# pk17r/online_3d_reconstruction

Hardware: AMD Instinct MI355X
Metric: frames_per_sec (higher is better)
Workload: dtype f32; 1 GPU; synthetic 1280x720 dense stereo, jump_pixels 1, 200 frames/GPU, voxel_size 0.05, min_points_per_voxel 1, SOR off, frames resident in HBM (BASELINE.json configs[1]); frames_per_gpu=200, rows=720, cols=1280, jump_pixels=1, parallelism=frame-sharded x1

## Files before the change

### include/o3dr_testing.h

```cpp
#ifndef O3DR_TESTING_H
#define O3DR_TESTING_H
#include "o3dr.h"
#ifdef __cplusplus
extern "C" {
#endif

int o3dr_test_corrupt_next_gather(o3dr_ctx* ctx);

int o3dr_test_sor_distances(o3dr_ctx* ctx, float* out, int64_t n);

int o3dr_test_local_comm_create(int32_t n_ranks, void** comm_out);
int o3dr_test_local_comm_destroy(void* comm);
int o3dr_test_merge_partitioned_local(o3dr_ctx* ctx, void* local_comm, int32_t rank, int32_t gather_result, o3dr_point* out,
                                      int64_t out_capacity, int64_t* n_out, int64_t* n_total, uint32_t* status, int32_t mem);
int o3dr_test_fail_at(o3dr_ctx* ctx, int32_t point);
int o3dr_test_plane_hypotheses(o3dr_ctx* ctx, float* planes, uint32_t* counts, int64_t capacity, int64_t* n_out);

#ifdef __cplusplus
}
#endif
#endif
```

### online_3d_reconstruction_amd/_lib.py

```python
import ctypes as C
import os

import numpy as np

_HERE = os.path.dirname(os.path.abspath(__file__))
_LIB = os.path.join(_HERE, "lib", "libo3dr.so")

POINT = np.dtype([("x", "<f4"), ("y", "<f4"), ("z", "<f4"), ("rgba", "<u4")])

OK = 0
ERR_INVALID_ARG, ERR_NO_DEVICE, ERR_HIP, ERR_CAPACITY, ERR_NOT_CONFIGURED, ERR_ALLOC, ERR_INTERNAL, ERR_PEER = -1, -2, -3, -4, -5, -6, -7, -8
MEM_HOST, MEM_DEVICE = 0, 1
STATUS_VOXEL_OVERFLOW = 1
STATUS_INTERNAL = 0x80000000
K_COUNT, K_REPROJECT, K_KEYGEN, K_SORT_HIST, K_SORT_SCATTER, K_SEGMENT, K_CENTROID, K_OTHER, K_CENTROID_RUNS = range(9)
KERNEL_NAMES = ["reproject_count", "reproject_emit", "voxel_keys", "radix_hist", "radix_scatter", "run_segments",
                "centroid", "other", "centroid_runs"]


class O3drError(RuntimeError):
    def __init__(self, code, text):
        super().__init__(f"libo3dr error {code}: {text}")
        self.code = code

# ... 51 lines not shown

KNN2 = np.dtype([("train_idx", "<u4", (2,)), ("distance", "<u4", (2,))])
assert KNN2.itemsize == 16
RIGID_RESULT = np.dtype([("T", "<f8", (16,)), ("rms", "<f8"), ("n_used", "<i8"), ("status", "<i4"), ("reserved", "<i4")])
assert RIGID_RESULT.itemsize == C.sizeof(RigidResultStruct) == 152
MATCH_NONE = 0xFFFFFFFF
RIGID_OK, RIGID_TOO_FEW, RIGID_DEGENERATE = range(3)


def lib_path():
    return _LIB


_vp, _i64, _i32, _u32, _f = C.c_void_p, C.c_int64, C.c_int32, C.c_uint32, C.c_float
_pi64, _pu32 = C.POINTER(C.c_int64), C.POINTER(C.c_uint32)
SYMBOLS = [
    ("o3dr_version", C.c_int, []),
    ("o3dr_last_error", C.c_char_p, []),
    ("o3dr_default_params", None, [C.POINTER(ParamsStruct)]),
    ("o3dr_ctx_create", C.c_int, [C.c_int, C.POINTER(_vp)]),
    ("o3dr_ctx_destroy", C.c_int, [_vp]),
    ("o3dr_ctx_set_stream", C.c_int, [_vp, _vp]),
    ("o3dr_ctx_synchronize", C.c_int, [_vp]),
    ("o3dr_set_camera", C.c_int, [_vp, _vp]),
    ("o3dr_set_params", C.c_int, [_vp, C.POINTER(ParamsStruct)]),
    ("o3dr_get_params", C.c_int, [_vp, C.POINTER(ParamsStruct)]),
    ("o3dr_create_single_img_pt_cloud", C.c_int, [_vp, _vp, _i64, _vp, _i64, _i32, _i32, _vp, _i32, _vp, _i64, _pi64, _i32]),
    ("o3dr_max_points", _i64, [_vp, _i32, _i32]),
    ("o3dr_transform_pt_cloud", C.c_int, [_vp, _vp, _i64, _vp, _vp, _i32]),
    ("o3dr_reproject_transform", C.c_int, [_vp, _vp, _i64, _vp, _i64, _i32, _i32, _vp, _vp, _i32, _vp, _i64, _pi64, _i32]),
    ("o3dr_voxel_grid", C.c_int, [_vp, _vp, _i64, _vp, _u32, _f, _vp, _i64, _pi64, _pu32, _i32]),
    ("o3dr_statistical_outlier_removal", C.c_int, [_vp, _vp, _i64, _vp, _i64, _pi64, _i32]),
    ("o3dr_bilateral_filter_u8", C.c_int, [_vp, _vp, _i64, _i32, _i32, _i32, C.c_double, C.c_double, _vp, _i64, _i32]),
    ("o3dr_disparity_variance", C.c_int, [_vp, _vp, _i64, _i64, _i32, _i32, _i32, _vp, _i32]),
    ("o3dr_downsample_pt_cloud", C.c_int, [_vp, _vp, _i64, _i32, _vp, _i64, _pi64, _pu32, _i32]),
    ("o3dr_create_and_transform_pt_cloud", C.c_int, [_vp, _vp, _i64, _vp, _i64, _i32, _i32, _vp, _vp, _i32, _vp, _i64, _pi64, _pu32, _i32]),
    ("o3dr_accumulate_frames", C.c_int, [_vp, _vp, _i64, _i64, _vp, _i64, _i64, _i32, _i32, _vp, _i32, _i32]),
    ("o3dr_accumulate_frames_kp", C.c_int, [_vp, _vp, _i64, _i64, _vp, _i64, _i64, _i32, _i32, _vp, _i32, _vp, _vp, _i32]),
    ("o3dr_cloud_big_reserve", C.c_int, [_vp, _i64]),
    ("o3dr_cloud_big_reset", C.c_int, [_vp]),
    ("o3dr_cloud_big_size", C.c_int, [_vp, _pi64, _pu32]),
    ("o3dr_cloud_big_read", C.c_int, [_vp, _vp, _i64, _pi64, _i32]),
    ("o3dr_cloud_big_append", C.c_int, [_vp, _vp, _i64, _i32]),
    ("o3dr_cloud_big_transform", C.c_int, [_vp, _vp]),
    ("o3dr_finalize", C.c_int, [_vp, _vp, _i64, _pi64, _pu32, _i32]),
    ("o3dr_finalize_incremental", C.c_int, [_vp, _vp, _i64, _pi64, _pu32, _i32]),
    ("o3dr_finalize_incremental_stats", C.c_int, [_vp, _pi64]),
    ("o3dr_cloud_big_bbox", C.c_int, [_vp, _vp, _vp, _pi64]),
    ("o3dr_cloud_big_partition", C.c_int, [_vp, _vp, _vp, _i32, _pi64, _pu32]),
    ("o3dr_finalize_global", C.c_int, [_vp, _vp, _vp, _vp, _i64, _pi64, _pu32, _i32]),
    ("o3dr_cloud_big_view", C.c_int, [_vp, C.POINTER(_vp), _pi64]),
    ("o3dr_cloud_big_recv_buffer", C.c_int, [_vp, _i64, C.POINTER(_vp)]),
    ("o3dr_cloud_big_adopt", C.c_int, [_vp, _i64]),
    ("o3dr_cloud_big_header_dev", C.c_int, [_vp, _vp]),
    ("o3dr_cloud_big_assume_size", C.c_int, [_vp, _i64]),
    ("o3dr_cloud_big_partition_dev", C.c_int, [_vp, _vp, _i32, _i32, _vp]),
    ("o3dr_cloud_big_slice_counts_dev", C.c_int, [_vp, _vp, _i32, _i32, _vp]),
    ("o3dr_cloud_big_place_slices", C.c_int, [_vp, _i32, _i32, _vp, _i64, _i64, _pi64]),
    ("o3dr_cloud_big_set_size", C.c_int, [_vp, _i64]),
    ("o3dr_cloud_big_raw_view", C.c_int, [_vp, C.POINTER(_vp), _pi64]),
    ("o3dr_merge_partitioned", C.c_int, [_vp, _vp, _i32, _vp, _i64, _pi64, _pi64, C.POINTER(C.c_uint32), _i32]),
    ("o3dr_merge_partitioned_stats", C.c_int, [_vp, _pi64]),
    ("o3dr_cloud_big_capacity", C.c_int, [_vp, _pi64, _pi64]),
    ("o3dr_comm_init_all", C.c_int, [_i32, _vp, _vp]),
    ("o3dr_comm_destroy", C.c_int, [_vp]),
    ("o3dr_host_register", C.c_int, [_vp, _i64]),
    ("o3dr_host_unregister", C.c_int, [_vp]),
    ("o3dr_icp_default_params", None, [C.POINTER(IcpParamsStruct)]),
    ("o3dr_nearest_neighbors", C.c_int, [_vp, _vp, _i64, _vp, _i64, C.c_double, _vp, _vp, _i32]),
    ("o3dr_icp_align", C.c_int, [_vp, _vp, _i64, _vp, _i64, _vp, C.POINTER(IcpParamsStruct), C.POINTER(IcpResultStruct), _i32]),
    ("o3dr_match_default_params", None, [C.POINTER(MatchParamsStruct)]),
    ("o3dr_match_knn2_hamming", C.c_int, [_vp, _vp, _vp, _i32, _vp, _i64, C.POINTER(MatchParamsStruct), _vp, _vp, _i64, _pi64, _i32]),
    ("o3dr_keypoints_3d", C.c_int, [_vp, _vp, _i64, _i64, _vp, _i64, _i64, _i32, _i32, _vp, _i32, _vp, _vp, _vp, _i64, _pi64, _i32]),
    ("o3dr_estimate_rigid_transform", C.c_int, [_vp, _vp, _vp, _i64, _vp, _i32, _vp, _vp, _i32]),
    ("o3dr_mls_default_params", None, [C.POINTER(MlsParamsStruct)]),
    ("o3dr_mls_smooth", C.c_int, [_vp, _vp, _i64, C.POINTER(MlsParamsStruct), _vp, _vp, _vp, _vp, C.POINTER(MlsResultStruct), _i32]),
    ("o3dr_plane_default_params", None, [C.POINTER(PlaneParamsStruct)]),
    ("o3dr_segment_plane", C.c_int, [_vp, _vp, _i64, C.POINTER(PlaneParamsStruct), _vp, _vp, _vp, _vp, _i64, _pi64, _i32]),
    ("o3dr_profile_enable", C.c_int, [_vp, _i32, _i32]),
    ("o3dr_profile_read", C.c_int, [_vp, _i32, C.POINTER(C.c_double), _pi64]),
    ("o3dr_profile_reset", C.c_int, [_vp]),
    ("o3dr_profile_stats", C.c_int, [_vp, _pi64]),
    ("o3dr_test_corrupt_next_gather", C.c_int, [_vp]),
    ("o3dr_test_sor_distances", C.c_int, [_vp, _vp, _i64]),
    ("o3dr_test_local_comm_create", C.c_int, [_i32, C.POINTER(_vp)]),
    ("o3dr_test_local_comm_destroy", C.c_int, [_vp]),
    ("o3dr_test_merge_partitioned_local", C.c_int, [_vp, _vp, _i32, _i32, _vp, _i64, _pi64, _pi64, C.POINTER(C.c_uint32), _i32]),
    ("o3dr_test_fail_at", C.c_int, [_vp, _i32]),
    ("o3dr_test_plane_hypotheses", C.c_int, [_vp, _vp, _vp, _i64, _pi64]),
    ("o3dr_device_info", C.c_int, [_vp, C.c_char_p, _i32, C.POINTER(_i32), _pi64]),
]

_lib = None


def load_library():
    global _lib
    if _lib is None:
        if not os.path.exists(_LIB):
            raise O3drError(ERR_NO_DEVICE, f"{_LIB} is not built: run `python __graft_entry__.py` or `make` "
                                           "(there is no CPU fallback)")
        try:
            import torch
        except ImportError:
            pass
        L = C.CDLL(_LIB)
        for name, res, args in SYMBOLS:
            fn = getattr(L, name)
            fn.restype = res
            fn.argtypes = args
        _lib = L
    return _lib


def check(code):
    if code != OK:
        raise O3drError(code, load_library().o3dr_last_error().decode(errors="replace"))
```

### online_3d_reconstruction_amd/csrc/kernels/bookkeeping.inc

```

__global__ void k_minmax_init(float* mm, int64_t mm_stride, int slot, uint32_t* n_kp, int frames)
{
    const int i = blockIdx.x * blockDim.x + threadIdx.x;
    if (i < frames * 6) {
        const int f = i / 6, a = i % 6;
        mm[((int64_t)f * mm_stride + slot) * 6 + a] = (a < 3) ? __builtin_inff() : -__builtin_inff();
    }
    if (n_kp && i < frames) n_kp[i] = 0;
}
__global__ void k_set_counts(uint32_t* n_dev, uint32_t value, int frames)
{
    const int i = blockIdx.x * blockDim.x + threadIdx.x;
    if (i < frames) n_dev[i] = value;
}

__device__ __forceinline__ int64_t scan_row_len(const VoxelGeom* __restrict__ geom, int f, int pass, int n_tiles,
                                                int64_t L)
{
    if (!geom) return L;
    const VoxelGeom g = geom[f];
    if (g.overflow || pass >= (int)g.passes) return 0;
    return (int64_t)geom_bins(g) * n_tiles;
}
__device__ __forceinline__ int scan_live_tiles(const VoxelGeom* __restrict__ geom, int f, int n_tiles)
{
    if (!geom) return n_tiles;
    const int64_t live = ((int64_t)geom[f].n + kSortTile - 1) / kSortTile;
    return live < n_tiles ? (int)live : n_tiles;
}
__global__ __launch_bounds__(1024) void k_scan_rows(uint32_t* __restrict__ data, int64_t L_in, int64_t row_stride,
                                                    uint32_t* __restrict__ totals, const uint32_t* __restrict__ add,
                                                    const VoxelGeom* __restrict__ geom, int pass, int n_tiles,
                                                    int chunked)
{
    __shared__ uint32_t lds[1024 / 64 + 1];
    uint32_t* row = data + (int64_t)blockIdx.x * row_stride;
    int64_t L = scan_row_len(geom, blockIdx.x, pass, n_tiles, L_in);
    if (chunked) L = (L + 4095) / 4096;
    if (L == 0 && !totals) return;
    const int64_t chunk = (L + 1023) / 1024;
    const int64_t b = (int64_t)threadIdx.x * chunk;
    const int64_t e = (b + chunk < L) ? b + chunk : L;
    const bool tiles = geom != nullptr && !chunked;
    const int live = tiles ? scan_live_tiles(geom, blockIdx.x, n_tiles) : 0;
    uint32_t s = 0;
    {
        int t = tiles ? (int)(b % n_tiles) : 0;
        for (int64_t i = b; i < e; ++i) {
            if (!tiles || t < live) s += row[i];
            if (tiles && ++t == n_tiles) t = 0;
        }
    }
    uint32_t total;
    uint32_t run = block_excl_scan_u32<16>(s, lds, total);
    {
        int t = tiles ? (int)(b % n_tiles) : 0;
        for (int64_t i = b; i < e; ++i) {
            const uint32_t v = (!tiles || t < live) ? row[i] : 0u;
            row[i] = run;
            run += v;
            if (tiles && ++t == n_tiles) t = 0;
        }
    }
    if (totals && threadIdx.x == 0) totals[blockIdx.x] = total + (add ? add[blockIdx.x] : 0u);
}

__global__ __launch_bounds__(1024) void k_scan_hist_tm(uint32_t* __restrict__ hist, const VoxelGeom* __restrict__ geom, int pass,
                                                       int n_tiles)
{
    extern __shared__ uint32_t tm_row[];
    __shared__ uint32_t lds[1024 / 64 + 1];
    const int f = blockIdx.x;
    const VoxelGeom g = geom[f];
    if (g.overflow || pass >= (int)g.passes) return;
    const int bins = geom_bins(g);
    uint32_t* row = hist + (int64_t)f * kMaxRadix * n_tiles;
    const int words = n_tiles * kMaxRadix;
    const int live = scan_live_tiles(geom, f, n_tiles);
    for (int i = threadIdx.x; i < words; i += 1024)
        tm_row[(i >> kMaxRadixBits) * (kMaxRadix + 1) + (i & (kMaxRadix - 1))] = (i >> kMaxRadixBits) < live ? row[i] : 0u;
    __syncthreads();
    const int L = bins * n_tiles;
    const int chunk = (L + 1023) / 1024;
    const int b = (int)threadIdx.x * chunk, e = b + chunk < L ? b + chunk : L;
    uint32_t s = 0;
    {
        int d = b / n_tiles, t = b - d * n_tiles;
        for (int i = b; i < e; ++i) {
            s += tm_row[t * (kMaxRadix + 1) + d];
            if (++t == n_tiles) t = 0, ++d;
        }
    }
    uint32_t total;
    uint32_t run = block_excl_scan_u32<16>(s, lds, total);
    {
        int d = b / n_tiles, t = b - d * n_tiles;
        for (int i = b; i < e; ++i) {
            const uint32_t v = tm_row[t * (kMaxRadix + 1) + d];
            tm_row[t * (kMaxRadix + 1) + d] = run;
            run += v;
            if (++t == n_tiles) t = 0, ++d;
        }
    }
    __syncthreads();
    for (int i = threadIdx.x; i < words; i += 1024)
        if ((i & (kMaxRadix - 1)) < bins) row[i] = tm_row[(i >> kMaxRadixBits) * (kMaxRadix + 1) + (i & (kMaxRadix - 1))];
}

constexpr int kScanChunk = 4096;
__global__ __launch_bounds__(256) void k_scan_chunk_sums(const uint32_t* __restrict__ data, int64_t L_in,
                                                         int64_t row_stride, int n_chunks,
                                                         uint32_t* __restrict__ partial,
                                                         const VoxelGeom* __restrict__ geom, int pass, int n_tiles)
{
    __shared__ uint32_t lds[4];
    const int64_t L = scan_row_len(geom, blockIdx.y, pass, n_tiles, L_in);
    if ((int64_t)blockIdx.x * kScanChunk >= L) return;
    const uint32_t* row = data + (int64_t)blockIdx.y * row_stride;
    const int64_t b = (int64_t)blockIdx.x * kScanChunk + (int64_t)threadIdx.x * 16;
    const int live = scan_live_tiles(geom, blockIdx.y, n_tiles);
    int t = geom ? (int)(b % n_tiles) : 0;
    uint32_t s = 0;
#pragma unroll
    for (int k = 0; k < 16; ++k) {
        if (b + k < L && (!geom || t < live)) s += row[b + k];
        if (geom && ++t == n_tiles) t = 0;
    }
    s = wave_sum_u32(s);
    if ((threadIdx.x & 63) == 0) lds[threadIdx.x >> 6] = s;
    __syncthreads();
    if (threadIdx.x == 0) partial[(int64_t)blockIdx.y * n_chunks + blockIdx.x] = lds[0] + lds[1] + lds[2] + lds[3];
}
__global__ __launch_bounds__(256) void k_scan_chunk_apply(uint32_t* __restrict__ data, int64_t L_in, int64_t row_stride,
                                                          int n_chunks, const uint32_t* __restrict__ partial_scanned,
                                                          const VoxelGeom* __restrict__ geom, int pass, int n_tiles)
{
    __shared__ uint32_t lds[5];
    const int64_t L = scan_row_len(geom, blockIdx.y, pass, n_tiles, L_in);
    if ((int64_t)blockIdx.x * kScanChunk >= L) return;
    uint32_t* row = data + (int64_t)blockIdx.y * row_stride;
    const int64_t b = (int64_t)blockIdx.x * kScanChunk + (int64_t)threadIdx.x * 16;
    const int live = scan_live_tiles(geom, blockIdx.y, n_tiles);
    int t = geom ? (int)(b % n_tiles) : 0;
    uint32_t v[16];
    uint32_t s = 0;
#pragma unroll
    for (int k = 0; k < 16; ++k) {
        v[k] = (b + k < L && (!geom || t < live)) ? row[b + k] : 0u;
        s += v[k];
        if (geom && ++t == n_tiles) t = 0;
    }
    uint32_t total;
    uint32_t run = block_excl_scan_u32<4>(s, lds, total) + partial_scanned[(int64_t)blockIdx.y * n_chunks + blockIdx.x];
#pragma unroll
    for (int k = 0; k < 16; ++k) {
        if (b + k < L) row[b + k] = run;
        run += v[k];
    }
}

__global__ __launch_bounds__(kPtThreads) void k_points_minmax(const o3dr_point* __restrict__ in, int64_t in_fstride,
                                                              const uint32_t* __restrict__ n_dev, int64_t mm_stride,
                                                              float* __restrict__ mm)
{
    __shared__ float mm_lds[6 * (kPtThreads / 64)];
    const int f = blockIdx.y;
    const int64_t n = n_dev[f];
    const uint4* src = reinterpret_cast<const uint4*>(in + (int64_t)f * in_fstride);
    float lo[3] = {__builtin_inff(), __builtin_inff(), __builtin_inff()};
    float hi[3] = {-__builtin_inff(), -__builtin_inff(), -__builtin_inff()};
    bool any = false;
    const int64_t stride = (int64_t)gridDim.x * (kPtThreads * 4);
    for (int64_t base = (int64_t)blockIdx.x * (kPtThreads * 4); base < n; base += stride) {
#pragma unroll
        for (int k = 0; k < 4; ++k) {
            const int64_t i = base + k * kPtThreads + threadIdx.x;
            if (i < n) {
// ... 12 lines not shown
```

### online_3d_reconstruction_amd/csrc/kernels/radix_sort.inc

```

__device__ __forceinline__ int64_t hist_at(bool tm, int dgt, int tile, int n_tiles)
{
    return tm ? (int64_t)tile * kMaxRadix + dgt : (int64_t)dgt * n_tiles + tile;
}

__global__ __launch_bounds__(kSortThreads) void k_radix_hist(const uint32_t* __restrict__ keys0,
                                                             const uint32_t* __restrict__ keys1, int64_t cap,
                                                             const VoxelGeom* __restrict__ geom, int pass,
                                                             int n_tiles, uint32_t* __restrict__ hist,
                                                             uint32_t* __restrict__ hist_part, int tm)
{
    constexpr int kSub = 4;
    __shared__ uint32_t h[kSub * kSortWaves * kMaxRadix];
    const int f = blockIdx.y, tile = blockIdx.x;
    const VoxelGeom g = geom[f];
    if (g.overflow || pass >= (int)g.passes) return;
    const uint32_t n = g.n;
    if ((int64_t)tile * kSortTile >= (int64_t)n) return;
    const int bins = geom_bins(g), shift = pass * (int)g.bpp;
    const uint32_t dmask = (uint32_t)bins - 1u;
    for (int i = threadIdx.x; i < kSub * kSortWaves * kMaxRadix; i += kSortThreads) h[i] = 0;
    __syncthreads();
    const uint32_t* src = (((pass + g.buf0) & 1) ? keys1 : keys0) + (int64_t)f * cap;
    const int64_t base = (int64_t)tile * kSortTile;
    uint32_t* hw = h + (((threadIdx.x >> 6) * kSub) + (threadIdx.x & (kSub - 1))) * kMaxRadix;
    if (base < n) {
        const bool vec = (((int64_t)f * cap) & 3) == 0;
        static_assert(kScatParts == 2 && kSortRounds / 4 == 4, "the first scatter part is rounds 0 and 1");
        uint4 v[kSortRounds / 4];
        bool whole[kSortRounds / 4];
#pragma unroll
        for (int r = 0; r < kSortRounds / 4; ++r) {
            const int64_t i = base + ((int64_t)r * kSortThreads + threadIdx.x) * 4;
            whole[r] = vec && i + 3 < n;
            if (whole[r]) v[r] = stream_load_u4(reinterpret_cast<const uint4*>(src + i));
        }
#pragma unroll
        for (int r = 0; r < kSortRounds / 4; ++r) {
            const int64_t i = base + ((int64_t)r * kSortThreads + threadIdx.x) * 4;
            if (r == kSortRounds / 8) {
                __syncthreads();
                for (int dgt = threadIdx.x; dgt < bins; dgt += kSortThreads) {
                    uint32_t t = 0;
#pragma unroll
                    for (int ww = 0; ww < kSub * kSortWaves; ++ww) t += h[ww * kMaxRadix + dgt];
                    hist_part[(int64_t)f * kMaxRadix * n_tiles + hist_at(tm != 0, dgt, tile, n_tiles)] = t;
                }
                __syncthreads();
            }
            if (whole[r]) {
                atomicAdd(&hw[(v[r].x >> shift) & dmask], 1u);
                atomicAdd(&hw[(v[r].y >> shift) & dmask], 1u);
                atomicAdd(&hw[(v[r].z >> shift) & dmask], 1u);
                atomicAdd(&hw[(v[r].w >> shift) & dmask], 1u);
            } else {
                for (int k = 0; k < 4; ++k)
                    if (i + k < n) atomicAdd(&hw[(src[i + k] >> shift) & dmask], 1u);
            }
        }
    }
    __syncthreads();
    uint32_t* dst = hist + (int64_t)f * kMaxRadix * n_tiles;
    for (int dgt = threadIdx.x; dgt < bins; dgt += kSortThreads) {
        uint32_t t = 0;
#pragma unroll
        for (int ww = 0; ww < kSub * kSortWaves; ++ww) t += h[ww * kMaxRadix + dgt];
        dst[hist_at(tm != 0, dgt, tile, n_tiles)] = t;
    }
}

__global__ __launch_bounds__(kSortThreads) void k_voxel_keys_hist0(const o3dr_point* __restrict__ in, int64_t in_fstride,
                                                                   const VoxelGeom* __restrict__ geom, float z_offset,
                                                                   int64_t cap, uint32_t* __restrict__ keys, int n_tiles,
                                                                   uint32_t* __restrict__ hist, uint32_t* __restrict__ hist_part,
                                                                   const VoxelGeom* __restrict__ skip_grouped, int tm)
{
    constexpr int kSub = 4;
    __shared__ uint32_t h[kSub * kSortWaves * kMaxRadix];
    const int f = blockIdx.y, tile = blockIdx.x;
    const VoxelGeom g = geom[f];
    if (g.overflow || g.n == 0u || g.passes == 0u) return;
    if (skip_grouped && skip_grouped[f].grouped != 0u) return;
    const uint32_t n = g.n;
    const int64_t base = (int64_t)tile * kSortTile;
    if (base >= (int64_t)n) return;
    const int bins = geom_bins(g);
    const uint32_t dmask = (uint32_t)bins - 1u;
    for (int i = threadIdx.x; i < kSub * kSortWaves * kMaxRadix; i += kSortThreads) h[i] = 0;
    __syncthreads();
    const uint4* src = reinterpret_cast<const uint4*>(in + (int64_t)f * in_fstride);
    uint32_t* dst = keys + (int64_t)f * cap;
    uint32_t* hw = h + (((threadIdx.x >> 6) * kSub) + (threadIdx.x & (kSub - 1))) * kMaxRadix;
#pragma unroll
    for (int r = 0; r < kSortRounds; ++r) {
        const int64_t i = base + (int64_t)r * kSortThreads + threadIdx.x;
        if (r == kSortRounds / kScatParts) {
            __syncthreads();
            for (int dgt = threadIdx.x; dgt < bins; dgt += kSortThreads) {
                uint32_t t = 0;
#pragma unroll
                for (int ww = 0; ww < kSub * kSortWaves; ++ww) t += h[ww * kMaxRadix + dgt];
                hist_part[(int64_t)f * kMaxRadix * n_tiles + hist_at(tm != 0, dgt, tile, n_tiles)] = t;
            }
            __syncthreads();
        }
        if (i < n) {
            const uint32_t key = voxel_key_of(src[i], g, z_offset);
            dst[i] = key;
            atomicAdd(&hw[key & dmask], 1u);
        }
    }
    __syncthreads();
    uint32_t* hd = hist + (int64_t)f * kMaxRadix * n_tiles;
    for (int dgt = threadIdx.x; dgt < bins; dgt += kSortThreads) {
        uint32_t t = 0;
#pragma unroll
        for (int ww = 0; ww < kSub * kSortWaves; ++ww) t += h[ww * kMaxRadix + dgt];
        hd[hist_at(tm != 0, dgt, tile, n_tiles)] = t;
    }
}

constexpr int kCntStride = 17;
constexpr int kCntWords = kMaxRadix * kCntStride;
constexpr int kRankWords = kScatWaves * kCntWords;
struct ScatterLds {
    __attribute__((aligned(16))) uint32_t smem[kRankWords > 2 * kScatTile ? kRankWords : 2 * kScatTile];
    uint32_t wave_tot[kScatWaves * kMaxRadix];
    uint32_t local_base[kMaxRadix];
    uint32_t delta[kMaxRadix];
    uint32_t scan_lds[kScatWaves + 1];
};
struct ScatterJob {
    const uint32_t *kin, *vin;
    uint32_t *kout, *vout;
    const uint32_t* hist;
    const uint32_t* hist_part;
    uint32_t n, dmask;
    int shift, bins, pass, n_tiles;
    bool frame_vec;
    bool tm;
};

__device__ __forceinline__ void scatter_load(const ScatterJob& J, int tile, int part, uint32_t (&key)[kSortRounds],
                                             uint32_t (&val)[kSortRounds], uint32_t& gstart)
{
    const int lane = threadIdx.x & 63, w = threadIdx.x >> 6;
    const int64_t n = J.n;
    const int64_t lbase = (int64_t)tile * kSortTile + (int64_t)part * kScatTile + (int64_t)w * kSortWaveItems + (int64_t)lane * kSortRounds;
    gstart = 0;
    if ((int)threadIdx.x < J.bins) {
        gstart = J.hist[hist_at(J.tm, threadIdx.x, tile, J.n_tiles)];
        if (part != 0) gstart += J.hist_part[hist_at(J.tm, threadIdx.x, tile, J.n_tiles)];
    }
    const bool vec = J.frame_vec && (lbase + kSortRounds <= n);
    if (vec) {
#pragma unroll
        for (int q = 0; q < kSortRounds / 4; ++q) {
            const uint4 k4 = *reinterpret_cast<const uint4*>(J.kin + lbase + 4 * q);
            key[4 * q] = k4.x; key[4 * q + 1] = k4.y; key[4 * q + 2] = k4.z; key[4 * q + 3] = k4.w;
        }
        if (J.pass != 0) {
#pragma unroll
            for (int q = 0; q < kSortRounds / 4; ++q) {
                const uint4 v4 = *reinterpret_cast<const uint4*>(J.vin + lbase + 4 * q);
                val[4 * q] = v4.x; val[4 * q + 1] = v4.y; val[4 * q + 2] = v4.z; val[4 * q + 3] = v4.w;
            }
        }
    } else {
#pragma unroll
        for (int r = 0; r < kSortRounds; ++r) {
            const int64_t i = lbase + r;
            const bool ok = i < n;
            key[r] = ok ? J.kin[i] : 0xffffffffu;
            val[r] = (J.pass != 0 && ok) ? J.vin[i] : 0u;
        }
    }
    if (J.pass == 0) {
#pragma unroll
        for (int r = 0; r < kSortRounds; ++r) val[r] = (uint32_t)(lbase + r);
    }
}

__device__ __forceinline__ void scatter_tile(const ScatterJob& J, int tile, int part, ScatterLds& L, const uint32_t (&key)[kSortRounds],
                                             const uint32_t (&val)[kSortRounds], uint32_t gstart)
{
    uint32_t* smem = L.smem;
    uint32_t* stage = L.smem;
    const int lane = threadIdx.x & 63, w = threadIdx.x >> 6;
    const int64_t n = J.n;
    const int64_t base = (int64_t)tile * kSortTile + (int64_t)part * kScatTile;
    const uint32_t cnt = (n - base < (int64_t)kScatTile) ? (uint32_t)(n - base) : (uint32_t)kScatTile;
    const int64_t lbase = base + (int64_t)w * kSortWaveItems + (int64_t)lane * kSortRounds;
    const int shift = J.shift, bins = J.bins;
    const uint32_t dmask = J.dmask;
    for (int i = threadIdx.x; i < kRankWords; i += kScatThreads) smem[i] = 0;
    __syncthreads();

    uint32_t* cw = smem + w * kCntWords;
    const int quad = lane >> 2, sub = lane & 3;
    const uint32_t fsh = 7u * (uint32_t)sub;
    uint32_t own[kSortRounds];
#pragma unroll
    for (int r = 0; r < kSortRounds; ++r) {
        own[r] = 0;
        if (lbase + r < n) {
            const uint32_t dgt = (key[r] >> shift) & dmask;
            const uint32_t old = atomicAdd(&cw[dgt * kCntStride + quad], 1u << fsh);
            own[r] = (old >> fsh) & 127u;
        }
    }
    __builtin_amdgcn_wave_barrier();
#pragma unroll
    for (int h = 0; h < kMaxRadix / 64; ++h) {
        const int row = lane + 64 * h;
        if (row < bins) {
            uint32_t run = 0;
#pragma unroll
            for (int j = 0; j < 16; ++j) {
                const uint32_t v = cw[row * kCntStride + j];
                const uint32_t t = v + (v << 7);
                const uint32_t t2 = t + (t << 14);
                cw[row * kCntStride + j] = (run << 21) | (t2 & 0x1fffffu);
                run += (t2 >> 21) & 127u;
            }
            L.wave_tot[w * kMaxRadix + row] = run;
        }
    }
    __syncthreads();

    uint32_t tot = 0;
    const int dg = threadIdx.x;
    if (dg < bins) {
#pragma unroll
        for (int ww = 0; ww < kScatWaves; ++ww) {
            const uint32_t t = L.wave_tot[ww * kMaxRadix + dg];
            L.wave_tot[ww * kMaxRadix + dg] = tot;
            tot += t;
        }
    }
    uint32_t tile_total;
    const uint32_t lb = block_excl_scan_u32<kScatWaves>(tot, L.scan_lds, tile_total);
    if (dg < bins) {
        L.local_base[dg] = lb;
        L.delta[dg] = gstart - lb;
    }
    __syncthreads();

    uint32_t pos[kSortRounds];
    const uint32_t qsh = sub ? 7u * (uint32_t)(sub - 1) : 0u, qmk = sub ? 127u : 0u;
#pragma unroll
    for (int r = 0; r < kSortRounds; ++r) {
        if (lbase + r < n) {
            const uint32_t dgt = (key[r] >> shift) & dmask;
            const uint32_t v = cw[dgt * kCntStride + quad];
            pos[r] = L.local_base[dgt] + L.wave_tot[w * kMaxRadix + dgt] + (v >> 21) + ((v >> qsh) & qmk) + own[r];
        }
    }
    __syncthreads();
    uint32_t* stage_v = L.smem + kScatTile;
#pragma unroll
    for (int r = 0; r < kSortRounds; ++r) {
        if (lbase + r < n) {
            stage[pos[r]] = key[r];
            stage_v[pos[r]] = val[r];
        }
    }
    __syncthreads();
#pragma unroll
    for (int r = 0; r < kSortRounds; ++r) {
        const uint32_t p = r * kScatThreads + threadIdx.x;
        if (p < cnt) {
            const uint32_t k = stage[p];
            const uint32_t d = p + L.delta[(k >> shift) & dmask];
            J.kout[d] = k;
            J.vout[d] = stage_v[p];
        }
    }
}

__global__ __launch_bounds__(kScatThreads) void k_radix_scatter_lane(uint32_t* __restrict__ keys0, uint32_t* __restrict__ vals0,
                                                                     uint32_t* __restrict__ keys1, uint32_t* __restrict__ vals1,
                                                                     int64_t cap, const VoxelGeom* __restrict__ geom, int pass,
                                                                     int n_tiles, const uint32_t* __restrict__ hist_scanned,
                                                                     const uint32_t* __restrict__ hist_part, int tm)
{
    __shared__ ScatterLds L;
    const int f = blockIdx.y;
    const VoxelGeom g = geom[f];
    if (g.overflow || pass >= (int)g.passes) return;
    const int item = xcd_chunk_item(blockIdx.x, (int)(((int64_t)g.n + kScatTile - 1) / kScatTile));
    if (item < 0) return;
    const int tile = item / kScatParts, part = item % kScatParts;
    ScatterJob J;
    const int par = (pass + (int)g.buf0) & 1;
    J.kin = (par ? keys1 : keys0) + (int64_t)f * cap;
    J.vin = (par ? vals1 : vals0) + (int64_t)f * cap;
    J.kout = (par ? keys0 : keys1) + (int64_t)f * cap;
    J.vout = (par ? vals0 : vals1) + (int64_t)f * cap;
    J.hist = hist_scanned + (int64_t)f * kMaxRadix * n_tiles;
    J.hist_part = hist_part + (int64_t)f * kMaxRadix * n_tiles;
    J.n = g.n;
    J.bins = geom_bins(g);
    J.dmask = (uint32_t)J.bins - 1u;
    J.shift = pass * (int)g.bpp;
    J.pass = pass;
    J.n_tiles = n_tiles;
    J.frame_vec = (((int64_t)f * cap) & 3) == 0;
    J.tm = tm != 0;
    uint32_t key0[kSortRounds], val0[kSortRounds], g0;
    scatter_load(J, tile, part, key0, val0, g0);
    scatter_tile(J, tile, part, L, key0, val0, g0);
}
```

### online_3d_reconstruction_amd/csrc/kernels/util.inc

```

__device__ __forceinline__ int xcd_chunk_item(int bx, int n_active)
{
    const int chunk = (n_active + kXcds - 1) / kXcds, q = bx / kXcds;
    const int item = (bx % kXcds) * chunk + q;
    return (q < chunk && item < n_active) ? item : -1;
}
typedef uint32_t u32x4_t __attribute__((ext_vector_type(4)));
__device__ __forceinline__ uint4 stream_load_u4(const uint4* p)
{
    const u32x4_t v = __builtin_nontemporal_load(reinterpret_cast<const u32x4_t*>(p));
    return make_uint4(v.x, v.y, v.z, v.w);
}
__device__ __forceinline__ uint32_t wave_incl_scan_u32(uint32_t v)
{
    v += (uint32_t)__builtin_amdgcn_update_dpp(0, (int)v, 0x111, 0xf, 0xf, false);
    v += (uint32_t)__builtin_amdgcn_update_dpp(0, (int)v, 0x112, 0xf, 0xf, false);
    v += (uint32_t)__builtin_amdgcn_update_dpp(0, (int)v, 0x114, 0xf, 0xf, false);
    v += (uint32_t)__builtin_amdgcn_update_dpp(0, (int)v, 0x118, 0xf, 0xf, false);
    v += (uint32_t)__builtin_amdgcn_update_dpp(0, (int)v, 0x142, 0xa, 0xf, false);
    v += (uint32_t)__builtin_amdgcn_update_dpp(0, (int)v, 0x143, 0xc, 0xf, false);
    return v;
}
__device__ __forceinline__ int32_t wave_shr1_i32(int32_t v) { return __builtin_amdgcn_update_dpp(v, v, 0x138, 0xf, 0xf, false); }
__device__ __forceinline__ uint32_t wave_max_u32(uint32_t v)
// ... 23 lines not shown
    return (uint32_t)__builtin_amdgcn_readlane((int)wave_incl_scan_u32(v), 63);
}
__device__ __forceinline__ uint32_t f32_ordered(float f)
{
    const uint32_t u = __float_as_uint(f);
    return u ^ ((uint32_t)((int32_t)u >> 31) | 0x80000000u);
}
__device__ __forceinline__ float ordered_f32(uint32_t u) { return __uint_as_float(u ^ (((u >> 31) - 1u) | 0x80000000u)); }
#define O3DR_WAVE_REDUCE_ORD(name, op, ident)                                                                                  \
    __device__ __forceinline__ float name(float f)                                                                       \
    {                                                                                                                    \
         \
        uint32_t v = f32_ordered(f);                                                                                     \
        v = op(v, (uint32_t)__builtin_amdgcn_update_dpp((int)(ident), (int)v, 0x111, 0xf, 0xf, false));                  \
        v = op(v, (uint32_t)__builtin_amdgcn_update_dpp((int)(ident), (int)v, 0x112, 0xf, 0xf, false));                  \
        v = op(v, (uint32_t)__builtin_amdgcn_update_dpp((int)(ident), (int)v, 0x114, 0xf, 0xf, false));                  \
        v = op(v, (uint32_t)__builtin_amdgcn_update_dpp((int)(ident), (int)v, 0x118, 0xf, 0xf, false));                  \
        v = op(v, (uint32_t)__builtin_amdgcn_update_dpp((int)(ident), (int)v, 0x142, 0xa, 0xf, false));                  \
        v = op(v, (uint32_t)__builtin_amdgcn_update_dpp((int)(ident), (int)v, 0x143, 0xc, 0xf, false));                  \
        return ordered_f32((uint32_t)__builtin_amdgcn_readlane((int)v, 63));                                             \
    }
__device__ __forceinline__ uint32_t u32_min(uint32_t a, uint32_t b) { return a < b ? a : b; }
__device__ __forceinline__ uint32_t u32_max(uint32_t a, uint32_t b) { return a > b ? a : b; }
O3DR_WAVE_REDUCE_ORD(wave_min_f32, u32_min, 0xffffffffu)
O3DR_WAVE_REDUCE_ORD(wave_max_f32, u32_max, 0u)
#undef O3DR_WAVE_REDUCE_ORD
template <int NW>
__device__ __forceinline__ uint32_t block_excl_scan_u32(uint32_t v, uint32_t* lds, uint32_t& total)
{
    const int lane = threadIdx.x & 63, w = threadIdx.x >> 6;
    const uint32_t incl = wave_incl_scan_u32(v);
    if (lane == 63) lds[w] = incl;
    __syncthreads();
    if (threadIdx.x == 0) {
        uint32_t run = 0;
#pragma unroll
        for (int i = 0; i < NW; ++i) {
            const uint32_t t = lds[i];
            lds[i] = run;
            run += t;
        }
        lds[NW] = run;
    }
    __syncthreads();
    const uint32_t r = lds[w] + incl - v;
    total = lds[NW];
    __syncthreads();
    return r;
}
template <int NW, int N>
__device__ __forceinline__ void block_excl_scan_multi_u32(uint32_t (&v)[N], uint32_t* lds, uint32_t (&total)[N])
{
    const int lane = threadIdx.x & 63, w = threadIdx.x >> 6;
    uint32_t incl[N];
#pragma unroll
    for (int j = 0; j < N; ++j) {
        incl[j] = wave_incl_scan_u32(v[j]);
        if (lane == 63) lds[w * N + j] = incl[j];
    }
    __syncthreads();
    if ((int)threadIdx.x < N) {
        uint32_t run = 0;
#pragma unroll
        for (int i = 0; i < NW; ++i) {
            const uint32_t t = lds[i * N + threadIdx.x];
            lds[i * N + threadIdx.x] = run;
            run += t;
        }
        lds[NW * N + threadIdx.x] = run;
    }
    __syncthreads();
#pragma unroll
    for (int j = 0; j < N; ++j) {
        v[j] = lds[w * N + j] + incl[j] - v[j];
        total[j] = lds[NW * N + j];
    }
    __syncthreads();
}
__device__ __forceinline__ int geom_bins(const VoxelGeom& g)
{
    const uint32_t bpp = g.bpp < (uint32_t)kMaxRadixBits ? g.bpp : (uint32_t)kMaxRadixBits;
    return 1 << bpp;
}
__device__ __forceinline__ uint32_t voxel_key_of(const uint4 v, const VoxelGeom& g, float z_offset)
{
    const float x = __uint_as_float(v.x), y = __uint_as_float(v.y), z = __uint_as_float(v.z) + z_offset;
    const int32_t i0 = (int32_t)floorf(x * g.inv[0]) - g.min_b[0];
    const int32_t i1 = (int32_t)floorf(y * g.inv[1]) - g.min_b[1];
    const int32_t i2 = (int32_t)floorf(z * g.inv[2]) - g.min_b[2];
    return (uint32_t)i0 + (uint32_t)i1 * g.mul1 + (uint32_t)i2 * g.mul2;
}
struct GroupCoord {
    int32_t bx, iy, iz;
};
__device__ __forceinline__ GroupCoord group_coord_of(const uint4 v, const float inv[3], float z_offset, uint32_t& cell)
{
    const float x = __uint_as_float(v.x), y = __uint_as_float(v.y), z = __uint_as_float(v.z) + z_offset;
    const int32_t i0 = (int32_t)floorf(x * inv[0]);
    cell = (uint32_t)(i0 & (kGroupCells - 1));
    GroupCoord c;
    c.bx = i0 >> kGroupBits;
    c.iy = (int32_t)floorf(y * inv[1]);
    c.iz = (int32_t)floorf(z * inv[2]);
    return c;
}
__device__ __forceinline__ bool group_differs(const GroupCoord& a, const GroupCoord& b)
{
    return a.bx != b.bx || a.iy != b.iy || a.iz != b.iz;
}
__device__ __forceinline__ uint32_t group_blocks_x(const VoxelGeom& g)
{
    return (uint32_t)(((g.min_b[0] + g.div_b[0] - 1) >> kGroupBits) - (g.min_b[0] >> kGroupBits) + 1);
}
__device__ __forceinline__ uint32_t group_key_of(const GroupCoord& c, const VoxelGeom& g)
{
    const uint32_t i1 = (uint32_t)(c.iy - g.min_b[1]), i2 = (uint32_t)(c.iz - g.min_b[2]);
    return (uint32_t)(c.bx - (g.min_b[0] >> kGroupBits)) + group_blocks_x(g) * (i1 + (uint32_t)g.div_b[1] * i2);
}
__device__ __forceinline__ void head_flag_place(uint64_t i, uint64_t& word, uint32_t& bit)
{
    word = i >> 4;
    bit = (uint32_t)(((i >> 2) & 3u) * 8u + (i & 3u));
}
__device__ __forceinline__ const uint32_t* sorted_buf(const VoxelGeom& g, const uint32_t* b0, const uint32_t* b1)
{
    return ((g.passes + g.buf0) & 1u) ? b1 : b0;
}
template <int NW>
__device__ __forceinline__ void block_minmax_store(const float lo[3], const float hi[3], bool any,
                                                   float* lds , float* __restrict__ slot6)
{
    const int lane = threadIdx.x & 63, w = threadIdx.x >> 6;
#pragma unroll
    for (int a = 0; a < 3; ++a) {
        const float l = wave_min_f32(any ? lo[a] : __builtin_inff());
        const float h = wave_max_f32(any ? hi[a] : -__builtin_inff());
        if (lane == 0) {
            lds[w * 6 + a] = l;
            lds[w * 6 + 3 + a] = h;
        }
    }
    __syncthreads();
    if (threadIdx.x < 6) {
        const int a = threadIdx.x;
        float v = lds[a];
#pragma unroll
        for (int i = 1; i < NW; ++i) v = (a < 3) ? fminf(v, lds[i * 6 + a]) : fmaxf(v, lds[i * 6 + a]);
        slot6[a] = v;
    }
    __syncthreads();
}

constexpr int kMlsJacobiSweeps = 8;
__device__ __forceinline__ void mls_jacobi3(double A[3][3], double V[3][3])
{
#pragma unroll
    for (int i = 0; i < 3; ++i)
#pragma unroll
        for (int j = 0; j < 3; ++j) V[i][j] = i == j ? 1.0 : 0.0;
    A[1][0] = A[0][1], A[2][0] = A[0][2], A[2][1] = A[1][2];
#pragma unroll
    for (int sweep = 0; sweep < kMlsJacobiSweeps; ++sweep) {
#pragma unroll
        for (int pq = 0; pq < 3; ++pq) {
            const int p = pq == 2 ? 1 : 0, q = pq == 0 ? 1 : 2, r = 3 - p - q;
            const double apq = A[p][q];
// ... 20 lines not shown
```

### online_3d_reconstruction_amd/csrc/kernels/voxel_runs.inc

```


constexpr int kHeadWaves = 4;
__global__ __launch_bounds__(kHeadWaves * kWave) void k_run_heads(const uint32_t* __restrict__ keys0, const uint32_t* __restrict__ keys1,
                                                                  int64_t cap, const VoxelGeom* __restrict__ geom, int n_tiles,
                                                                  uint32_t* __restrict__ seg_cnt, int buf_sel,
                                                                  uint8_t* __restrict__ head_bits)
{
    static_assert(kSegTile == 16 * kWave, "16 records per lane");
    const int f = blockIdx.y, lane = threadIdx.x & 63;
    const int tile = blockIdx.x * kHeadWaves + (threadIdx.x >> 6);
    const VoxelGeom g = geom[f];
    if (g.overflow || tile >= n_tiles) return;
    const int64_t n = g.n;
    const uint32_t* k = (buf_sel < 0 ? sorted_buf(g, keys0, keys1) : (buf_sel ? keys1 : keys0)) + (int64_t)f * cap;
    uint32_t c = 0;
    const int64_t i0 = (int64_t)tile * kSegTile + lane * 16;
    if ((int64_t)tile * kSegTile < n) {
        uint32_t kk[16];
        if (((((int64_t)f * cap) & 3) == 0) && i0 + 15 < n) {
#pragma unroll
            for (int q = 0; q < 4; ++q) {
                const uint4 v = *reinterpret_cast<const uint4*>(k + i0 + 4 * q);
                kk[4 * q] = v.x; kk[4 * q + 1] = v.y; kk[4 * q + 2] = v.z; kk[4 * q + 3] = v.w;
            }
        } else {
#pragma unroll
            for (int q = 0; q < 16; ++q) kk[q] = (i0 + q < n) ? k[i0 + q] : 0u;
        }
        uint32_t prev = (uint32_t)wave_shr1_i32((int32_t)kk[15]);
        if (lane == 0) prev = (i0 > 0 && i0 < n) ? k[i0 - 1] : 0u;
        uint32_t bits = 0;
#pragma unroll
        for (int q = 0; q < 16; ++q) {
            const int64_t i = i0 + q;
            if (i < n && (i == 0 || kk[q] != (q ? kk[q - 1] : prev))) bits |= 1u << ((q >> 2) * 8 + (q & 3));
        }
        reinterpret_cast<uint32_t*>(head_bits + ((int64_t)f * n_tiles + tile) * 256)[lane] = bits;
        c = (uint32_t)__popc(bits);
    }
    c = wave_sum_u32(c);
    if (lane == 0) seg_cnt[(int64_t)f * n_tiles + tile] = c;
}

constexpr int kStartWaves = 4;
__global__ __launch_bounds__(kStartWaves * kWave) void k_run_starts(
    const uint32_t* __restrict__ keys0, const uint32_t* __restrict__ keys1, int64_t cap, const VoxelGeom* __restrict__ geom,
    int n_tiles, const uint32_t* __restrict__ seg_off, const uint32_t* __restrict__ n_vox, uint32_t* __restrict__ seg_start,
    int buf_sel, uint32_t* __restrict__ head_keys_out, const VoxelGeom* __restrict__ mode, const o3dr_point* __restrict__ in_pts,
    float z_offset, const uint8_t* __restrict__ head_bits)
{
    static_assert(kSegTile == 16 * kWave, "16 records per lane");
    const int f = blockIdx.y, lane = threadIdx.x & 63;
    const int tile = blockIdx.x * kStartWaves + (threadIdx.x >> 6);
    const VoxelGeom g = geom[f];
    if (g.overflow) return;
    if (mode && mode[f].grouped == 0u) return;
    const uint32_t n = g.n;
    const int64_t base = (int64_t)tile * kSegTile;
    if (tile >= n_tiles || base >= n) return;
    uint32_t* ss = seg_start + (int64_t)f * (cap + 1);
    if (tile == 0 && lane == 0) ss[n_vox[f]] = n;
    uint32_t bits = reinterpret_cast<const uint32_t*>(head_bits + ((int64_t)f * n_tiles + tile) * 256)[lane];
    bits &= 0x0f0f0f0fu;
    if (base + lane * 16 + 16 > (int64_t)n) {
#pragma unroll
        for (int q = 0; q < 16; ++q)
            if (base + lane * 16 + q >= (int64_t)n) bits &= ~(1u << ((q >> 2) * 8 + (q & 3)));
    }
    const uint32_t cnt = (uint32_t)__popc(bits);
    const uint32_t incl = wave_incl_scan_u32(cnt);
    const uint32_t tile_runs = __shfl(incl, 63, 64);
    __shared__ uint32_t stage_all[kStartWaves][kSegTile];
    uint32_t* stage = stage_all[threadIdx.x >> 6];
    uint32_t pos = incl - cnt;
    const uint32_t i0 = (uint32_t)base + (uint32_t)lane * 16u;
#pragma unroll
    for (int q = 0; q < 16; ++q) {
        if (bits & (1u << ((q >> 2) * 8 + (q & 3)))) stage[pos++] = i0 + (uint32_t)q;
    }
    __builtin_amdgcn_wave_barrier();
    const uint32_t off = seg_off[(int64_t)f * n_tiles + tile];
    for (uint32_t j = lane; j < tile_runs; j += kWave) {
        const uint32_t i = stage[j];
        ss[off + j] = i;
        if (head_keys_out) {
            uint32_t cell;
            const GroupCoord gc = group_coord_of(reinterpret_cast<const uint4*>(in_pts)[i], g.inv, z_offset, cell);
            head_keys_out[(int64_t)f * cap + off + j] = group_key_of(gc, g);
        }
    }
}

__global__ __launch_bounds__(256) void k_keep_count(const uint32_t* __restrict__ seg_start, int64_t cap,
                                                    const VoxelGeom* __restrict__ geom,
                                                    const uint32_t* __restrict__ n_vox, uint32_t min_points,
                                                    int n_tiles, uint32_t* __restrict__ seg_cnt)
{
    __shared__ uint32_t lds[4];
    const int f = blockIdx.y, tile = blockIdx.x;
    if (geom[f].overflow || geom[f].grouped != 0u) return;
    const uint32_t nv = n_vox[f];
    const uint32_t* ss = seg_start + (int64_t)f * (cap + 1);
    uint32_t c = 0;
    const int64_t base = (int64_t)tile * kSegTile;
    if (base < nv) {
        for (int j = 0; j < kSegTile / 256; ++j) {
            const int64_t o = base + j * 256 + threadIdx.x;
            if (o < nv) c += (ss[o + 1] - ss[o] >= min_points) ? 1u : 0u;
        }
    }
    c = wave_sum_u32(c);
    if ((threadIdx.x & 63) == 0) lds[threadIdx.x >> 6] = c;
    __syncthreads();
    if (threadIdx.x == 0) seg_cnt[(int64_t)f * n_tiles + tile] = lds[0] + lds[1] + lds[2] + lds[3];
}
__global__ __launch_bounds__(256) void k_keep_write(const uint32_t* __restrict__ seg_start, int64_t cap,
                                                    const VoxelGeom* __restrict__ geom,
                                                    const uint32_t* __restrict__ n_vox, uint32_t min_points,
                                                    int n_tiles, const uint32_t* __restrict__ seg_off,
                                                    uint32_t* __restrict__ keep_idx)
{
    __shared__ uint32_t scan_lds[5];
    const int f = blockIdx.y, tile = blockIdx.x;
    if (geom[f].overflow || geom[f].grouped != 0u) return;
    const uint32_t nv = n_vox[f];
    const int64_t base = (int64_t)tile * kSegTile;
    if (base >= nv) return;
    const uint32_t* ss = seg_start + (int64_t)f * (cap + 1);
    uint32_t* ki = keep_idx + (int64_t)f * cap;
    uint32_t off = seg_off[(int64_t)f * n_tiles + tile];
    for (int j = 0; j < kSegTile / 256; ++j) {
        const int64_t o = base + j * 256 + threadIdx.x;
        const bool keep = (o < nv) && (ss[o + 1] - ss[o] >= min_points);
        uint32_t total;
        const uint32_t pos = block_excl_scan_u32<4>(keep ? 1u : 0u, scan_lds, total);
        if (keep) ki[off + pos] = (uint32_t)o;
        off += total;
    }
}

__global__ __launch_bounds__(256) void k_frame_offsets(const VoxelGeom* __restrict__ geom, const uint32_t* __restrict__ n_vox,
                                                       const uint32_t* __restrict__ n_keep,
                                                       const uint32_t* __restrict__ n_grp, int frames, int passthrough,
                                                       uint32_t* __restrict__ n_out, uint64_t* __restrict__ out_off,
                                                       CloudCounters* __restrict__ cc, SortStats* __restrict__ stats,
                                                       const VoxelGeom* __restrict__ sort_geom)
{
    __shared__ uint32_t scan_lds[5];
    __shared__ unsigned long long acc[6];
    if (threadIdx.x < 6) acc[threadIdx.x] = 0;
    __syncthreads();
    const uint64_t base = cc->count;
    uint64_t carry = 0;
    for (int f0 = 0; f0 < frames; f0 += 256) {
        const int f = f0 + threadIdx.x;
        uint32_t m = 0;
        if (f < frames) {
            const VoxelGeom g = geom[f];
            if (passthrough) {
                m = g.n;
            } else if (g.overflow) {
                m = g.n;
                atomicOr(&acc[3], (unsigned long long)O3DR_STATUS_VOXEL_OVERFLOW);
            } else {
                m = (n_grp && sort_geom[f].grouped) ? n_grp[f] : (n_keep ? n_keep[f] : n_vox[f]);
                atomicAdd(&acc[0], (unsigned long long)sort_geom[f].n * g.passes);
                atomicAdd(&acc[5], (unsigned long long)sort_geom[f].n);
                atomicAdd(&acc[1], (unsigned long long)g.n);
                atomicAdd(&acc[2], (unsigned long long)m);
            }
        }
        uint32_t total;
        const uint32_t excl = block_excl_scan_u32<4>(m, scan_lds, total);
        if (f < frames) {
            n_out[f] = m;
            out_off[f] = base + carry + excl;
        }
        carry += total;
    }
    __syncthreads();
    if (threadIdx.x == 0) {
        cc->count = base + carry;
        cc->status |= (uint32_t)acc[3];
        if (stats) {
            stats->sort_record_passes += acc[0];
            stats->voxel_points_in += acc[1];
            stats->voxel_points_out += acc[2];
            stats->sort_records += acc[5];
        }
    }
}

__global__ void k_test_corrupt_payload(uint32_t* __restrict__ vals0, uint32_t* __restrict__ vals1, const VoxelGeom* __restrict__ geom)
{
    const VoxelGeom g = geom[0];
    if (g.overflow || g.n == 0u) return;
    uint32_t* v = ((g.passes + g.buf0) & 1u) ? vals1 : vals0;
    v[g.n / 2u] = 0xfffffff0u;
}

__device__ __forceinline__ void centroid_block(int64_t bx, int f, const VoxelGeom& g, uint32_t n_o,
                                               const o3dr_point* __restrict__ in, int64_t in_fstride,
                                               const uint32_t* __restrict__ vals0, const uint32_t* __restrict__ vals1,
                                               int64_t cap, const uint32_t* __restrict__ seg_start,
                                               const uint32_t* __restrict__ keep_idx, const uint64_t* __restrict__ out_off,
                                               float z_offset, int passthrough, o3dr_point* __restrict__ out_base,
                                               float* __restrict__ out_mm, int nbx, CloudCounters* __restrict__ cc,
                                               const CloudHeads& ch)
{
    const int64_t o = bx * kPtThreads + threadIdx.x;
    const bool active = o < (int64_t)n_o;
    if (__ballot(active) == 0ull) return;
    uint4 res = make_uint4(0, 0, 0, 0);
    if (active) {
        const uint4* src = reinterpret_cast<const uint4*>(in + (int64_t)f * in_fstride);
        if (passthrough) {
            res = src[o];
        } else if (g.overflow) {
            res = src[o];
            res.z = __float_as_uint((__uint_as_float(res.z) + z_offset) - z_offset);
        } else {
            const uint32_t* ss = seg_start + (int64_t)f * (cap + 1);
            const uint32_t* pid = sorted_buf(g, vals0, vals1) + (int64_t)f * cap;
            const uint32_t v = keep_idx ? keep_idx[(int64_t)f * cap + o] : (uint32_t)o;
            uint32_t b = ss[v], e = ss[v + 1];
            bool bad = b > e || e > g.n;
            if (bad) b = e = 0;
            float sx = 0.f, sy = 0.f, sz = 0.f, sr = 0.f, sg = 0.f, sb = 0.f, sa = 0.f;
            for (uint32_t li = b; li < e; li += 8) {
                uint32_t id[8];
                uint4 p[8];
#pragma unroll
                for (int k = 0; k < 8; ++k) {
                    id[k] = (li + k < e) ? pid[li + k] : 0xffffffffu;
                    if (id[k] != 0xffffffffu && id[k] >= g.n) {
                        bad = true;
                        id[k] = 0xffffffffu;
                    }
                }
#pragma unroll
                for (int k = 0; k < 8; ++k)
                    if (id[k] != 0xffffffffu) p[k] = src[id[k]];
#pragma unroll
                for (int k = 0; k < 8; ++k) {
                    if (id[k] != 0xffffffffu) {
                        sx += __uint_as_float(p[k].x);
                        sy += __uint_as_float(p[k].y);
                        sz += __uint_as_float(p[k].z) + z_offset;
                        sr += (float)((p[k].w >> 16) & 255u);
                        sg += (float)((p[k].w >> 8) & 255u);
                        sb += (float)(p[k].w & 255u);
                        sa += (float)(p[k].w >> 24);
                    }
                }
            }
            const float nf = (float)(e - b);
            const float cx = sx / nf, cy = sy / nf, cz = sz / nf - z_offset;
            const uint32_t rgba = ((uint32_t)(sa / nf) << 24) | ((uint32_t)(sr / nf) << 16) | ((uint32_t)(sg / nf) << 8) |
                                  (uint32_t)(sb / nf);
            res = make_uint4(__float_as_uint(cx), __float_as_uint(cy), __float_as_uint(cz), rgba);
            if (bad) atomicOr(&cc->status, O3DR_STATUS_INTERNAL);
        }
        reinterpret_cast<uint4*>(out_base + out_off[f])[o] = res;
    }
    if (ch.flags) {
        uint32_t cell;
        GroupCoord gc = {0, 0, 0};
        if (active) gc = group_coord_of(res, ch.inv, ch.z_offset, cell);
        GroupCoord prev;
        prev.bx = wave_shr1_i32(gc.bx);
        prev.iy = wave_shr1_i32(gc.iy);
        prev.iz = wave_shr1_i32(gc.iz);
        const int lane = threadIdx.x & 63;
        const unsigned long long hm = __ballot(active && lane != 0 && group_differs(gc, prev));
        if (hm != 0ull && lane < 5) {
            const uint64_t g0 = out_off[f] + (uint64_t)(o - lane);
            const uint64_t word = (g0 >> 4) + (uint64_t)lane;
            const int shift = (int)((int64_t)(word << 4) - (int64_t)g0);
            uint32_t f16 = 0;
            if (shift < 64) f16 = (uint32_t)((shift >= 0 ? (hm >> shift) : (hm << -shift)) & 0xffffull);
            const uint32_t bits = (f16 & 0xfu) | ((f16 & 0xf0u) << 4) | ((f16 & 0xf00u) << 8) | ((f16 & 0xf000u) << 12);
            if (bits) atomicOr(&ch.flags[word], bits);
        }
        int32_t* slot = ch.wave_gc + (((int64_t)f * nbx + bx) * (kPtThreads / 64) + (threadIdx.x >> 6)) * 6;
        const int last = 63 - __builtin_clzll(__ballot(active));
        const int32_t f0 = __builtin_amdgcn_readlane(gc.bx, 0), f1 = __builtin_amdgcn_readlane(gc.iy, 0),
                      f2 = __builtin_amdgcn_readlane(gc.iz, 0);
        const int32_t l0 = __builtin_amdgcn_readlane(gc.bx, last), l1 = __builtin_amdgcn_readlane(gc.iy, last),
                      l2 = __builtin_amdgcn_readlane(gc.iz, last);
        if (lane < 6) slot[lane] = lane == 0 ? f0 : (lane == 1 ? f1 : (lane == 2 ? f2 : (lane == 3 ? l0 : (lane == 4 ? l1 : l2))));
    }
    if (out_mm) {
        float* slot = out_mm + (((int64_t)f * nbx + bx) * (kPtThreads / 64) + (threadIdx.x >> 6)) * 6;
        const float c3[3] = {__uint_as_float(res.x), __uint_as_float(res.y), __uint_as_float(res.z)};
        float mine = 0.f;
#pragma unroll
        for (int a = 0; a < 3; ++a) {
            const float l = wave_min_f32(active ? c3[a] : __builtin_inff());
            const float h = wave_max_f32(active ? c3[a] : -__builtin_inff());
            if ((threadIdx.x & 63) == a) mine = l;
            if ((threadIdx.x & 63) == 3 + a) mine = h;
        }
        if ((threadIdx.x & 63) < 6) slot[threadIdx.x & 63] = mine;
    }
}

template <bool kStride>
__global__ __launch_bounds__(kPtThreads) void k_centroid(const o3dr_point* __restrict__ in, int64_t in_fstride,
                                                         const uint32_t* __restrict__ vals0,
                                                         const uint32_t* __restrict__ vals1, int64_t cap,
                                                         const uint32_t* __restrict__ seg_start,
                                                         const uint32_t* __restrict__ keep_idx,
                                                         const VoxelGeom* __restrict__ geom,
                                                         const uint32_t* __restrict__ n_out,
                                                         const uint64_t* __restrict__ out_off, float z_offset,
                                                         int passthrough, o3dr_point* __restrict__ out_base,
                                                         float* __restrict__ out_mm, int nbx, CloudCounters* __restrict__ cc,
                                                         CloudHeads ch)
{
    const int f = blockIdx.y;
    const VoxelGeom g = geom[f];
    if (!passthrough && (g.n == 0 || g.grouped != 0u)) return;
    const uint32_t n_o = n_out[f];
    if (kStride) {
        for (int64_t bx = blockIdx.x; bx * kPtThreads < (int64_t)n_o; bx += gridDim.x)
            centroid_block(bx, f, g, n_o, in, in_fstride, vals0, vals1, cap, seg_start, keep_idx, out_off, z_offset,
                           passthrough, out_base, out_mm, nbx, cc, ch);
    } else {
        const int bx = xcd_chunk_item(blockIdx.x, (int)(((int64_t)n_o + kPtThreads - 1) / kPtThreads));
        if (bx < 0) return;
        centroid_block(bx, f, g, n_o, in, in_fstride, vals0, vals1, cap, seg_start, keep_idx, out_off, z_offset,
                       passthrough, out_base, out_mm, nbx, cc, ch);
    }
}

__global__ __launch_bounds__(256) void k_cloud_heads_fix(const uint32_t* __restrict__ n_out, const uint64_t* __restrict__ out_off,
                                                         int waves_per_frame, CloudHeads ch)
{
    const int f = blockIdx.y;
    const int64_t j = (int64_t)blockIdx.x * 256 + threadIdx.x;
    if (j >= waves_per_frame || j * kWave >= (int64_t)n_out[f]) return;
    bool head = j == 0;
    if (!head) {
        const int32_t* cur = ch.wave_gc + ((int64_t)f * waves_per_frame + j) * 6;
        head = cur[0] != cur[-3] || cur[1] != cur[-2] || cur[2] != cur[-1];
    }
    if (head) {
        uint64_t word;
        uint32_t bit;
        head_flag_place(out_off[f] + (uint64_t)j * kWave, word, bit);
        atomicOr(&ch.flags[word], 1u << bit);
    }
}

__global__ __launch_bounds__(256) void k_cloud_bbox_fold(const float* __restrict__ slots, int nbx, int frames,
                                                         const uint32_t* __restrict__ n_out, float* __restrict__ partial)
{
    __shared__ float mm_lds[6 * 4];
    float lo[3] = {__builtin_inff(), __builtin_inff(), __builtin_inff()};
    float hi[3] = {-__builtin_inff(), -__builtin_inff(), -__builtin_inff()};
    const int64_t total = (int64_t)nbx * frames;
    for (int64_t i = (int64_t)blockIdx.x * 256 + threadIdx.x; i < total; i += (int64_t)gridDim.x * 256) {
        const int f = (int)(i / nbx), bx = (int)(i - (int64_t)f * nbx);
        if ((int64_t)bx * 64 < (int64_t)n_out[f]) {
#pragma unroll
            for (int a = 0; a < 3; ++a) {
                lo[a] = fminf(lo[a], slots[i * 6 + a]);
                hi[a] = fmaxf(hi[a], slots[i * 6 + 3 + a]);
            }
        }
    }
    block_minmax_store<4>(lo, hi, true, mm_lds, partial + (int64_t)blockIdx.x * 6);
}
__global__ __launch_bounds__(384) void k_cloud_bbox_merge(const float* __restrict__ partial, int n_partial, float* __restrict__ box6)
{
    const int a = threadIdx.x >> 6, lane = threadIdx.x & 63;
    float v = a < 3 ? __builtin_inff() : -__builtin_inff();
    for (int i = lane; i < n_partial; i += 64) v = a < 3 ? fminf(v, partial[i * 6 + a]) : fmaxf(v, partial[i * 6 + a]);
    v = a < 3 ? wave_min_f32(v) : wave_max_f32(v);
    if (lane == 0) box6[a] = a < 3 ? fminf(box6[a], v) : fmaxf(box6[a], v);
}

__global__ void k_run_geom(const VoxelGeom* __restrict__ geom, const uint32_t* __restrict__ n_runs, int frames,
                           VoxelGeom* __restrict__ geom_runs, int force, int64_t slots)
{
    const int f = blockIdx.x * blockDim.x + threadIdx.x;
    if (f >= frames) return;
    VoxelGeom g = geom[f];
    const uint32_t nr = n_runs[f];
    const uint64_t group_keys = (uint64_t)group_blocks_x(g) * (uint64_t)(uint32_t)g.div_b[1] * (uint64_t)(uint32_t)g.div_b[2];
    uint64_t max_groups = group_keys;
    if ((uint64_t)nr < max_groups) max_groups = nr;
    const bool fits = max_groups * kGroupCells <= (uint64_t)slots;
    const bool pays = (uint64_t)nr * kGroupMinRunNum <= (uint64_t)g.n * kGroupMinRunDen;
    if (g.overflow) {
        g.grouped = 1;
        g.n = 0;
    } else if (fits && (pays || force)) {
        g.grouped = 1;
        g.n = nr;
        g.buf0 = 1;
        sort_plan(g, group_keys);
    }
    geom_runs[f] = g;
}

constexpr int kGroupChunks = 4;
constexpr int kGroupStep = kGroupChunks * kWave;
struct GroupLds {
    uint4 sorted[kGroupStep];
    unsigned long long mask[kWave][kGroupChunks];
    uint32_t pre[kWave][kGroupChunks];
    unsigned long long bnd[kGroupChunks];
};
__global__ __launch_bounds__(kGroupWaves * kWave) void k_centroid_groups(
    const o3dr_point* __restrict__ in, const uint32_t* __restrict__ keys0, const uint32_t* __restrict__ keys1,
    const uint32_t* __restrict__ ids0, const uint32_t* __restrict__ ids1, const uint32_t* __restrict__ seg_start,
    const uint32_t* __restrict__ run_start, const VoxelGeom* __restrict__ geom_runs, const VoxelGeom* __restrict__ geom_pts,
    const uint32_t* __restrict__ n_vox, float z_offset, uint32_t min_points, uint4* __restrict__ slots, int64_t n_slots,
    uint32_t* __restrict__ grp_cnt, CloudCounters* __restrict__ cc)
{
    __shared__ GroupLds lds[kGroupWaves];
    const VoxelGeom g = geom_runs[0];
    if (g.grouped == 0u || g.overflow) return;
    const VoxelGeom gp = geom_pts[0];
    const int lane = threadIdx.x & 63, w = threadIdx.x >> 6;
    GroupLds& L = lds[w];
#pragma unroll
    for (int q = 0; q < kGroupChunks; ++q) L.mask[lane][q] = 0ull;
    if (lane < kGroupChunks) L.bnd[lane] = 0ull;
    __builtin_amdgcn_wave_barrier();
    const uint32_t nv = n_vox[0], n_rec = g.n, n_points = gp.n;
    const uint32_t* sk = sorted_buf(g, keys0, keys1);
    const uint32_t* rv = sorted_buf(g, ids0, ids1);
    const uint4* src = reinterpret_cast<const uint4*>(in);
    const uint32_t need = min_points > 1u ? min_points : 1u;
    const bool flat = gp.div_b[2] == 1 && (uint32_t)gp.div_b[0] < (1u << 24) && (uint32_t)gp.div_b[1] < (1u << 24);
    const int32_t bx0 = gp.min_b[0] >> kGroupBits;
    const uint32_t nbx = group_blocks_x(gp);
    const unsigned long long lanes_below = (1ull << lane) - 1ull;
    const unsigned long long starts_upto = (2ull << lane) - 2ull;
    bool bad = false;
    for (uint32_t v = blockIdx.x * kGroupWaves + w; v < nv; v += gridDim.x * kGroupWaves) {
        uint32_t jb = seg_start[v], je = seg_start[v + 1];
        if (jb >= je || je > n_rec || ((int64_t)v + 1) * kGroupCells > n_slots) {
            bad = true;
            if (lane == 0 && ((int64_t)v + 1) * kGroupCells <= n_slots) grp_cnt[v] = 0;
// ... 98 lines not shown
                    }
                }
                __builtin_amdgcn_wave_barrier();
#pragma unroll
                for (int q = 0; q < kGroupChunks; ++q) {
                    if (okm & (1u << q)) {
                        const uint32_t pos = (L.pre[cq[q]][q] + (uint32_t)__popcll(L.mask[cq[q]][q] & lanes_below)) &
                                             (uint32_t)(kGroupStep - 1);
                        L.sorted[pos] = make_uint4(p[q].x, p[q].y, __float_as_uint(__uint_as_float(p[q].z) + z_offset), p[q].w);
                    }
                }
                __builtin_amdgcn_wave_barrier();
#pragma unroll
                for (int q = 0; q < kGroupChunks; ++q) L.mask[lane][q] = 0ull;
                n_pts += cnt;
                const uint32_t trips = wave_max_u32(cnt);
                for (uint32_t t = 0; t < trips; t += 4) {
                    uint4 a4[4];
#pragma unroll
                    for (int j = 0; j < 4; ++j) {
                        const uint4* at = (t + j < cnt) ? &L.sorted[(off + t) & (uint32_t)(kGroupStep - 1)] : &L.sorted[0];
                        a4[j] = at[j];
                    }
#pragma unroll
                    for (int j = 0; j < 4; ++j) {
                        if (t + j < cnt) {
                            const uint32_t c4 = a4[j].w;
                            s_xy += f32x2{__uint_as_float(a4[j].x), __uint_as_float(a4[j].y)};
                            sz += __uint_as_float(a4[j].z);
                            s_rg += f32x2{(float)((c4 >> 16) & 255u), (float)((c4 >> 8) & 255u)};
                            s_ba += f32x2{(float)(c4 & 255u), (float)(c4 >> 24)};
                        }
                    }
                }
                __builtin_amdgcn_wave_barrier();
#pragma unroll
                for (int q = 0; q < kGroupChunks; ++q) p[q] = pn[q];
                okm = okn;
            }
        }
        const bool keep = n_pts >= need;
        const unsigned long long km = __ballot(keep);
        if (keep) {
            const float nf = (float)n_pts;
            const float cx = s_xy.x / nf, cy = s_xy.y / nf, cz = sz / nf - z_offset;
            const uint32_t rgba = ((uint32_t)(s_ba.y / nf) << 24) | ((uint32_t)(s_rg.x / nf) << 16) | ((uint32_t)(s_rg.y / nf) << 8) |
                                  (uint32_t)(s_ba.x / nf);
            const uint32_t rank = (uint32_t)__popcll(km & lanes_below);
            slots[(int64_t)v * kGroupCells + rank] = make_uint4(__float_as_uint(cx), __float_as_uint(cy), __float_as_uint(cz), rgba);
        }
        if (lane == 0) grp_cnt[v] = (uint32_t)__popcll(km);
    }
    if (bad) atomicOr(&cc->status, O3DR_STATUS_INTERNAL);
}

__global__ __launch_bounds__(256) void k_group_compact(const o3dr_point* __restrict__ in, const VoxelGeom* __restrict__ geom_runs,
                                                       const VoxelGeom* __restrict__ geom_pts, const uint32_t* __restrict__ n_vox,
                                                       const uint32_t* __restrict__ grp_off, const uint4* __restrict__ slots,
                                                       const uint64_t* __restrict__ out_off, float z_offset,
                                                       o3dr_point* __restrict__ out_base)
{
    const VoxelGeom g = geom_runs[0];
    if (g.grouped == 0u) return;
    uint4* dst = reinterpret_cast<uint4*>(out_base + out_off[0]);
    const int64_t step = (int64_t)gridDim.x * 256;
    if (g.overflow) {
        const uint4* src = reinterpret_cast<const uint4*>(in);
        const int64_t n = geom_pts[0].n;
        for (int64_t o = (int64_t)blockIdx.x * 256 + threadIdx.x; o < n; o += step) {
            uint4 v = src[o];
            v.z = __float_as_uint((__uint_as_float(v.z) + z_offset) - z_offset);
            dst[o] = v;
        }
        return;
    }
    const int64_t total = (int64_t)n_vox[0] * kGroupCells;
    for (int64_t sidx = (int64_t)blockIdx.x * 256 + threadIdx.x; sidx < total; sidx += step) {
        const int64_t v = sidx >> kGroupBits;
        const uint32_t c = (uint32_t)(sidx & (kGroupCells - 1));
        const uint32_t o0 = grp_off[v], cnt = grp_off[v + 1] - o0;
        if (c < cnt) dst[o0 + c] = slots[sidx];
    }
}
```

### online_3d_reconstruction_amd/csrc/o3dr_api.hip

```cpp
#include <dlfcn.h>
#include <stdio.h>
#include <stdlib.h>
#include <string.h>

#include <algorithm>
#include <cfloat>
#include <chrono>
#include <cmath>
#include <condition_variable>
#include <mutex>
#include <string>
#include <vector>

#include <rccl/rccl.h>

#include "../../include/o3dr_testing.h"
#include "o3dr_device.h"
#include "o3dr_profile.h"

using namespace o3dr;

static thread_local std::string g_err;
static int fail(int code, const char* what)
{
    g_err = what;
    return code;
}
#define HIPCHK(expr)                                                                             \
    do {                                                                                         \
        hipError_t e_ = (expr);                                                                  \
        if (e_ != hipSuccess) {                                                                  \
            char buf_[512];                                                                      \
            snprintf(buf_, sizeof buf_, "%s failed: %s (%s:%d)", #expr, hipGetErrorString(e_), __FILE__, __LINE__); \
            g_err = buf_;                                                                        \
            return O3DR_ERR_HIP;                                                                 \
        }                                                                                        \
    } while (0)
#define CHK(expr)                  \
    do {                           \
        int r_ = (expr);           \
        if (r_ != O3DR_OK) return r_; \
    } while (0)

struct DevBuf {
    void* p = nullptr;
    size_t cap = 0;
};

struct o3dr_ctx {
    int device = 0;
    hipStream_t own_stream = nullptr;
    hipStream_t stream = nullptr;
    o3dr_params params;
    double Q[16];
    bool has_Q = false;
    QLutEntry* q_lut = nullptr;
    bool q_lut_on = false;
    DevBuf bil_tab, st_blur, st_blur_in, st_hist;
    int bil_d = 0, bil_radius = 0, bil_maxk = 0;
    double bil_sc = 0, bil_ss = 0;
    bool bil_valid = false;
    int max_batch = 256;
    int slab_shift_env = -2;
    int exact_box = 0;
    int use_runs = 1;
    int small_path = 1;

    Workspace ws;
    size_t ws_elems = 0;
    size_t ws_pts_elems = 0;
    int ws_frames = 0;
    size_t ws_emit_tiles = 0, ws_sort_tiles = 0, ws_seg_tiles = 0, ws_mm_floats = 0;
    DevBuf ws_block, ws_pts_block, ws_sor_block;
    int64_t ws_sor_cap = 0;
    int ws_sor_frames = 0;

    o3dr_point* cloud_big = nullptr;
    int64_t cloud_cap = 0;
    o3dr_point* cloud_alt = nullptr;
    int64_t cloud_alt_cap = 0;
    int64_t cloud_ub = 0;
    bool cloud_n_exact = true;
    float* cloud_box = nullptr;
    bool cloud_box_valid = false;
    uint32_t* cloud_heads = nullptr;
    int64_t cloud_heads_cap = 0;
    bool cloud_heads_valid = false;
    float cloud_heads_leaf[3] = {0.f, 0.f, 0.f};
    float cloud_heads_zo = 0.f;
    int cloud_box_enable = 1;
    CloudCounters* cc_big = nullptr;
    CloudCounters* cc_tmp = nullptr;
    CloudCounters* cc_host = nullptr;
    CloudCounters* cc_host_dev = nullptr;
    uint8_t* small_host = nullptr;
    uint32_t* n_host = nullptr;
    uint8_t* misc_dev = nullptr;
    uint8_t* misc_host = nullptr;
    uint8_t* misc_host_lut = nullptr;
    SortStats* stats_dev = nullptr;
    SortStats* stats_host = nullptr;

    DevBuf st_disp, st_bgr, st_in, st_out, st_kp, st_kpoff, st_poses;
    DevBuf st_xchg, st_merge, st_gather;
    uint8_t* xchg_host = nullptr;
    size_t xchg_host_cap = 0;
    DevBuf st2_disp[2], st2_bgr[2], st2_poses[2];
    hipStream_t copy_stream = nullptr;
    hipEvent_t ev_copied[2] = {nullptr, nullptr}, ev_done[2] = {nullptr, nullptr};
    int test_corrupt = 0;
    int test_fail_at = 0;
    int64_t xchg_stats[8] = {0, 0, 0, 0, 0, 0, 0, 0};
    DevBuf nn_q, nn_t, nn_cells, nn_src;
    DevBuf mls_out, mls_misc;
    DevBuf pl_pts, pl_tiles, pl_hyp, pl_misc, pl_out;
    uint64_t pl_last_hyp = 0;
    DevBuf mt_desc, mt_tab, mt_part, mt_out;
    std::vector<MatchPair> mt_tab_h;
    DevBuf rg_in, rg_work;
    std::vector<RigidSeg> rg_seg_h;
    std::vector<double> rg_T_h;
    int64_t place_ub = -1;
    int place_parts = 0;
    int test_hooks = 0;
    int host_batch = 32;
    uint64_t cloud_gen = 0;
    struct {
        bool valid = false;
        int64_t folded = 0;
        uint64_t gen = 0;
        float leaf[3] = {0.f, 0.f, 0.f};
        float zo = 0.f;
        uint32_t n_groups = 0, n_cells = 0;
        int cur = 0;
        DevBuf grp[2], off[2], cells[2], box;
        DevBuf scratch, tg, tmatch, flag, src, keep, partial, words;
        DevBuf fb;
        int64_t stats[8] = {0, 0, 0, 0, 0, 0, 0, 0};
    } inc;
    Profiler prof;
};

static int dev_ensure(o3dr_ctx* c, DevBuf& b, size_t bytes)
{
    if (bytes <= b.cap) return O3DR_OK;
    if (b.p) {
        HIPCHK(hipStreamSynchronize(c->stream));
        HIPCHK(hipFree(b.p));
        b.p = nullptr;
        b.cap = 0;
    }
    size_t want = bytes + bytes / 8 + 256;
    if (hipMalloc(&b.p, want) != hipSuccess) {
        (void)hipGetLastError();
        want = bytes;
        if (hipMalloc(&b.p, want) != hipSuccess) {
            b.p = nullptr;
            return fail(O3DR_ERR_ALLOC, "hipMalloc failed (workspace)");
        }
    }
    b.cap = want;
    return O3DR_OK;
}
static void dev_release(DevBuf& b)
{
    if (b.p) (void)hipFree(b.p);
    b.p = nullptr;
    b.cap = 0;
}

static inline size_t align256(size_t x) { return (x + 255) & ~(size_t)255; }

static int ws_ensure(o3dr_ctx* c, int frames, int64_t cap, bool need_pts, bool grp_tmp = false)
{
    if (cap < 1) cap = 1;
    const size_t elems = (size_t)frames * (size_t)(cap + 1);
    const size_t emit_tiles = (size_t)frames * (size_t)((cap + kEmitTile - 1) / kEmitTile);
    const size_t sort_tiles = (size_t)frames * (size_t)((cap + kSortTile - 1) / kSortTile);
    const size_t seg_tiles = (size_t)frames * (size_t)((cap + kSegTile - 1) / kSegTile);
    size_t mm_slots = (size_t)((cap + kEmitTile - 1) / kEmitTile) + 1;
    if (mm_slots < (size_t)kMinmaxBlocks) mm_slots = kMinmaxBlocks;
    const size_t mm_floats = (size_t)frames * mm_slots * 6;
    if (elems > c->ws_elems || frames > c->ws_frames || emit_tiles > c->ws_emit_tiles ||
        sort_tiles > c->ws_sort_tiles || seg_tiles > c->ws_seg_tiles || mm_floats > c->ws_mm_floats) {
        const size_t MM = mm_floats > c->ws_mm_floats ? mm_floats : c->ws_mm_floats;
        const size_t E = elems > c->ws_elems ? elems : c->ws_elems;
        const int F = frames > c->ws_frames ? frames : c->ws_frames;
        const size_t TE = emit_tiles > c->ws_emit_tiles ? emit_tiles : c->ws_emit_tiles;
        const size_t TS = sort_tiles > c->ws_sort_tiles ? sort_tiles : c->ws_sort_tiles;
        const size_t TG = seg_tiles > c->ws_seg_tiles ? seg_tiles : c->ws_seg_tiles;
        size_t off = 0;
        size_t o_keys0 = off; off += align256(E * 4);
        size_t o_keys1 = off; off += align256(E * 4);
        size_t o_vals0 = off; off += align256(E * 4);
        size_t o_vals1 = off; off += align256(E * 4);
        size_t o_seg = off;   off += align256(E * 4);
        size_t o_keep = off;  off += align256(E * 4);
        size_t o_rs = off;    off += align256(E * 4);
        size_t o_gc = off;    off += align256(((E > (size_t)kGroupMinSlots ? E : (size_t)kGroupMinSlots) / kGroupCells + 2) * 4);
        size_t o_tile = off;  off += align256(TE * 4);
        size_t o_hist = off;  off += align256(TS * kMaxRadix * 4);
        size_t o_histp = off; off += align256(TS * kMaxRadix * 4);
        size_t o_segc = off;  off += align256(TG * 4);
        size_t o_hb = off;    off += align256(TG * 256);
        size_t o_part = off;  off += align256(((TS * kMaxRadix + TG + TE + E) / 4096 + 8 * (size_t)F + 16) * 4);
        size_t o_mm = off;    off += align256(MM * 4);
        size_t o_nv = off;    off += align256((size_t)F * 4);
        size_t o_nk = off;    off += align256((size_t)F * 4);
        size_t o_nx = off;    off += align256((size_t)F * 4);
        size_t o_no = off;    off += align256((size_t)F * 4);
        size_t o_oo = off;    off += align256((size_t)F * 8);
        size_t o_geom = off;  off += align256((size_t)F * sizeof(VoxelGeom));
        size_t o_geomr = off; off += align256((size_t)F * sizeof(VoxelGeom));
        size_t o_nr = off;    off += align256((size_t)F * 4);
        size_t o_ng = off;    off += align256((size_t)F * 4);
        size_t o_omm = off;   off += align256((E / 64 + 8 * (size_t)F + 64) * 6 * sizeof(float));
        size_t o_ommp = off;  off += align256((size_t)kBoxFoldBlocks * 6 * sizeof(float));
        size_t o_wgc = off;   off += align256((E / 64 + 8 * (size_t)F + 64) * 6 * sizeof(int32_t));
        CHK(dev_ensure(c, c->ws_block, off));
        char* base = (char*)c->ws_block.p;
        Workspace& w = c->ws;
        w.keys[0] = (uint32_t*)(base + o_keys0);
        w.keys[1] = (uint32_t*)(base + o_keys1);
        w.vals[0] = (uint32_t*)(base + o_vals0);
        w.vals[1] = (uint32_t*)(base + o_vals1);
        w.seg_start = (uint32_t*)(base + o_seg);
        w.keep_idx = (uint32_t*)(base + o_keep);
        w.run_start = (uint32_t*)(base + o_rs);
        w.grp_cnt = (uint32_t*)(base + o_gc);
        w.n_grp_out = (uint32_t*)(base + o_ng);
        w.geom_runs = (VoxelGeom*)(base + o_geomr);
        w.n_runs = (uint32_t*)(base + o_nr);
        w.out_mm = (float*)(base + o_omm);
        w.out_mm_partial = (float*)(base + o_ommp);
        w.wave_gc = (int32_t*)(base + o_wgc);
        w.tile_cnt = (uint32_t*)(base + o_tile);
        w.hist = (uint32_t*)(base + o_hist);
        w.hist_part = (uint32_t*)(base + o_histp);
        w.seg_cnt = (uint32_t*)(base + o_segc);
        w.head_bits = (uint8_t*)(base + o_hb);
        w.scan_partial = (uint32_t*)(base + o_part);
        w.mm = (float*)(base + o_mm);
        w.n_valid = (uint32_t*)(base + o_nv);
        w.n_kp = (uint32_t*)(base + o_nk);
        w.n_vox = (uint32_t*)(base + o_nx);
        w.n_out = (uint32_t*)(base + o_no);
        w.out_off = (uint64_t*)(base + o_oo);
        w.geom = (VoxelGeom*)(base + o_geom);
        w.bytes = off;
        c->ws_elems = E;
        c->ws_frames = F;
        c->ws_emit_tiles = TE;
        c->ws_sort_tiles = TS;
        c->ws_seg_tiles = TG;
        c->ws_mm_floats = MM;
    }
    c->ws.mm_stride = (int64_t)mm_slots;
    c->ws.grp_slots = 0;
    if (need_pts || grp_tmp) {
        size_t pe = (size_t)frames * (size_t)cap;
        if (grp_tmp && pe < (size_t)kGroupMinSlots) pe = (size_t)kGroupMinSlots;
        if (grp_tmp) c->ws.grp_slots = (int64_t)pe;
        if (pe > c->ws_pts_elems) {
            CHK(dev_ensure(c, c->ws_pts_block, pe * sizeof(o3dr_point)));
            c->ws_pts_elems = pe;
        }
        c->ws.pts = (o3dr_point*)c->ws_pts_block.p;
    }
    c->ws.frames = frames;
    c->ws.cap = cap;
    return O3DR_OK;
}

static int sor_ensure(o3dr_ctx* c, int frames, int64_t cap)
{
    if (cap < 1) cap = 1;
    if (frames < 1) frames = 1;
    if (cap > c->ws_sor_cap || frames > c->ws_sor_frames) {
        const int64_t C = cap > c->ws_sor_cap ? cap : c->ws_sor_cap;
        const size_t F = (size_t)(frames > c->ws_sor_frames ? frames : c->ws_sor_frames);
        uint32_t max_cells = (uint32_t)(C / 2 > 1024 ? C / 2 : 1024);
        if (max_cells > (1u << 22)) max_cells = 1u << 22;
        size_t off = 0;
        size_t o_xyz = off;  off += align256(F * (size_t)C * 16);
        size_t o_pts = off;  off += align256(F * (size_t)C * 16);
        size_t o_dist = off; off += align256(F * (size_t)C * 4);
        size_t o_cf = off;   off += align256(F * ((size_t)max_cells + 1) * 4);
        size_t o_cz = off;   off += align256(F * ((size_t)max_cells + 1) * 8);
        size_t o_part = off; off += align256(F * 256 * 2 * 8);
        size_t o_geom = off; off += align256(F * sizeof(SorGeom));
        size_t o_n = off;    off += align256(F * 4);
        size_t o_left = off; off += align256(F * (size_t)C * 4);
        size_t o_lc = off;   off += align256(F * 4);
        CHK(dev_ensure(c, c->ws_sor_block, off));
        char* base = (char*)c->ws_sor_block.p;
        Workspace& w = c->ws;
        w.sor_xyz = (float4*)(base + o_xyz);
        w.sor_pts = (o3dr_point*)(base + o_pts);
        w.sor_dist = (float*)(base + o_dist);
        w.sor_cell_first = (uint32_t*)(base + o_cf);
        w.sor_cell_z = (float2*)(base + o_cz);
        w.sor_partial = (double*)(base + o_part);
        w.sor_geom = (SorGeom*)(base + o_geom);
        w.sor_n = (uint32_t*)(base + o_n);
        w.sor_left = (uint32_t*)(base + o_left);
        w.sor_left_cnt = (uint32_t*)(base + o_lc);
        w.sor_max_cells = max_cells;
        w.sor_cap = C;
        c->ws_sor_cap = C;
        c->ws_sor_frames = (int)F;
    }
    return O3DR_OK;
}
static inline bool sor_on(const o3dr_ctx* c) { return c->params.sor_enable && c->params.jump_pixels > 0; }

extern "C" int o3dr_version(void) { return O3DR_VERSION; }
extern "C" const char* o3dr_last_error(void) { return g_err.c_str(); }

extern "C" void o3dr_default_params(o3dr_params* p)
{
    if (!p) return;
    p->min_disparity = 64;
    p->voxel_size = 0.1;
    p->bounding_box = 20;
    p->cutout_ratio = 8;
    p->jump_pixels = 10;
    p->min_points_per_voxel = 1;
    p->dont_downsample = 0;
    p->sor_enable = 1;
    p->blur_kernel = 1;
    p->disparity_f64 = 0;
}

static int cloud_box_clear(o3dr_ctx* c);

extern "C" int o3dr_ctx_create(int device_id, o3dr_ctx** out_ctx)
{
    if (!out_ctx) return fail(O3DR_ERR_INVALID_ARG, "out_ctx is NULL");
    *out_ctx = nullptr;
    int n = 0;
    if (hipGetDeviceCount(&n) != hipSuccess || n <= 0) {
        (void)hipGetLastError();
        return fail(O3DR_ERR_NO_DEVICE, "no HIP device: libo3dr has no CPU path");
    }
    if (device_id < 0 || device_id >= n) return fail(O3DR_ERR_INVALID_ARG, "device_id out of range");
    if (hipSetDevice(device_id) != hipSuccess) return fail(O3DR_ERR_NO_DEVICE, "hipSetDevice failed");
    o3dr_ctx* c = new o3dr_ctx();
    c->device = device_id;
    o3dr_default_params(&c->params);
    if (hipStreamCreateWithFlags(&c->own_stream, hipStreamNonBlocking) != hipSuccess) {
        delete c;
        return fail(O3DR_ERR_NO_DEVICE, "hipStreamCreate failed");
    }
    c->stream = c->own_stream;
    if (hipMalloc((void**)&c->cloud_box, 6 * sizeof(float)) != hipSuccess ||
        hipMalloc((void**)&c->cc_big, sizeof(CloudCounters)) != hipSuccess ||
        hipMalloc((void**)&c->cc_tmp, sizeof(CloudCounters)) != hipSuccess ||
        hipHostMalloc((void**)&c->cc_host, 2 * sizeof(CloudCounters), hipHostMallocDefault) != hipSuccess ||
        hipHostMalloc((void**)&c->n_host, 4 * sizeof(uint32_t), hipHostMallocDefault) != hipSuccess ||
        hipHostMalloc((void**)&c->small_host, (size_t)kSmallMax * sizeof(o3dr_point), hipHostMallocDefault) != hipSuccess ||
        hipHostGetDevicePointer((void**)&c->cc_host_dev, c->cc_host, 0) != hipSuccess ||
        hipMalloc((void**)&c->stats_dev, sizeof(SortStats)) != hipSuccess ||
        hipMalloc((void**)&c->misc_dev, 4096) != hipSuccess ||
        hipHostMalloc((void**)&c->misc_host, 4096, hipHostMallocDefault) != hipSuccess ||
        hipHostMalloc((void**)&c->misc_host_lut, 256 * sizeof(QLutEntry), hipHostMallocDefault) != hipSuccess ||
        hipMalloc((void**)&c->q_lut, 256 * sizeof(QLutEntry)) != hipSuccess ||
        hipHostMalloc((void**)&c->stats_host, sizeof(SortStats), hipHostMallocDefault) != hipSuccess) {
        delete c;
        return fail(O3DR_ERR_ALLOC, "counter allocation failed");
    }
    (void)hipMemsetAsync(c->cc_big, 0, sizeof(CloudCounters), c->stream);
    (void)hipMemsetAsync(c->cc_tmp, 0, sizeof(CloudCounters), c->stream);
    (void)hipMemsetAsync(c->stats_dev, 0, sizeof(SortStats), c->stream);
    (void)hipMemsetAsync(c->misc_dev, 0, 4096, c->stream);
    const char* hb_env = getenv("O3DR_HOST_BATCH_FRAMES");
    if (hb_env && atoi(hb_env) > 0) c->host_batch = atoi(hb_env);
    const char* ru_env = getenv("O3DR_RUNS");
    if (ru_env && atoi(ru_env) == 0) c->use_runs = 0;
    else if (ru_env && atoi(ru_env) == 2) c->use_runs = 2;
    if (getenv("O3DR_NO_CLOUD_BOX")) c->cloud_box_enable = 0;
    const char* eb_env = getenv("O3DR_EXACT_BOX");
    c->exact_box = eb_env && atoi(eb_env) == 1;
    const char* sm_env = getenv("O3DR_SMALL");
    if (sm_env) c->small_path = atoi(sm_env) != 0;
    const char* th_env = getenv("O3DR_TEST_HOOKS");
    c->test_hooks = th_env && atoi(th_env) == 1;
    const char* sl_env = getenv("O3DR_SLABS");
    if (sl_env && sl_env[0] == '0') c->slab_shift_env = -1;
    else if (sl_env && sl_env[0] == 's' && atoi(sl_env + 1) >= 0 && atoi(sl_env + 1) <= 20) c->slab_shift_env = atoi(sl_env + 1);
    const char* env = getenv("O3DR_BATCH_FRAMES");
    if (env && atoi(env) > 0) c->max_batch = atoi(env) > 512 ? 512 : atoi(env);
    (void)cloud_box_clear(c);
    *out_ctx = c;
    return O3DR_OK;
}

extern "C" int o3dr_ctx_destroy(o3dr_ctx* c)
{
    if (!c) return O3DR_OK;
    (void)hipSetDevice(c->device);
    (void)hipStreamSynchronize(c->stream);
    dev_release(c->ws_block);
    dev_release(c->ws_pts_block);
    dev_release(c->ws_sor_block);
    dev_release(c->st_disp);
    dev_release(c->st_bgr);
    dev_release(c->st_in);
    dev_release(c->st_out);
    dev_release(c->st_kp);
    dev_release(c->st_kpoff);
    dev_release(c->st_poses);
    dev_release(c->st_xchg);
    dev_release(c->st_merge);
    dev_release(c->st_gather);
    if (c->xchg_host) (void)hipHostFree(c->xchg_host);
    dev_release(c->bil_tab);
    dev_release(c->st_blur);
    dev_release(c->st_blur_in);
    dev_release(c->st_hist);
    if (c->cloud_big) (void)hipFree(c->cloud_big);
    if (c->cloud_alt) (void)hipFree(c->cloud_alt);
    if (c->cloud_box) (void)hipFree(c->cloud_box);
    if (c->cloud_heads) (void)hipFree(c->cloud_heads);
    if (c->cc_big) (void)hipFree(c->cc_big);
    if (c->cc_tmp) (void)hipFree(c->cc_tmp);
    if (c->cc_host) (void)hipHostFree(c->cc_host);
    if (c->n_host) (void)hipHostFree(c->n_host);
    if (c->small_host) (void)hipHostFree(c->small_host);
    if (c->stats_dev) (void)hipFree(c->stats_dev);
    if (c->misc_dev) (void)hipFree(c->misc_dev);
    if (c->misc_host) (void)hipHostFree(c->misc_host);
    if (c->misc_host_lut) (void)hipHostFree(c->misc_host_lut);
    if (c->q_lut) (void)hipFree(c->q_lut);
    if (c->stats_host) (void)hipHostFree(c->stats_host);
    for (int i = 0; i < 2; ++i) {
        dev_release(c->st2_disp[i]);
        dev_release(c->st2_bgr[i]);
        dev_release(c->st2_poses[i]);
        if (c->ev_copied[i]) (void)hipEventDestroy(c->ev_copied[i]);
        if (c->ev_done[i]) (void)hipEventDestroy(c->ev_done[i]);
    }
    if (c->copy_stream) (void)hipStreamDestroy(c->copy_stream);
    if (c->own_stream) (void)hipStreamDestroy(c->own_stream);
    for (int i = 0; i < 2; ++i) {
        dev_release(c->inc.grp[i]);
        dev_release(c->inc.off[i]);
        dev_release(c->inc.cells[i]);
    }
    for (DevBuf* b : {&c->inc.box, &c->inc.scratch, &c->inc.tg, &c->inc.tmatch, &c->inc.flag, &c->inc.src, &c->inc.keep,
                      &c->inc.partial, &c->inc.words, &c->inc.fb, &c->nn_q, &c->nn_t, &c->nn_cells, &c->nn_src, &c->mls_out, &c->mls_misc,
                      &c->pl_pts, &c->pl_tiles, &c->pl_hyp, &c->pl_misc, &c->pl_out, &c->mt_desc, &c->mt_tab, &c->mt_part,
                      &c->mt_out, &c->rg_in, &c->rg_work})
        dev_release(*b);
    delete c;
    return O3DR_OK;
}

#define CTX_ENTER(c)                                                        \
    do {                                                                    \
        if (!(c)) return fail(O3DR_ERR_INVALID_ARG, "ctx is NULL");         \
        HIPCHK(hipSetDevice((c)->device));                                  \
    } while (0)

extern "C" int o3dr_ctx_set_stream(o3dr_ctx* c, void* hip_stream)
{
    CTX_ENTER(c);
    HIPCHK(hipStreamSynchronize(c->stream));
    c->stream = hip_stream ? (hipStream_t)hip_stream : c->own_stream;
    return O3DR_OK;
// ... 922 lines not shown
    const bool with_sor = sor_on(c) && !c->params.dont_downsample;
    int B = n_frames < c->max_batch ? n_frames : c->max_batch;
    {
        const int64_t per_frame = (with_sor ? 56 + 50 : 56) * cap + (1 << 20);
        const int64_t fit = ((int64_t)12 << 30) / per_frame;
        if (fit < B) B = fit < 1 ? 1 : (int)fit;
    }
    const bool streaming = mem == O3DR_MEM_HOST;
    if (streaming && c->host_batch < B) B = c->host_batch;
    CHK(ws_ensure(c, B, cap, true));
    if (with_sor) CHK(sor_ensure(c, B, cap));

    if (streaming) {
        if (!c->copy_stream) HIPCHK(hipStreamCreateWithFlags(&c->copy_stream, hipStreamNonBlocking));
        for (int i = 0; i < 2; ++i) {
            if (!c->ev_copied[i]) HIPCHK(hipEventCreateWithFlags(&c->ev_copied[i], hipEventDisableTiming));
            if (!c->ev_done[i]) HIPCHK(hipEventCreateWithFlags(&c->ev_done[i], hipEventDisableTiming));
        }
        HIPCHK(hipStreamSynchronize(c->stream));
    }
    int slot = 0;
    for (int f0 = 0; f0 < n_frames; f0 += B, slot ^= 1) {
        const int nb = (n_frames - f0) < B ? (n_frames - f0) : B;
        CHK(cloud_make_room(c, (int64_t)nb * cap));
        const void *disp_d, *bgr_d, *poses_d;
        if (streaming) {
            const size_t db = (size_t)nb * disp_frame_stride, cb = (size_t)nb * bgr_frame_stride, pb = (size_t)nb * 16 * sizeof(float);
            CHK(dev_ensure(c, c->st2_disp[slot], db));
            CHK(dev_ensure(c, c->st2_bgr[slot], cb));
            CHK(dev_ensure(c, c->st2_poses[slot], pb));
            if (f0 >= 2 * B) HIPCHK(hipStreamWaitEvent(c->copy_stream, c->ev_done[slot], 0));
            HIPCHK(hipMemcpyAsync(c->st2_disp[slot].p, disp + (int64_t)f0 * disp_frame_stride, db, hipMemcpyHostToDevice, c->copy_stream));
            HIPCHK(hipMemcpyAsync(c->st2_bgr[slot].p, bgr + (int64_t)f0 * bgr_frame_stride, cb, hipMemcpyHostToDevice, c->copy_stream));
            HIPCHK(hipMemcpyAsync(c->st2_poses[slot].p, poses + 16 * (int64_t)f0, pb, hipMemcpyHostToDevice, c->copy_stream));
            HIPCHK(hipEventRecord(c->ev_copied[slot], c->copy_stream));
            HIPCHK(hipStreamWaitEvent(c->stream, c->ev_copied[slot], 0));
            disp_d = c->st2_disp[slot].p;
            bgr_d = c->st2_bgr[slot].p;
            poses_d = c->st2_poses[slot].p;
        } else {
            disp_d = disp + (int64_t)f0 * disp_frame_stride;
            bgr_d = bgr + (int64_t)f0 * bgr_frame_stride;
            poses_d = poses + 16 * (int64_t)f0;
        }
        const uint8_t* dsp = (const uint8_t*)disp_d;
        int64_t dsp_pitch = disp_pitch, dsp_fstride = disp_frame_stride;
        CHK(maybe_blur(c, &dsp, &dsp_pitch, &dsp_fstride, rows, cols, nb));
        ReprojectArgs a;
        fill_args(c, a, dsp, dsp_pitch, dsp_fstride, (const uint8_t*)bgr_d, bgr_pitch,
                  bgr_frame_stride, rows, cols, g, cap);
        a.xf_mode = 2;
        a.poses = (const float*)poses_d;
        for (int i = 0; i < 3; ++i) a.slab_inv[i] = 1.0f / leaf[i];
        a.slab_shift = slab_shift_for(c, rows, cols, leaf);
        launch_minmax_init(&c->prof, c->stream, c->ws.mm, c->ws.mm_stride, a.n_tiles, c->ws.n_kp, nb);
        const bool fused = !use_kp && !c->params.dont_downsample && a.n_tiles > 0 && !with_sor;
        if (use_kp)
            launch_keypoint_pass(&c->prof, c->stream, a, kp_d, 0, c->ws.pts, c->ws.n_kp, c->ws.mm, kpoff_d + f0, nb);
        if (fused)
            launch_reproject_fused(&c->prof, c->stream, c->ws, a, nb, cap, leaf, !c->exact_box);
        else
            launch_reproject(&c->prof, c->stream, a, nb, c->ws.pts, c->ws.tile_cnt, c->ws.n_kp, c->ws.n_valid, c->ws.mm,
                             c->ws.scan_partial);
        VoxelArgs v;
        v.keys_ready = fused ? 1 : 0;
        v.cloud_box = c->cloud_box_valid ? c->cloud_box : nullptr;
        heads_for_append(c, v);
        v.in = c->ws.pts;
        v.in_fstride = cap;
        v.n_dev = c->ws.n_valid;
        v.frames = nb;
        v.cap = cap;
        v.leaf[0] = leaf[0];
        v.leaf[1] = leaf[1];
        v.leaf[2] = leaf[2];
        v.min_points = mp;
        v.z_offset = zo;
        v.out_base = c->cloud_big;
        v.cc = c->cc_big;
        v.passthrough = c->params.dont_downsample ? 1 : 0;
        v.mm_used = a.n_tiles + 1;
        v.stats = c->stats_dev;
        v.use_runs = 0;
        if (with_sor) {
            v.mm_used = launch_sor(&c->prof, c->stream, c->ws, c->ws.pts, cap, c->ws.n_valid, nb, cap, a.n_tiles + 1, 1.0, c->ws.sor_pts,
                                   cap, c->ws.sor_n);
            v.in = c->ws.sor_pts;
            v.n_dev = c->ws.sor_n;
        }
        launch_voxel_grid(&c->prof, c->stream, c->ws, v);
        HIPCHK(hipGetLastError());
        c->cloud_ub += (int64_t)nb * cap;
        c->cloud_n_exact = false;
        if (streaming) HIPCHK(hipEventRecord(c->ev_done[slot], c->stream));
    }
    if (streaming) HIPCHK(hipStreamSynchronize(c->stream));
    return O3DR_OK;
}

extern "C" int o3dr_accumulate_frames(o3dr_ctx* c, const uint8_t* disp, int64_t disp_frame_stride, int64_t disp_pitch,
                                      const uint8_t* bgr, int64_t bgr_frame_stride, int64_t bgr_pitch, int32_t rows,
                                      int32_t cols, const float* poses, int32_t n_frames, int32_t mem)
{
    return accumulate_impl(c, disp, disp_frame_stride, disp_pitch, bgr, bgr_frame_stride, bgr_pitch, rows, cols, poses, n_frames,
                           nullptr, nullptr, mem);
}
extern "C" int o3dr_accumulate_frames_kp(o3dr_ctx* c, const uint8_t* disp, int64_t disp_frame_stride, int64_t disp_pitch,
                                         const uint8_t* bgr, int64_t bgr_frame_stride, int64_t bgr_pitch, int32_t rows,
                                         int32_t cols, const float* poses, int32_t n_frames, const float* kp_xy,
                                         const int64_t* kp_offsets, int32_t mem)
{
    return accumulate_impl(c, disp, disp_frame_stride, disp_pitch, bgr, bgr_frame_stride, bgr_pitch, rows, cols, poses, n_frames,
                           kp_xy, kp_offsets, mem);
}

static int finalize_impl(o3dr_ctx* c, const float* gmin, const float* gmax, o3dr_point* out, int64_t out_capacity,
                         int64_t* n_out, uint32_t* status, int32_t mem)
{
    if (n_out) *n_out = 0;
    if (status) *status = 0;
    CTX_ENTER(c);
    if (!n_out) return fail(O3DR_ERR_INVALID_ARG, "n_out is NULL");
    if (mem != O3DR_MEM_HOST && mem != O3DR_MEM_DEVICE) return fail(O3DR_ERR_INVALID_ARG, "bad mem kind");
    CloudCounters cc;
    const bool known = c->cloud_n_exact && !c->params.dont_downsample && c->cloud_ub > 0;
    if (known) {
        cc.count = (uint64_t)c->cloud_ub;
        cc.status = 0;
    } else {
        CHK(read_counters(c, c->cc_big, &cc));
    }
    const int64_t n = (int64_t)cc.count;
    if (n == 0) return O3DR_OK;
    if (n >= (int64_t)0xffffffffLL) return fail(O3DR_ERR_INVALID_ARG, "cloud_big exceeds 2^32-1 points");
    if (!out) return fail(O3DR_ERR_INVALID_ARG, "out is NULL");
    if (c->params.dont_downsample) {
        if (n > out_capacity) return fail(O3DR_ERR_CAPACITY, "output buffer too small");
        return o3dr_cloud_big_read(c, out, out_capacity, n_out, mem);
    }
    float leaf[3], zo;
    uint32_t mp;
    downsample_leaf(c->params, 1, leaf, &mp, &zo);
    o3dr_point* out_d = out;
    if (mem == O3DR_MEM_HOST) {
        CHK(dev_ensure(c, c->st_out, (size_t)n * sizeof(o3dr_point)));
        out_d = (o3dr_point*)c->st_out.p;
    } else if (out_capacity < n) {
        return fail(O3DR_ERR_CAPACITY, "device output must hold cloud_big (overflow fallback returns the input)");
    }
    int64_t m = 0;
    uint32_t st = 0;
    CHK(voxel_single(c, c->cloud_big, n, leaf, mp, zo, out_d, &m, &st, gmin, gmax, false,
                     c->cloud_box_valid ? c->cloud_box : nullptr, heads_for_merge(c, leaf, zo), known ? &cc : nullptr));
    if ((int64_t)cc.count != n) return fail(O3DR_ERR_INTERNAL, "cloud_big's device count differs from the host's");
    if (mem == O3DR_MEM_HOST) {
        if (m > out_capacity) return fail(O3DR_ERR_CAPACITY, "output buffer too small");
        if (m > 0) {
            HIPCHK(hipMemcpyAsync(out, out_d, (size_t)m * sizeof(o3dr_point), hipMemcpyDeviceToHost, c->stream));
            HIPCHK(hipStreamSynchronize(c->stream));
        }
    }
    *n_out = m;
    if (status) *status = st | cc.status;
    return O3DR_OK;
}

// ... 1036 lines not shown
        char buf[256];
        snprintf(buf, sizeof buf, "hipHostRegister failed: %s", hipGetErrorString(e));
        return fail(O3DR_ERR_HIP, buf);
    }
    return O3DR_OK;
}
extern "C" int o3dr_host_unregister(void* ptr)
{
    if (!ptr) return O3DR_OK;
    const hipError_t e = hipHostUnregister(ptr);
    if (e != hipSuccess) {
        (void)hipGetLastError();
        char buf[256];
        snprintf(buf, sizeof buf, "hipHostUnregister failed: %s", hipGetErrorString(e));
        return fail(O3DR_ERR_HIP, buf);
    }
    return O3DR_OK;
}

extern "C" int o3dr_bilateral_filter_u8(o3dr_ctx* c, const uint8_t* src, int64_t src_pitch, int32_t rows, int32_t cols, int32_t d,
                                        double sigma_color, double sigma_space, uint8_t* dst, int64_t dst_pitch, int32_t mem)
{
    CTX_ENTER(c);
    if (mem != O3DR_MEM_HOST && mem != O3DR_MEM_DEVICE) return fail(O3DR_ERR_INVALID_ARG, "bad mem kind");
    if (rows < 0 || cols < 0) return fail(O3DR_ERR_INVALID_ARG, "negative image size");
    if (rows == 0 || cols == 0) return O3DR_OK;
    if (!src || !dst) return fail(O3DR_ERR_INVALID_ARG, "src / dst is NULL");
    if (src_pitch < cols || dst_pitch < cols) return fail(O3DR_ERR_INVALID_ARG, "pitch smaller than a row");
    CHK(bilateral_prepare(c, d, sigma_color, sigma_space));
    const uint8_t* src_d = src;
    uint8_t* dst_d = dst;
    if (mem == O3DR_MEM_HOST) {
        const void* p;
        CHK(stage_in(c, c->st_blur_in, src, (size_t)src_pitch * rows, mem, &p));
        src_d = (const uint8_t*)p;
        CHK(dev_ensure(c, c->st_blur, (size_t)dst_pitch * rows));
        dst_d = (uint8_t*)c->st_blur.p;
    }
    launch_bilateral(&c->prof, c->stream, src_d, src_pitch, 0, rows, cols, 1, c->bil_radius, c->bil_maxk,
                     (const float*)c->bil_tab.p, dst_d, dst_pitch, 0);
    HIPCHK(hipGetLastError());
    if (mem == O3DR_MEM_HOST) {
        HIPCHK(hipMemcpy2DAsync(dst, (size_t)dst_pitch, dst_d, (size_t)dst_pitch, (size_t)cols, (size_t)rows,
                                hipMemcpyDeviceToHost, c->stream));
        HIPCHK(hipStreamSynchronize(c->stream));
    }
    return O3DR_OK;
}

extern "C" int o3dr_disparity_variance(o3dr_ctx* c, const uint8_t* disp, int64_t disp_pitch, int64_t disp_frame_stride,
                                       int32_t rows, int32_t cols, int32_t n_frames, double* variance_out, int32_t mem)
{
    CTX_ENTER(c);
    if (mem != O3DR_MEM_HOST && mem != O3DR_MEM_DEVICE) return fail(O3DR_ERR_INVALID_ARG, "bad mem kind");
    if (n_frames < 0 || rows <= 0 || cols <= 0) return fail(O3DR_ERR_INVALID_ARG, "bad image size / frame count");
    if (n_frames == 0) return O3DR_OK;
    if (!disp || !variance_out) return fail(O3DR_ERR_INVALID_ARG, "disp / variance_out is NULL");
    if (disp_pitch < cols) return fail(O3DR_ERR_INVALID_ARG, "pitch smaller than a row");
    if (c->params.disparity_f64) return fail(O3DR_ERR_INVALID_ARG, "o3dr_disparity_variance takes CV_8UC1 images");
    if (n_frames > 1 && disp_frame_stride < (int64_t)rows * disp_pitch)
        return fail(O3DR_ERR_INVALID_ARG, "frame stride smaller than a frame");
    const GridShape g = grid_shape(c->params, rows, cols);
    const void* disp_d;
    CHK(stage_in(c, c->st_blur_in, disp, (size_t)disp_frame_stride * (n_frames - 1) + (size_t)disp_pitch * rows, mem, &disp_d));
    const size_t hist_bytes = sizeof(unsigned long long) * 256 * (size_t)n_frames;
    CHK(dev_ensure(c, c->st_hist, hist_bytes + sizeof(double) * (size_t)n_frames));
    unsigned long long* hist = (unsigned long long*)c->st_hist.p;
    double* var_d = (double*)((char*)c->st_hist.p + hist_bytes);
    launch_disp_variance(&c->prof, c->stream, (const uint8_t*)disp_d, disp_pitch, disp_frame_stride, rows, cols, n_frames,
                         c->params.bounding_box, g.cs, c->params.min_disparity, hist, var_d);
    HIPCHK(hipGetLastError());
    HIPCHK(hipMemcpyAsync(variance_out, var_d, sizeof(double) * (size_t)n_frames, hipMemcpyDeviceToHost, c->stream));
    HIPCHK(hipStreamSynchronize(c->stream));
    return O3DR_OK;
}

extern "C" int o3dr_test_corrupt_next_gather(o3dr_ctx* c)
{
    CTX_ENTER(c);
    if (!c->test_hooks) return fail(O3DR_ERR_INVALID_ARG, "test hooks are off (create the context with O3DR_TEST_HOOKS=1)");
    c->test_corrupt = 1;
    return O3DR_OK;
}

extern "C" int o3dr_test_sor_distances(o3dr_ctx* c, float* out, int64_t n)
{
    CTX_ENTER(c);
    if (!c->test_hooks) return fail(O3DR_ERR_INVALID_ARG, "test hooks are off (create the context with O3DR_TEST_HOOKS=1)");
    if (!out || n < 0 || n > c->ws_sor_cap || !c->ws.sor_dist) return fail(O3DR_ERR_INVALID_ARG, "no outlier removal of that size has run");
    if (n == 0) return O3DR_OK;
    HIPCHK(hipMemcpyAsync(out, c->ws.sor_dist, (size_t)n * sizeof(float), hipMemcpyDeviceToHost, c->stream));
    HIPCHK(hipStreamSynchronize(c->stream));
    return O3DR_OK;
}

extern "C" void o3dr_icp_default_params(o3dr_icp_params* p)
{
    if (!p) return;
    p->max_iterations = 10;
    p->max_correspondence_distance = HUGE_VAL;
    p->transformation_epsilon = 0.0;
}

static int nn_target(o3dr_ctx* c, const o3dr_point* target, int64_t n, int mem, float** box6, float4** cell_lo, float4** cell_hi)
{
    c->place_ub = -1;
    const void* t_d;
    CHK(stage_in(c, c->nn_t, target, (size_t)n * sizeof(o3dr_point), mem, &t_d));
    CHK(ws_ensure(c, 1, n, false));
    CHK(sor_ensure(c, 1, n));
    const size_t cell_bytes = align256(((size_t)c->ws.sor_max_cells + 1) * sizeof(float4));
    CHK(dev_ensure(c, c->nn_cells, 2 * cell_bytes + 256));
    char* base = (char*)c->nn_cells.p;
    *cell_lo = (float4*)base;
    *cell_hi = (float4*)(base + cell_bytes);
    *box6 = (float*)(base + 2 * cell_bytes);
    launch_set_counts(&c->prof, c->stream, c->ws.n_valid, (uint32_t)n, 1);
    const int used = launch_points_minmax(&c->prof, c->stream, (const o3dr_point*)t_d, 0, c->ws.n_valid, 1, n, c->ws.mm_stride, c->ws.mm);
    launch_nn_grid(&c->prof, c->stream, c->ws, (const o3dr_point*)t_d, n, used, *box6, *cell_lo, *cell_hi);
    HIPCHK(hipGetLastError());
    return O3DR_OK;
}

struct NnSrc {
    uint32_t* idx[2];
    float* d2;
    double* partial;
    double* rec;
};
static int nn_source(o3dr_ctx* c, int64_t n, NnSrc* o)
{
    const size_t b_idx = align256((size_t)n * 4), b_part = align256((size_t)kIcpRecord * (size_t)nn_partial_blocks(n) * 8);
    CHK(dev_ensure(c, c->nn_src, 3 * b_idx + b_part + align256(kIcpRecord * 8)));
    char* base = (char*)c->nn_src.p;
    o->idx[0] = (uint32_t*)base;
    o->idx[1] = (uint32_t*)(base + b_idx);
    o->d2 = (float*)(base + 2 * b_idx);
    o->partial = (double*)(base + 3 * b_idx);
    o->rec = (double*)(base + 3 * b_idx + b_part);
    return O3DR_OK;
}

static int nn_check_cloud(int64_t n, const void* p)
{
    if (n < 0 || (n > 0 && !p)) return fail(O3DR_ERR_INVALID_ARG, "bad arguments (cloud pointer / size)");
    if (n > (int64_t)0xffffffffLL) return fail(O3DR_ERR_INVALID_ARG, "more than 2^32-1 points in one cloud");
    return O3DR_OK;
}

extern "C" int o3dr_nearest_neighbors(o3dr_ctx* c, const o3dr_point* query, int64_t n_query, const o3dr_point* target,
                                      int64_t n_target, double max_distance, uint32_t* idx_out, float* d2_out, int32_t mem)
{
    if (mem == O3DR_MEM_HOST && n_query > 0 && n_query <= (int64_t)0xffffffffLL) {
        if (idx_out) memset(idx_out, 0, (size_t)n_query * sizeof(uint32_t));
        if (d2_out) memset(d2_out, 0, (size_t)n_query * sizeof(float));
    }
    CTX_ENTER(c);
    CHK(nn_check_cloud(n_query, query));
    CHK(nn_check_cloud(n_target, target));
    if (n_query > 0 && (!idx_out || !d2_out)) return fail(O3DR_ERR_INVALID_ARG, "idx_out / d2_out is NULL");
    if (!(max_distance >= 0.0)) return fail(O3DR_ERR_INVALID_ARG, "max_distance must be >= 0 (+inf: no limit)");
    if (mem != O3DR_MEM_HOST && mem != O3DR_MEM_DEVICE) return fail(O3DR_ERR_INVALID_ARG, "bad mem kind");
    c->place_ub = -1;
    if (n_query == 0) return O3DR_OK;
    const float r2 = (float)(max_distance * max_distance);
    NnSrc o;
// ... 788 lines not shown
```

### online_3d_reconstruction_amd/csrc/o3dr_device.h

```cpp
#pragma once
#include <hip/hip_runtime.h>
#include <stdint.h>

#include "../../include/o3dr.h"

namespace o3dr {

constexpr int kWave = 64;
constexpr int kEmitThreads = 256;
constexpr int kEmitPerLane = 4;
constexpr int kEmitTile = kEmitThreads * kEmitPerLane;
constexpr int kSortWaves = 8;
constexpr int kSortThreads = kSortWaves * kWave;
constexpr int kSortRounds = 16;
constexpr int kSortWaveItems = kSortRounds * kWave;
constexpr int kSortTile = kSortWaves * kSortWaveItems;
constexpr int kScatParts = 2;
constexpr int kScatWaves = kSortWaves / kScatParts;
constexpr int kScatThreads = kScatWaves * kWave;
constexpr int kScatTile = kScatWaves * kSortWaveItems;
constexpr int kMaxRadixBits = 7;
constexpr int kMaxRadix = 1 << kMaxRadixBits;
constexpr int kMaxPasses = 5;
static_assert(kMaxRadix <= 2 * kSortThreads, "k_radix_scatter handles two digits per thread");
constexpr int kSlabClasses = 4;
constexpr int kXcds = 8;
constexpr int kPtThreads = 256;
constexpr int kSegTile = 1024;
constexpr int kMinmaxBlocks = 1024;
constexpr int kSmallMax = 8192;
constexpr int kGroupBits = 5;
constexpr int kGroupCells = 1 << kGroupBits;
static_assert(kGroupCells <= kWave, "one lane per voxel of a group");
constexpr int kGroupWaves = 4;
constexpr int kGroupMinRunNum = 5, kGroupMinRunDen = 4;
constexpr int64_t kGroupMinCloud = 1 << 20;
constexpr int64_t kGroupMinSlots = 1 << 20;

struct VoxelGeom {
    float inv[3];
    int32_t min_b[3];
    int32_t div_b[3];
    uint32_t mul1, mul2;
    uint32_t overflow;
    uint32_t n;
    uint32_t passes;
    uint32_t bpp;
    uint32_t buf0;
    uint32_t grouped;
};

constexpr int kSorMeanK = 50;
#ifndef O3DR_SOR_CELLPTS
#define O3DR_SOR_CELLPTS 30.0
#endif
constexpr double kSorCellPoints = O3DR_SOR_CELLPTS;
struct SorGeom {
    float mnx, mny, inv_h, h;
    int32_t gx, gy;
    uint32_t n, active;
    double threshold;
};

struct QLutEntry {
    double alpha;
    float z, pad;
};

struct ReprojectArgs {
    const uint8_t* disp;
    const uint8_t* bgr;
    int64_t disp_pitch, bgr_pitch, disp_fstride, bgr_fstride;
    const float* poses;
    int32_t xf_mode;
    float T[12];
    int32_t rows, cols, bb, cs, jump;
    int32_t Ny, Nx;
    int32_t n_tiles;
    int32_t vec4;
    double Q[16];
    double min_disp;
    int32_t min_disp_u8;
    int64_t out_fstride;
    int64_t mm_stride;
    const QLutEntry* lut;
    int32_t disp_f64;
    float slab_inv[3];
    int32_t slab_shift;
};

struct Workspace {
    int32_t frames = 0;
    int64_t cap = 0;
    int32_t n_emit_tiles = 0, n_sort_tiles = 0, n_seg_tiles = 0;
    o3dr_point* pts = nullptr;
    uint32_t* keys[2] = {nullptr, nullptr};
    uint32_t* vals[2] = {nullptr, nullptr};
    uint32_t* seg_start = nullptr;
    uint32_t* tile_cnt = nullptr;
    uint32_t* hist = nullptr;
    uint32_t* hist_part = nullptr;
    uint32_t* seg_cnt = nullptr;
    uint8_t* head_bits = nullptr;
    uint32_t* scan_partial = nullptr;
    SorGeom* sor_geom = nullptr;
    float4* sor_xyz = nullptr;
    float* sor_dist = nullptr;
    uint32_t* sor_cell_first = nullptr;
    float2* sor_cell_z = nullptr;
    uint32_t sor_max_cells = 0;
    double* sor_partial = nullptr;
    o3dr_point* sor_pts = nullptr;
    uint32_t* sor_n = nullptr;
    uint32_t* sor_left = nullptr;
    uint32_t* sor_left_cnt = nullptr;
    int64_t sor_cap = 0;
    uint32_t* keep_idx = nullptr;
    uint32_t* run_start = nullptr;
    uint32_t* grp_cnt = nullptr;
    int64_t grp_slots = 0;
    uint32_t* n_runs = nullptr;
    uint32_t* n_grp_out = nullptr;
    VoxelGeom* geom_runs = nullptr;
    float* out_mm = nullptr;
    float* out_mm_partial = nullptr;
    int32_t* wave_gc = nullptr;
    float* mm = nullptr;
    int64_t mm_stride = 0;
    uint32_t* n_valid = nullptr;
    uint32_t* n_kp = nullptr;
    uint32_t* n_vox = nullptr;
    uint32_t* n_out = nullptr;
    uint64_t* out_off = nullptr;
    VoxelGeom* geom = nullptr;
    size_t bytes = 0;
};

struct SortStats {
    uint64_t sort_record_passes;
    uint64_t voxel_points_in;
    uint64_t voxel_points_out;
    uint64_t reserved;
    uint64_t sort_records;
    uint64_t pad[3];
};

struct CloudHeads {
    uint32_t* flags;
    float inv[3];
    float z_offset;
    int32_t* wave_gc;
};

struct CloudCounters {
    uint64_t count;
    uint32_t status;
    uint32_t pad;
};

struct IncGroup {
    int32_t bx, iy, iz;
    uint32_t mask;
};
struct IncCell {
    float s[7];
    uint32_t n;
};
static_assert(sizeof(IncCell) == 32, "32-byte cell records");

struct Profiler;

void launch_minmax_init(Profiler* pf, hipStream_t s, float* mm, int64_t mm_stride, int slot, uint32_t* n_kp, int frames);
void launch_keypoint_pass(Profiler* pf, hipStream_t s, const ReprojectArgs& a, const float* kp_xy, int n_kp,
                          o3dr_point* out, uint32_t* n_kp_out, float* mm, const int32_t* kp_off = nullptr, int frames = 1);
void launch_reproject(Profiler* pf, hipStream_t s, const ReprojectArgs& a, int frames, o3dr_point* out,
                      uint32_t* tile_cnt, const uint32_t* n_kp, uint32_t* n_valid, float* mm,
                      uint32_t* scan_partial);
void launch_reproject_fused(Profiler* pf, hipStream_t s, Workspace& ws, const ReprojectArgs& a, int frames, int64_t cap,
                            const float leaf[3], bool conservative_box = true);
void launch_transform(Profiler* pf, hipStream_t s, const o3dr_point* in, int64_t n, const float* T16_host,
                      o3dr_point* out);
int launch_points_minmax(Profiler* pf, hipStream_t s, const o3dr_point* in, int64_t in_fstride,
                         const uint32_t* n_dev, int frames, int64_t cap, int64_t mm_stride, float* mm);
struct VoxelArgs {
    const o3dr_point* in;
    int64_t in_fstride;
    const uint32_t* n_dev;
    int frames;
    int64_t cap;
    float leaf[3];
    uint32_t min_points;
    float z_offset;
    o3dr_point* out_base;
    CloudCounters* cc;
    int passthrough;
    int mm_used;
    SortStats* stats;
    int use_runs;
    float* cloud_box = nullptr;
    CloudHeads cloud_heads = {nullptr, {0.f, 0.f, 0.f}, 0.f, nullptr};
    const uint8_t* heads_in = nullptr;
    int keys_ready = 0;
    int test_corrupt = 0;
};
constexpr int kBoxFoldBlocks = 1024;
void launch_voxel_grid(Profiler* pf, hipStream_t s, Workspace& ws, const VoxelArgs& v);
void launch_set_counts(Profiler* pf, hipStream_t s, uint32_t* n_dev, uint32_t value, int frames);
void launch_small_frame(Profiler* pf, hipStream_t s, const ReprojectArgs& a, const float* kp_xy, int n_kp, int downsample,
                        const float leaf[3], o3dr_point* pts, o3dr_point* out, CloudCounters* cc, uint32_t* n_out_dev,
                        float* box_out6);
void launch_sor_small(Profiler* pf, hipStream_t s, Workspace& ws, const o3dr_point* in, const uint32_t* n_dev, int64_t cap,
                      double stddev_mul, o3dr_point* out, uint32_t* n_out_dev);
void launch_small_voxel(Profiler* pf, hipStream_t s, const o3dr_point* in, const uint32_t* n_in_dev, uint32_t n_in,
                        const float* box6, const float leaf[3], uint32_t min_points, float z_offset, o3dr_point* out,
                        CloudCounters* cc);
constexpr int kBilMaxRadius = 64;
void launch_bilateral(Profiler* pf, hipStream_t s, const uint8_t* src, int64_t src_pitch, int64_t src_fstride, int rows,
                      int cols, int frames, int radius, int maxk, const float* tab, uint8_t* dst, int64_t dst_pitch,
                      int64_t dst_fstride);
int bilateral_tile_width(int radius);
void launch_disp_variance(Profiler* pf, hipStream_t s, const uint8_t* disp, int64_t pitch, int64_t fstride, int rows, int cols,
                          int frames, int bb, int cs, double min_disp, unsigned long long* hist, double* var_out);
void launch_bbox(Profiler* pf, hipStream_t s, const float* mm, int used, float* out6);
int launch_sor(Profiler* pf, hipStream_t s, Workspace& ws, const o3dr_point* in, int64_t in_fstride, const uint32_t* n_dev,
               int frames, int64_t cap, int mm_used, double stddev_mul, o3dr_point* out, int64_t out_fstride,
               uint32_t* n_out_dev);
void launch_search_grid(Workspace& ws, hipStream_t s, const o3dr_point* in, int64_t in_fstride, const uint32_t* n_dev, int frames,
                        int64_t cap, int mm_used, double cell_points, uint32_t active_above);
constexpr int kIcpRecord = 18;
void launch_nn_grid(Profiler* pf, hipStream_t s, Workspace& ws, const o3dr_point* target, int64_t n, int mm_used, float* box6,
                    float4* cell_lo, float4* cell_hi);
void launch_nn_query(Profiler* pf, hipStream_t s, const Workspace& ws, const o3dr_point* query, int64_t n, const float* T12,
                     const float* box6, const float4* cell_lo, const float4* cell_hi, float r2, uint32_t* idx_out, float* d2_out,
                     const uint32_t* idx_prev, const double c0[3], double* partial, double* rec);
inline int64_t nn_partial_blocks(int64_t n) { return (n + 255) / 256; }
void launch_mls_finite(Profiler* pf, hipStream_t s, const o3dr_point* in, int64_t n, uint32_t* flag);
void launch_mls(Profiler* pf, hipStream_t s, const Workspace& ws, const o3dr_point* cloud, int64_t n, const float* box6,
                const float4* cell_lo, const float4* cell_hi, double r, int order, double h, o3dr_point* out, float* normals,
                uint32_t* nn_count, uint8_t* fit, unsigned long long* counters);
struct MatchPair {
    uint32_t qbase, nq, tbase, nt;
    uint32_t chunks;
    uint32_t qwaves;
    uint64_t item0;
    uint64_t rec0;
    uint64_t part0;
};
struct MatchArgs {
    const uint4* desc;
    uint32_t n_pairs;
    uint32_t chunk_rows;
    uint64_t n_items, n_rec;
    uint4* rec;
    uint8_t* good;
    float ratio;
    uint32_t max_distance;
};
constexpr uint32_t kMatchMaxChunk = 1u << 23;
constexpr int64_t kMatchSliceItems = 1 << 24;
void launch_match(Profiler* pf, hipStream_t s, const MatchArgs& a, const MatchPair* pairs, uint2* partial);
void launch_keypoints_3d(Profiler* pf, hipStream_t s, const ReprojectArgs& a, const float* kp_xy, const int32_t* kp_off, int n_frames,
                         int n_kp, o3dr_point* out);
constexpr int kRigidPoints = 256;
constexpr int kRigidFields = 16;
struct RigidSeg {
    uint64_t start;
    uint32_t n;
    uint32_t block0;
};
struct RigidArgs {
    const o3dr_point* src;
    const o3dr_point* tgt;
    const uint8_t* mask;
    const RigidSeg* seg;
    uint32_t n_segs, n_blocks;
    uint32_t* first;
    double* partial;
    double* rec;
    double* c0;
    const double* T;
};
void launch_rigid(Profiler* pf, hipStream_t s, const RigidArgs& a, bool residual);
struct PlaneArgs {
    const float4* pts;
    const o3dr_point* cloud;
    int tiled;
// ... 64 lines not shown
```

### online_3d_reconstruction_amd/csrc/o3dr_kernels.hip

```cpp
#include <string.h>

#include "o3dr_device.h"
#include "o3dr_profile.h"

namespace o3dr {

#include "kernels/util.inc"
#include "kernels/reproject.inc"
#include "kernels/bookkeeping.inc"
#include "kernels/prepass.inc"
#include "kernels/voxel_index.inc"
#include "kernels/radix_sort.inc"
#include "kernels/voxel_runs.inc"
#include "kernels/incremental.inc"
#include "kernels/multigpu.inc"
#include "kernels/sor.inc"
#include "kernels/small.inc"
#include "kernels/nn.inc"
#include "kernels/mls.inc"
#include "kernels/plane.inc"
#include "kernels/match.inc"

static inline int cdiv64(int64_t a, int64_t b) { return (int)((a + b - 1) / b); }

// ... 117 lines not shown
    {
        ProfScope ps(pf, O3DR_K_REPROJECT, s);
        if (a.disp_f64)
            k_reproject_emit<true, false><<<grid, kEmitThreads, 0, s>>>(a, out, tile_cnt, n_kp, mm, nullptr, 0, nullptr);
        else
            k_reproject_emit<false, false><<<grid, kEmitThreads, 0, s>>>(a, out, tile_cnt, n_kp, mm, nullptr, 0, nullptr);
    }
}

static inline int xcd_grid(int64_t n) { return (int)((n + kXcds - 1) / kXcds * kXcds); }
void launch_reproject_fused(Profiler* pf, hipStream_t s, Workspace& ws, const ReprojectArgs& a, int frames, int64_t cap,
                            const float leaf[3], bool conservative_box)
{
    const dim3 grid(a.n_tiles, frames);
    const bool cbox = a.lut != nullptr && !a.disp_f64 && conservative_box;
    const dim3 cgrid(cdiv64(a.n_tiles, kCountTiles), frames);
    {
        ProfScope ps(pf, O3DR_K_COUNT, s);
        if (cbox)
            k_reproject_count_cbox<kCboxTiles><<<dim3(cdiv64(a.n_tiles, kCboxTiles), frames), kEmitThreads, 0, s>>>(a, ws.tile_cnt, ws.mm);
        else if (a.disp_f64)
            k_reproject_bbox_count<true><<<cgrid, kEmitThreads, 0, s>>>(a, ws.tile_cnt, ws.mm, nullptr);
        else
            k_reproject_bbox_count<false><<<cgrid, kEmitThreads, 0, s>>>(a, ws.tile_cnt, ws.mm, nullptr);
    }
    {
        ProfScope ps(pf, O3DR_K_OTHER, s);
        launch_scan(s, ws.tile_cnt, a.n_tiles, a.n_tiles, frames, ws.n_valid, ws.n_kp, ws.scan_partial);
        k_voxel_geom<<<frames, 256, 0, s>>>(ws.mm, ws.mm_stride, a.n_tiles + 1, ws.n_valid, leaf[0], leaf[1], leaf[2], 0.f, ws.geom);
    }
    if (cbox) {
        ProfScope ps(pf, O3DR_K_COUNT, s);
        k_reproject_bbox_count<false><<<cgrid, kEmitThreads, 0, s>>>(a, ws.tile_cnt, ws.mm, ws.geom);
        k_voxel_geom<<<frames, 256, 0, s>>>(ws.mm, ws.mm_stride, a.n_tiles + 1, ws.n_valid, leaf[0], leaf[1], leaf[2], 0.f, ws.geom, 1);
    }
    {
        ProfScope ps(pf, O3DR_K_REPROJECT, s);
        if (a.disp_f64)
            k_reproject_emit<true, true><<<grid, kEmitThreads, 0, s>>>(a, ws.pts, ws.tile_cnt, ws.n_kp, ws.mm, ws.geom, cap, ws.keys[0]);
        else
            k_reproject_emit<false, true><<<grid, kEmitThreads, 0, s>>>(a, ws.pts, ws.tile_cnt, ws.n_kp, ws.mm, ws.geom, cap, ws.keys[0]);
    }
}

void launch_transform(Profiler* pf, hipStream_t s, const o3dr_point* in, int64_t n, const float* T16_host,
                      o3dr_point* out)
{
    if (n <= 0) return;
    Mat34 T;
    for (int i = 0; i < 12; ++i) T.m[i] = T16_host[i];
    ProfScope ps(pf, O3DR_K_OTHER, s);
    k_transform<<<cdiv64(n, kPtThreads), kPtThreads, 0, s>>>(in, n, T, out);
}

int launch_points_minmax(Profiler* pf, hipStream_t s, const o3dr_point* in, int64_t in_fstride,
                         const uint32_t* n_dev, int frames, int64_t cap, int64_t mm_stride, float* mm)
{
    if (cap <= 0) return 0;
    int nblk = cdiv64(cap, kPtThreads * 4);
    if (nblk > kMinmaxBlocks) nblk = kMinmaxBlocks;
    ProfScope ps(pf, O3DR_K_OTHER, s);
    k_points_minmax<<<dim3(nblk, frames), kPtThreads, 0, s>>>(in, in_fstride, n_dev, mm_stride, mm);
    return nblk;
}

void launch_voxel_grid(Profiler* pf, hipStream_t s, Workspace& ws, const VoxelArgs& v)
{
    const int F = v.frames;
    const int64_t cap = v.cap;
    const int n_sort_tiles = cdiv64(cap, kSortTile);
    const int n_seg_tiles = cdiv64(cap, kSegTile);
    const size_t tm_lds = (size_t)n_sort_tiles * (kMaxRadix + 1) * sizeof(uint32_t);
    const int tm = tm_lds <= 48 * 1024 ? 1 : 0;
    if (!v.keys_ready) {
        ProfScope ps(pf, O3DR_K_OTHER, s);
        k_voxel_geom<<<F, 256, 0, s>>>(ws.mm, ws.mm_stride, v.mm_used, v.n_dev, v.leaf[0], v.leaf[1], v.leaf[2],
                                       v.z_offset, ws.geom);
    }
    uint32_t* n_keep = nullptr;
    const bool use_runs = v.use_runs && !v.passthrough && F == 1 && v.in != ws.pts && (v.use_runs > 1 || cap >= kGroupMinCloud);
    const int64_t grp_slots = use_runs ? ws.grp_slots : 0;
    const int64_t max_groups = grp_slots / kGroupCells;
    const VoxelGeom* sort_geom = use_runs ? ws.geom_runs : ws.geom;
    if (!v.passthrough && cap > 0) {
        const dim3 grid(n_sort_tiles, F);
        if (use_runs) {
            const uint8_t* hb = v.heads_in ? v.heads_in : ws.head_bits;
            {
                ProfScope ps(pf, O3DR_K_KEYGEN, s);
                if (v.heads_in)
                    k_head_counts<<<cdiv64(n_seg_tiles, 4), 256, 0, s>>>(v.heads_in, ws.geom, n_seg_tiles, ws.seg_cnt);
                else
                    k_group_heads<<<n_seg_tiles, 256, 0, s>>>(v.in, ws.geom, v.z_offset, n_seg_tiles, ws.seg_cnt, ws.head_bits);
            }
            {
                ProfScope ps(pf, O3DR_K_OTHER, s);
                launch_scan(s, ws.seg_cnt, n_seg_tiles, n_seg_tiles, F, ws.n_runs, nullptr, ws.scan_partial);
            }
            {
                ProfScope ps(pf, O3DR_K_SEGMENT, s);
                k_run_geom<<<cdiv64(F, 64), 64, 0, s>>>(ws.geom, ws.n_runs, F, ws.geom_runs, v.use_runs > 1 ? 1 : 0, grp_slots);
                k_run_starts<<<dim3(cdiv64(n_seg_tiles, kStartWaves), F), kStartWaves * kWave, 0, s>>>(
                    ws.keys[0], ws.keys[1], cap, ws.geom, n_seg_tiles, ws.seg_cnt, ws.n_runs, ws.run_start, 0, ws.keys[1],
                    ws.geom_runs, v.in, v.z_offset, hb);
            }
            {
                ProfScope ps(pf, O3DR_K_KEYGEN, s);
                k_voxel_keys_hist0<<<grid, kSortThreads, 0, s>>>(v.in, v.in_fstride, ws.geom, v.z_offset, cap, ws.keys[0],
                                                                 n_sort_tiles, ws.hist, ws.hist_part, ws.geom_runs, tm);
            }
        } else if (!v.keys_ready) {
            ProfScope ps(pf, O3DR_K_KEYGEN, s);
            k_voxel_keys_hist0<<<grid, kSortThreads, 0, s>>>(v.in, v.in_fstride, ws.geom, v.z_offset, cap, ws.keys[0],
                                                             n_sort_tiles, ws.hist, ws.hist_part, nullptr, tm);
        }
        const int64_t hist_row = (int64_t)kMaxRadix * n_sort_tiles;

        for (int pass = 0; pass < kMaxPasses; ++pass) {
            if (!(pass == 0 && !use_runs && !v.keys_ready)) {
                ProfScope ps(pf, O3DR_K_SORT_HIST, s);
                k_radix_hist<<<grid, kSortThreads, 0, s>>>(ws.keys[0], ws.keys[1], cap, sort_geom, pass, n_sort_tiles,
                                                          ws.hist, ws.hist_part, tm);
            }
            {
                ProfScope ps(pf, O3DR_K_OTHER, s);
                if (tm)
                    k_scan_hist_tm<<<F, 1024, tm_lds, s>>>(ws.hist, sort_geom, pass, n_sort_tiles);
                else
                    launch_scan(s, ws.hist, hist_row, hist_row, F, nullptr, nullptr, ws.scan_partial, sort_geom, pass,
                                n_sort_tiles);
            }
            {
                ProfScope ps(pf, O3DR_K_SORT_SCATTER, s);
                k_radix_scatter_lane<<<dim3(xcd_grid((int64_t)n_sort_tiles * kScatParts), F), kScatThreads, 0, s>>>(
                    ws.keys[0], ws.vals[0], ws.keys[1], ws.vals[1], cap, sort_geom, pass, n_sort_tiles, ws.hist, ws.hist_part, tm);
            }
        }
        const dim3 sgrid(n_seg_tiles, F);
        {
            ProfScope ps(pf, O3DR_K_SEGMENT, s);
            k_run_heads<<<dim3(cdiv64(n_seg_tiles, kHeadWaves), F), kHeadWaves * kWave, 0, s>>>(ws.keys[0], ws.keys[1], cap, sort_geom, n_seg_tiles,
                                                                                       ws.seg_cnt, -1, ws.head_bits);
        }
        {
            ProfScope ps(pf, O3DR_K_OTHER, s);
            launch_scan(s, ws.seg_cnt, n_seg_tiles, n_seg_tiles, F, ws.n_vox, nullptr, ws.scan_partial);
        }
        {
            ProfScope ps(pf, O3DR_K_SEGMENT, s);
            k_run_starts<<<dim3(cdiv64(n_seg_tiles, kStartWaves), F), kStartWaves * kWave, 0, s>>>(ws.keys[0], ws.keys[1], cap, sort_geom, n_seg_tiles, ws.seg_cnt, ws.n_vox,
                                              ws.seg_start, -1, nullptr, nullptr, nullptr, 0.f, ws.head_bits);
        }
        if (v.min_points > 1) {
            {
                ProfScope ps(pf, O3DR_K_SEGMENT, s);
                k_keep_count<<<sgrid, 256, 0, s>>>(ws.seg_start, cap, sort_geom, ws.n_vox, v.min_points, n_seg_tiles, ws.seg_cnt);
            }
            {
                ProfScope ps(pf, O3DR_K_OTHER, s);
                launch_scan(s, ws.seg_cnt, n_seg_tiles, n_seg_tiles, F, ws.n_out, nullptr, ws.scan_partial);
            }
            {
                ProfScope ps(pf, O3DR_K_SEGMENT, s);
                k_keep_write<<<sgrid, 256, 0, s>>>(ws.seg_start, cap, sort_geom, ws.n_vox, v.min_points, n_seg_tiles, ws.seg_cnt,
                                                  ws.keep_idx);
            }
            n_keep = ws.n_out;
        }
    }
    if (v.test_corrupt && cap > 0 && !v.passthrough)
        k_test_corrupt_payload<<<1, 1, 0, s>>>(ws.vals[0], ws.vals[1], sort_geom);
    if (cap > 0 && use_runs) {
        {
            ProfScope ps(pf, O3DR_K_OTHER, s);
            (void)hipMemsetAsync(ws.grp_cnt, 0, sizeof(uint32_t) * (size_t)(max_groups + 1), s);
        }
        {
            ProfScope ps(pf, O3DR_K_CENTROID_RUNS, s);
            int64_t nwg = cdiv64(max_groups < cap ? max_groups : cap, kGroupWaves);
            if (nwg > 16384) nwg = 16384;
            if (nwg < 1) nwg = 1;
            k_centroid_groups<<<(int)nwg, kGroupWaves * kWave, 0, s>>>(
                v.in, ws.keys[0], ws.keys[1], ws.vals[0], ws.vals[1], ws.seg_start, ws.run_start, ws.geom_runs, ws.geom, ws.n_vox,
                v.z_offset, v.min_points, reinterpret_cast<uint4*>(ws.pts), grp_slots, ws.grp_cnt, v.cc);
        }
        {
            ProfScope ps(pf, O3DR_K_OTHER, s);
            launch_scan(s, ws.grp_cnt, max_groups + 1, max_groups + 1, 1, ws.n_grp_out, nullptr, ws.scan_partial);
        }
    }
    {
        ProfScope ps(pf, O3DR_K_OTHER, s);
        k_frame_offsets<<<1, 256, 0, s>>>(ws.geom, ws.n_vox, n_keep, use_runs ? ws.n_grp_out : nullptr, F, v.passthrough,
                                          ws.n_out, ws.out_off, v.cc, v.stats, sort_geom);
    }
    const int nbx = cdiv64(cap, kPtThreads);
    if (cap > 0 && use_runs) {
        ProfScope ps(pf, O3DR_K_CENTROID_RUNS, s);
        int64_t nwg = cdiv64(cap, 256);
        if (nwg > 8192) nwg = 8192;
        k_group_compact<<<(int)nwg, 256, 0, s>>>(v.in, ws.geom_runs, ws.geom, ws.n_vox, ws.grp_cnt,
                                                reinterpret_cast<const uint4*>(ws.pts), ws.out_off, v.z_offset, v.out_base);
    }
    if (cap > 0) {
        ProfScope ps(pf, O3DR_K_CENTROID, s);
        float* out_mm = v.cloud_box ? ws.out_mm : nullptr;
        CloudHeads heads = v.cloud_heads;
        heads.wave_gc = ws.wave_gc;
        const uint32_t* keep = (v.min_points > 1 && !v.passthrough) ? ws.keep_idx : nullptr;
        if (use_runs)
            k_centroid<true><<<dim3(nbx < 4096 ? nbx : 4096, F), kPtThreads, 0, s>>>(
                v.in, v.in_fstride, ws.vals[0], ws.vals[1], cap, ws.seg_start, keep, ws.geom_runs, ws.n_out, ws.out_off,
                v.z_offset, v.passthrough, v.out_base, out_mm, nbx, v.cc, CloudHeads{nullptr, {0.f, 0.f, 0.f}, 0.f, nullptr});
        else
            k_centroid<false><<<dim3(xcd_grid(nbx), F), kPtThreads, 0, s>>>(
                v.in, v.in_fstride, ws.vals[0], ws.vals[1], cap, ws.seg_start, keep, ws.geom, ws.n_out, ws.out_off,
                v.z_offset, v.passthrough, v.out_base, out_mm, nbx, v.cc, heads);
        if (!use_runs && v.cloud_heads.flags) {
            const int wpf = nbx * (kPtThreads / 64);
            k_cloud_heads_fix<<<dim3(cdiv64(wpf, 256), F), 256, 0, s>>>(ws.n_out, ws.out_off, wpf, heads);
        }
    }
    if (v.cloud_box && cap > 0 && !use_runs) {
        ProfScope ps(pf, O3DR_K_OTHER, s);
        const int nbx = cdiv64(cap, kPtThreads) * (kPtThreads / 64);
        k_cloud_bbox_fold<<<kBoxFoldBlocks, 256, 0, s>>>(ws.out_mm, nbx, F, ws.n_out, ws.out_mm_partial);
        k_cloud_bbox_merge<<<1, 384, 0, s>>>(ws.out_mm_partial, kBoxFoldBlocks, v.cloud_box);
    }
}

void launch_inc_runs(Profiler* pf, hipStream_t s, Workspace& ws, const o3dr_point* in, int64_t n, const float leaf[3], float z_offset,
                     const uint8_t* rec_heads, int64_t first, int test_corrupt)
{
    const int64_t cap = n;
    const int n_sort_tiles = cdiv64(cap, kSortTile);
    const int n_seg_tiles = cdiv64(cap, kSegTile);
    const size_t tm_lds = (size_t)n_sort_tiles * (kMaxRadix + 1) * sizeof(uint32_t);
    const int tm = tm_lds <= 48 * 1024 ? 1 : 0;
    const VoxelGeom* sort_geom = ws.geom_runs;
    {
        ProfScope ps(pf, O3DR_K_OTHER, s);
        k_voxel_geom<<<1, 256, 0, s>>>(ws.mm, ws.mm_stride, 1, ws.n_valid, leaf[0], leaf[1], leaf[2], z_offset, ws.geom);
    }
    {
        ProfScope ps(pf, O3DR_K_KEYGEN, s);
        if (rec_heads) {
            const int64_t bytes = (int64_t)n_seg_tiles * 256;
            k_inc_heads_shift<<<cdiv64(bytes, 256), 256, 0, s>>>(rec_heads, (uint64_t)first, (uint64_t)n, ws.head_bits, (uint64_t)bytes);
            k_head_counts<<<cdiv64(n_seg_tiles, 4), 256, 0, s>>>(ws.head_bits, ws.geom, n_seg_tiles, ws.seg_cnt);
        } else {
            k_group_heads<<<n_seg_tiles, 256, 0, s>>>(in, ws.geom, z_offset, n_seg_tiles, ws.seg_cnt, ws.head_bits);
        }
    }
    {
        ProfScope ps(pf, O3DR_K_OTHER, s);
        launch_scan(s, ws.seg_cnt, n_seg_tiles, n_seg_tiles, 1, ws.n_runs, nullptr, ws.scan_partial);
    }
    {
        ProfScope ps(pf, O3DR_K_SEGMENT, s);
        k_run_geom<<<1, 64, 0, s>>>(ws.geom, ws.n_runs, 1, ws.geom_runs, 1, INT64_MAX);
        k_run_starts<<<dim3(cdiv64(n_seg_tiles, kStartWaves), 1), kStartWaves * kWave, 0, s>>>(
            ws.keys[0], ws.keys[1], cap, ws.geom, n_seg_tiles, ws.seg_cnt, ws.n_runs, ws.run_start, 0, ws.keys[1], ws.geom_runs, in,
            z_offset, ws.head_bits);
    }
    const dim3 grid(n_sort_tiles, 1);
    const int64_t hist_row = (int64_t)kMaxRadix * n_sort_tiles;
    for (int pass = 0; pass < kMaxPasses; ++pass) {
        {
            ProfScope ps(pf, O3DR_K_SORT_HIST, s);
            k_radix_hist<<<grid, kSortThreads, 0, s>>>(ws.keys[0], ws.keys[1], cap, sort_geom, pass, n_sort_tiles, ws.hist, ws.hist_part, tm);
        }
        {
            ProfScope ps(pf, O3DR_K_OTHER, s);
            if (tm)
                k_scan_hist_tm<<<1, 1024, tm_lds, s>>>(ws.hist, sort_geom, pass, n_sort_tiles);
            else
                launch_scan(s, ws.hist, hist_row, hist_row, 1, nullptr, nullptr, ws.scan_partial, sort_geom, pass, n_sort_tiles);
        }
        {
            ProfScope ps(pf, O3DR_K_SORT_SCATTER, s);
            k_radix_scatter_lane<<<dim3(xcd_grid((int64_t)n_sort_tiles * kScatParts), 1), kScatThreads, 0, s>>>(
                ws.keys[0], ws.vals[0], ws.keys[1], ws.vals[1], cap, sort_geom, pass, n_sort_tiles, ws.hist, ws.hist_part, tm);
        }
    }
    {
        ProfScope ps(pf, O3DR_K_SEGMENT, s);
        k_run_heads<<<dim3(cdiv64(n_seg_tiles, kHeadWaves), 1), kHeadWaves * kWave, 0, s>>>(ws.keys[0], ws.keys[1], cap, sort_geom,
                                                                                             n_seg_tiles, ws.seg_cnt, -1, ws.head_bits);
    }
    {
        ProfScope ps(pf, O3DR_K_OTHER, s);
        launch_scan(s, ws.seg_cnt, n_seg_tiles, n_seg_tiles, 1, ws.n_vox, nullptr, ws.scan_partial);
    }
    {
        ProfScope ps(pf, O3DR_K_SEGMENT, s);
        k_run_starts<<<dim3(cdiv64(n_seg_tiles, kStartWaves), 1), kStartWaves * kWave, 0, s>>>(
            ws.keys[0], ws.keys[1], cap, sort_geom, n_seg_tiles, ws.seg_cnt, ws.n_vox, ws.seg_start, -1, nullptr, nullptr, nullptr, 0.f,
            ws.head_bits);
    }
    if (test_corrupt) k_test_corrupt_payload<<<1, 1, 0, s>>>(ws.vals[0], ws.vals[1], sort_geom);
}

void launch_inc_fold(Profiler* pf, hipStream_t s, Workspace& ws, const o3dr_point* in, float z_offset, const IncFoldArgs& a,
                     uint32_t* partial)
{
    {
        ProfScope ps(pf, O3DR_K_CENTROID_RUNS, s);
        int64_t nwg = cdiv64(a.nt, kGroupWaves);
        if (nwg > 16384) nwg = 16384;
        if (nwg < 1) nwg = 1;
        k_inc_fold<<<(int)nwg, kGroupWaves * kWave, 0, s>>>(in, ws.keys[0], ws.keys[1], ws.vals[0], ws.vals[1], ws.seg_start, ws.run_start,
                                                            ws.geom_runs, ws.geom, ws.n_vox, z_offset, a.old_g, a.old_off, a.old_cells,
                                                            a.n_old, a.n_old_cells, a.scratch, a.nt, a.tg, a.tmatch, a.cc);
    }
    ProfScope ps(pf, O3DR_K_OTHER, s);
    k_inc_new_flags<<<cdiv64((int64_t)a.nt + 1, 256), 256, 0, s>>>(a.tmatch, a.nt, a.flag);
    launch_scan(s, a.flag, (int64_t)a.nt + 1, (int64_t)a.nt + 1, 1, a.n_new_only, nullptr, partial);
}

void launch_inc_place(Profiler* pf, hipStream_t s, const IncFoldArgs& a, uint32_t n_new, IncGroup* new_g, uint32_t* src,
                      uint32_t* new_off, uint32_t* n_cells_dev, uint32_t* partial)
{
    ProfScope ps(pf, O3DR_K_OTHER, s);
    (void)hipMemsetAsync(new_off, 0, sizeof(uint32_t) * ((size_t)n_new + 1), s);
    if (a.n_old > 0)
        k_inc_place_old<<<cdiv64(a.n_old, 256), 256, 0, s>>>(a.old_g, a.n_old, a.tg, a.tmatch, a.nt, a.flag, new_g, src, new_off, n_new, a.cc);
    if (a.nt > 0)
        k_inc_place_new<<<cdiv64(a.nt, 256), 256, 0, s>>>(a.old_g, a.n_old, a.tg, a.tmatch, a.nt, a.flag, new_g, src, new_off, n_new, a.cc);
    launch_scan(s, new_off, (int64_t)n_new + 1, (int64_t)n_new + 1, 1, n_cells_dev, nullptr, partial);
}

void launch_inc_copy(Profiler* pf, hipStream_t s, const IncFoldArgs& a, const IncGroup* new_g, const uint32_t* new_off,
                     const uint32_t* src, uint32_t n_new, IncCell* cells, uint32_t cells_cap)
{
    if (n_new == 0) return;
    ProfScope ps(pf, O3DR_K_OTHER, s);
    k_inc_copy<<<cdiv64((int64_t)n_new * kGroupCells, 256), 256, 0, s>>>(new_g, new_off, src, n_new, a.old_off, a.old_cells, a.n_old,
                                                                         a.n_old_cells, a.scratch, a.nt, cells, cells_cap, a.cc);
}

void launch_inc_keep(Profiler* pf, hipStream_t s, const IncGroup* grp, const uint32_t* off, const IncCell* cells, uint32_t n_groups,
                     uint32_t n_cells, uint32_t need, uint32_t* keep_cnt, uint32_t* n_keep_dev, uint32_t* partial)
{
    ProfScope ps(pf, O3DR_K_OTHER, s);
    (void)hipMemsetAsync(keep_cnt + n_groups, 0, sizeof(uint32_t), s);
    if (n_groups > 0) k_inc_keep_count<<<cdiv64(n_groups, 4), 256, 0, s>>>(grp, off, cells, n_groups, n_cells, need, keep_cnt);
    launch_scan(s, keep_cnt, (int64_t)n_groups + 1, (int64_t)n_groups + 1, 1, n_keep_dev, nullptr, partial);
}

void launch_inc_snapshot(Profiler* pf, hipStream_t s, const IncGroup* grp, const uint32_t* off, const IncCell* cells, uint32_t n_groups,
                         uint32_t n_cells, uint32_t need, const uint32_t* out_off, float z_offset, o3dr_point* out, uint32_t out_cap,
                         CloudCounters* cc)
{
    if (n_groups == 0) return;
    ProfScope ps(pf, O3DR_K_CENTROID, s);
    k_inc_snapshot<<<cdiv64(n_groups, 4), 256, 0, s>>>(grp, off, cells, n_groups, n_cells, need, out_off, z_offset,
                                                       reinterpret_cast<uint4*>(out), out_cap, cc);
}

void launch_inc_box_fold(hipStream_t s, float* box6, const float* tail6, float* mm6) { k_inc_box_fold<<<1, 64, 0, s>>>(box6, tail6, mm6); }

void launch_bilateral(Profiler* pf, hipStream_t s, const uint8_t* src, int64_t src_pitch, int64_t src_fstride, int rows,
                      int cols, int frames, int radius, int maxk, const float* tab, uint8_t* dst, int64_t dst_pitch,
                      int64_t dst_fstride)
{
    if (rows <= 0 || cols <= 0 || frames <= 0) return;
    const int tiles_x = cdiv64(cols, kBilTX), tiles_y = cdiv64(rows, kBilTY);
    const size_t lds = 1024 + (size_t)(kBilTX + 2 * radius) * (kBilTY + 2 * radius);
    ProfScope ps(pf, O3DR_K_OTHER, s);
    k_bilateral_u8<<<dim3(tiles_x * tiles_y, frames), 256, lds, s>>>(src, src_pitch, src_fstride, rows, cols, radius, maxk, tab,
                                                                    dst, dst_pitch, dst_fstride, tiles_x);
}
int bilateral_tile_width(int radius) { return kBilTX + 2 * radius; }

void launch_disp_variance(Profiler* pf, hipStream_t s, const uint8_t* disp, int64_t pitch, int64_t fstride, int rows, int cols,
                          int frames, int bb, int cs, double min_disp, unsigned long long* hist, double* var_out)
{
    ProfScope ps(pf, O3DR_K_OTHER, s);
    (void)hipMemsetAsync(hist, 0, sizeof(unsigned long long) * 256 * (size_t)frames, s);
    const int roi_rows = rows - 2 * bb;
    if (roi_rows > 0) k_disp_hist<<<dim3(roi_rows, frames), 256, 0, s>>>(disp, pitch, fstride, rows, cols, bb, cs, min_disp, hist);
    k_disp_variance<<<cdiv64(frames, 64), 64, 0, s>>>(hist, frames, rows, cols, bb, cs, var_out);
}

void launch_bbox(Profiler* pf, hipStream_t s, const float* mm, int used, float* out6)
{
    ProfScope ps(pf, O3DR_K_OTHER, s);
    k_bbox_fold<<<1, 256, 0, s>>>(mm, used, out6);
}

void launch_pack_header(hipStream_t s, const float* box6_dev, const CloudCounters* cc, void* hdr32_dev)
{
    k_pack_header<<<1, 1, 0, s>>>(box6_dev, cc, reinterpret_cast<CloudHeader*>(hdr32_dev));
}
void launch_count_from_cc(hipStream_t s, const CloudCounters* cc, uint32_t* n_dev) { k_count_from_cc<<<1, 1, 0, s>>>(cc, n_dev); }
void launch_set_cloud_count(hipStream_t s, CloudCounters* cc, uint64_t n) { k_set_cloud_count<<<1, 1, 0, s>>>(cc, n); }

void launch_partition_count(Profiler* pf, hipStream_t s, Workspace& ws, const VoxelArgs& v, int n_parts, uint64_t* counts_dev,
                            uint32_t* overflow_dev, const void* hdrs_dev, int n_hdrs)
{
    const int64_t cap = v.cap;
    const int n_sort_tiles = cdiv64(cap, kSortTile);
    const int64_t hist_row = (int64_t)kMaxRadix * n_sort_tiles;
    ProfScope ps(pf, O3DR_K_OTHER, s);
    if (hdrs_dev) k_fold_headers<<<1, 1, 0, s>>>(reinterpret_cast<const CloudHeader*>(hdrs_dev), n_hdrs, ws.mm);
    k_voxel_geom<<<1, 256, 0, s>>>(ws.mm, ws.mm_stride, 1, v.n_dev, v.leaf[0], v.leaf[1], v.leaf[2], v.z_offset, ws.geom);
    k_part_plan<<<1, 1, 0, s>>>(ws.geom, n_parts);
    k_part_count<<<n_sort_tiles, kSortThreads, 0, s>>>(v.in, ws.geom, v.z_offset, n_parts, n_sort_tiles, ws.hist);
    launch_scan(s, ws.hist, hist_row, hist_row, 1, nullptr, nullptr, ws.scan_partial, ws.geom, 0, n_sort_tiles);
    k_part_counts_scanned<<<cdiv64(n_parts, 64), 64, 0, s>>>(ws.hist, ws.geom, n_parts, n_sort_tiles, counts_dev, overflow_dev);
}
void launch_partition_move(Profiler* pf, hipStream_t s, Workspace& ws, const VoxelArgs& v, int n_parts, o3dr_point* out,
                           const int64_t* part_shift_dev)
{
    ProfScope ps(pf, O3DR_K_OTHER, s);
    const int n_sort_tiles = cdiv64(v.cap, kSortTile);
    k_part_move<<<n_sort_tiles, kSortThreads, 0, s>>>(v.in, ws.geom, v.z_offset, n_parts, n_sort_tiles, ws.hist, out, part_shift_dev);
}
void launch_partition(Profiler* pf, hipStream_t s, Workspace& ws, const VoxelArgs& v, int n_parts, o3dr_point* out,
                      uint64_t* counts_dev, uint32_t* overflow_dev, const void* hdrs_dev, int n_hdrs)
{
    launch_partition_count(pf, s, ws, v, n_parts, counts_dev, overflow_dev, hdrs_dev, n_hdrs);
    launch_partition_move(pf, s, ws, v, n_parts, out, nullptr);
}

static void launch_radix_passes(Workspace& ws, hipStream_t s, int64_t cap, int passes, int frames = 1)
{
    const int F = frames;
    const int n_sort_tiles = cdiv64(cap, kSortTile);
    const int64_t hist_row = (int64_t)kMaxRadix * n_sort_tiles;
    const size_t tm_lds = (size_t)n_sort_tiles * (kMaxRadix + 1) * sizeof(uint32_t);
    const int tm = tm_lds <= 48 * 1024 ? 1 : 0;
    for (int pass = 0; pass < passes && pass < kMaxPasses; ++pass) {
        k_radix_hist<<<dim3(n_sort_tiles, F), kSortThreads, 0, s>>>(ws.keys[0], ws.keys[1], cap, ws.geom, pass, n_sort_tiles, ws.hist,
                                                                    ws.hist_part, tm);
        if (tm)
            k_scan_hist_tm<<<F, 1024, tm_lds, s>>>(ws.hist, ws.geom, pass, n_sort_tiles);
        else
            launch_scan(s, ws.hist, hist_row, hist_row, F, nullptr, nullptr, ws.scan_partial, ws.geom, pass, n_sort_tiles);
        k_radix_scatter_lane<<<dim3(xcd_grid((int64_t)n_sort_tiles * kScatParts), F), kScatThreads, 0, s>>>(
            ws.keys[0], ws.vals[0], ws.keys[1], ws.vals[1], cap, ws.geom, pass, n_sort_tiles, ws.hist, ws.hist_part, tm);
    }
}

void launch_search_grid(Workspace& ws, hipStream_t s, const o3dr_point* in, int64_t in_fstride, const uint32_t* n_dev, int frames,
                        int64_t cap, int mm_used, double cell_points, uint32_t active_above)
{
    const int F = frames;
    const int64_t cell_stride = (int64_t)ws.sor_max_cells + 1;
    uint32_t max_cells = (uint32_t)(cap / 2 > 1024 ? cap / 2 : 1024);
    if (max_cells > ws.sor_max_cells) max_cells = ws.sor_max_cells;
    int cell_bits = 1;
    while ((1u << cell_bits) < max_cells) ++cell_bits;
    const int sort_passes = (cell_bits + kMaxRadixBits - 1) / kMaxRadixBits;
    k_sor_plan<<<F, 256, 0, s>>>(ws.mm, ws.mm_stride, mm_used, n_dev, max_cells, ws.sor_geom, ws.geom, cell_points, active_above);
    (void)hipMemsetAsync(ws.sor_cell_first, 0, (size_t)F * (size_t)cell_stride * 4, s);
    k_sor_cells<<<dim3(cdiv64(cap, 256), F), 256, 0, s>>>(in, in_fstride, ws.sor_geom, cap, ws.keys[0]);
    launch_radix_passes(ws, s, cap, sort_passes, F);
    k_sor_cell_counts<<<dim3(cdiv64(cap, 256), F), 256, 0, s>>>(ws.keys[0], ws.keys[1], ws.geom, ws.sor_geom, cap, cell_stride, ws.sor_cell_first);
    launch_scan(s, ws.sor_cell_first, cell_stride, cell_stride, F, nullptr, nullptr, ws.scan_partial);
    k_sor_gather<<<dim3(cdiv64(cap, 256), F), 256, 0, s>>>(in, in_fstride, ws.vals[0], ws.vals[1], ws.sor_geom, ws.geom, cap, ws.sor_xyz);
}

int launch_sor(Profiler* pf, hipStream_t s, Workspace& ws, const o3dr_point* in, int64_t in_fstride, const uint32_t* n_dev,
               int frames, int64_t cap, int mm_used, double stddev_mul, o3dr_point* out, int64_t out_fstride,
               uint32_t* n_out_dev)
{
    ProfScope ps(pf, O3DR_K_OTHER, s);
    const int F = frames;
    const int n_tiles = cdiv64(cap, 1024);
    const int64_t cell_stride = (int64_t)ws.sor_max_cells + 1;
    launch_search_grid(ws, s, in, in_fstride, n_dev, F, cap, mm_used, kSorCellPoints, (uint32_t)kSorMeanK);
    (void)hipMemsetAsync(ws.sor_left_cnt, 0, (size_t)F * 4, s);
    k_sor_knn<<<dim3(cdiv64(cap, kWave), F), kWave, 0, s>>>(ws.sor_xyz, ws.vals[0], ws.vals[1], ws.geom, ws.sor_cell_first, cell_stride,
                                                           ws.sor_geom, cap, ws.sor_dist, ws.sor_left, ws.sor_left_cnt);
    {
        int lg = cdiv64(cap, kWave * kSorLeftWaves);
        if (lg > 1024) lg = 1024;
        int zg = cdiv64((int64_t)ws.sor_max_cells, 256);
        if (zg > 256) zg = 256;
        k_sor_cell_z<<<dim3(zg, F), 256, 0, s>>>(ws.sor_xyz, ws.sor_cell_first, cell_stride, ws.sor_geom, cap, ws.sor_left_cnt, ws.sor_cell_z);
        k_sor_knn_left<<<dim3(lg, F), kSorLeftWaves * kWave, 0, s>>>(ws.sor_xyz, ws.vals[0], ws.vals[1], ws.geom, ws.sor_cell_first, cell_stride,
                                                                    ws.sor_geom, cap, ws.sor_dist, ws.sor_left, ws.sor_left_cnt, ws.sor_cell_z);
    }
    k_sor_partial<<<dim3(kSorStatBlocks, F), 256, 0, s>>>(ws.sor_dist, cap, ws.sor_geom, ws.sor_partial);
    k_sor_threshold<<<cdiv64(F, 64), 64, 0, s>>>(ws.sor_partial, stddev_mul, ws.sor_geom, F);
    k_sor_count<<<dim3(n_tiles, F), 256, 0, s>>>(ws.sor_dist, cap, ws.sor_geom, n_tiles, ws.tile_cnt);
    launch_scan(s, ws.tile_cnt, n_tiles, n_tiles, F, n_out_dev, nullptr, ws.scan_partial);
    k_sor_emit<<<dim3(n_tiles, F), 256, 0, s>>>(in, in_fstride, ws.sor_dist, cap, ws.sor_geom, n_tiles, ws.tile_cnt, out, out_fstride,
                                                ws.mm_stride, ws.mm);
    return n_tiles;
}

void launch_nn_grid(Profiler* pf, hipStream_t s, Workspace& ws, const o3dr_point* target, int64_t n, int mm_used, float* box6,
                    float4* cell_lo, float4* cell_hi)
{
    ProfScope ps(pf, O3DR_K_OTHER, s);
    k_bbox_fold<<<1, 256, 0, s>>>(ws.mm, mm_used, box6);
    launch_search_grid(ws, s, target, 0, ws.n_valid, 1, n, mm_used, kNnCellPoints, 0u);
    int cg = cdiv64((int64_t)ws.sor_max_cells, 256);
    if (cg > 4096) cg = 4096;
    k_nn_cell_box<<<cg, 256, 0, s>>>(ws.sor_xyz, ws.sor_cell_first, ws.sor_geom, cell_lo, cell_hi);
}

void launch_nn_query(Profiler* pf, hipStream_t s, const Workspace& ws, const o3dr_point* query, int64_t n, const float* T12,
                     const float* box6, const float4* cell_lo, const float4* cell_hi, float r2, uint32_t* idx_out, float* d2_out,
                     const uint32_t* idx_prev, const double c0[3], double* partial, double* rec)
{
    if (n <= 0) return;
    ProfScope ps(pf, O3DR_K_OTHER, s);
    NnArgs a;
    memset(&a, 0, sizeof a);
    a.query = query;
    a.n = (uint32_t)n;
    a.xf = T12 ? 1 : 0;
    for (int k = 0; k < 12; ++k) a.T.m[k] = T12 ? T12[k] : 0.f;
    a.txyz = ws.sor_xyz;
    a.cell_first = ws.sor_cell_first;
    a.cell_lo = cell_lo;
    a.cell_hi = cell_hi;
    a.sg = ws.sor_geom;
    a.box6 = box6;
    a.r2 = r2;
    a.idx_out = idx_out;
// ... 163 lines not shown
```

Measured before the change: 34230 frames/s.

## Fuse last radix pass with voxel segmentation and centroid sums

During the final radix pass the histogram kernel now also counts distinct voxel keys per digit bucket. A new scatter-with-sums kernel then writes voxel centroids straight from the last scatter, skipping the separate run-heads, run-starts and centroid passes for eligible frames (more than one pass, not grouped). This removes a full pass over the sorted keys and payloads plus several launches. In exchange it adds backward scans in first_of_key, extra LDS histograms and a heads-fix kernel.

```diff
diff --git a/include/o3dr_testing.h b/include/o3dr_testing.h
--- a/include/o3dr_testing.h
+++ b/include/o3dr_testing.h
@@ -6,6 +6,8 @@
 #endif
 
 int o3dr_test_corrupt_next_gather(o3dr_ctx* ctx);
+
+int o3dr_test_corrupt_next_batch(o3dr_ctx* ctx);
 
 int o3dr_test_sor_distances(o3dr_ctx* ctx, float* out, int64_t n);
 
diff --git a/online_3d_reconstruction_amd/_lib.py b/online_3d_reconstruction_amd/_lib.py
--- a/online_3d_reconstruction_amd/_lib.py
+++ b/online_3d_reconstruction_amd/_lib.py
@@ -157,6 +157,7 @@
     ("o3dr_profile_reset", C.c_int, [_vp]),
     ("o3dr_profile_stats", C.c_int, [_vp, _pi64]),
     ("o3dr_test_corrupt_next_gather", C.c_int, [_vp]),
+    ("o3dr_test_corrupt_next_batch", C.c_int, [_vp]),
     ("o3dr_test_sor_distances", C.c_int, [_vp, _vp, _i64]),
     ("o3dr_test_local_comm_create", C.c_int, [_i32, C.POINTER(_vp)]),
     ("o3dr_test_local_comm_destroy", C.c_int, [_vp]),
diff --git a/online_3d_reconstruction_amd/csrc/kernels/bookkeeping.inc b/online_3d_reconstruction_amd/csrc/kernels/bookkeeping.inc
--- a/online_3d_reconstruction_amd/csrc/kernels/bookkeeping.inc
+++ b/online_3d_reconstruction_amd/csrc/kernels/bookkeeping.inc
@@ -14,12 +14,16 @@
     if (i < frames) n_dev[i] = value;
 }
 
+__device__ __forceinline__ bool scan_row_live(const VoxelGeom& g, int pass)
+{
+    return !g.overflow && (pass < 0 ? fused_frame(g) : pass < (int)g.passes);
+}
 __device__ __forceinline__ int64_t scan_row_len(const VoxelGeom* __restrict__ geom, int f, int pass, int n_tiles,
                                                 int64_t L)
 {
     if (!geom) return L;
     const VoxelGeom g = geom[f];
-    if (g.overflow || pass >= (int)g.passes) return 0;
+    if (!scan_row_live(g, pass)) return 0;
     return (int64_t)geom_bins(g) * n_tiles;
 }
 __device__ __forceinline__ int scan_live_tiles(const VoxelGeom* __restrict__ geom, int f, int n_tiles)
@@ -66,13 +70,13 @@
 }
 
 __global__ __launch_bounds__(1024) void k_scan_hist_tm(uint32_t* __restrict__ hist, const VoxelGeom* __restrict__ geom, int pass,
-                                                       int n_tiles)
+                                                       int n_tiles, uint32_t* __restrict__ totals)
 {
     extern __shared__ uint32_t tm_row[];
     __shared__ uint32_t lds[1024 / 64 + 1];
     const int f = blockIdx.x;
     const VoxelGeom g = geom[f];
-    if (g.overflow || pass >= (int)g.passes) return;
+    if (!scan_row_live(g, pass)) return;
     const int bins = geom_bins(g);
     uint32_t* row = hist + (int64_t)f * kMaxRadix * n_tiles;
     const int words = n_tiles * kMaxRadix;
@@ -93,6 +97,7 @@
     }
     uint32_t total;
     uint32_t run = block_excl_scan_u32<16>(s, lds, total);
+    if (totals && threadIdx.x == 0) totals[f] = total;
     {
         int d = b / n_tiles, t = b - d * n_tiles;
         for (int i = b; i < e; ++i) {
diff --git a/online_3d_reconstruction_amd/csrc/kernels/radix_sort.inc b/online_3d_reconstruction_amd/csrc/kernels/radix_sort.inc
--- a/online_3d_reconstruction_amd/csrc/kernels/radix_sort.inc
+++ b/online_3d_reconstruction_amd/csrc/kernels/radix_sort.inc
@@ -4,11 +4,25 @@
     return tm ? (int64_t)tile * kMaxRadix + dgt : (int64_t)dgt * n_tiles + tile;
 }
 
+__device__ __forceinline__ bool first_of_key(const uint32_t* __restrict__ src, int64_t i, uint32_t k, uint32_t prev, uint32_t lomask)
+{
+    if (i == 0 || ((prev ^ k) & lomask) != 0u) return true;
+    if (prev == k) return false;
+    for (int64_t j = i - 2; j >= 0; --j) {
+        const uint32_t kj = src[j];
+        if (((kj ^ k) & lomask) != 0u) return true;
+        if (kj == k) return false;
+    }
+    return true;
+}
+
+template <bool kVox>
 __global__ __launch_bounds__(kSortThreads) void k_radix_hist(const uint32_t* __restrict__ keys0,
                                                              const uint32_t* __restrict__ keys1, int64_t cap,
                                                              const VoxelGeom* __restrict__ geom, int pass,
                                                              int n_tiles, uint32_t* __restrict__ hist,
-                                                             uint32_t* __restrict__ hist_part, int tm)
+                                                             uint32_t* __restrict__ hist_part, int tm,
+                                                             uint32_t* __restrict__ vhist, uint32_t* __restrict__ vhist_part)
 {
     constexpr int kSub = 4;
     __shared__ uint32_t h[kSub * kSortWaves * kMaxRadix];
@@ -24,6 +38,17 @@
     const uint32_t* src = (((pass + g.buf0) & 1) ? keys1 : keys0) + (int64_t)f * cap;
     const int64_t base = (int64_t)tile * kSortTile;
     uint32_t* hw = h + (((threadIdx.x >> 6) * kSub) + (threadIdx.x & (kSub - 1))) * kMaxRadix;
+    __shared__ uint32_t hv[kVox ? kSub * kSortWaves * kMaxRadix : 1];
+    const bool vox = kVox && fused_frame(g) && pass == (int)g.passes - 1;
+    const uint32_t lomask = (1u << shift) - 1u;
+    uint32_t* hvw = hv + (kVox ? (((threadIdx.x >> 6) * kSub) + (threadIdx.x & (kSub - 1))) * kMaxRadix : 0);
+    if (kVox) {
+        for (int i = threadIdx.x; i < kSub * kSortWaves * kMaxRadix; i += kSortThreads) hv[i] = 0;
+        __syncthreads();
+    }
+    auto count_vox = [&](int64_t i, uint32_t k, uint32_t prev) {
+        if (first_of_key(src, i, k, prev, lomask)) atomicAdd(&hvw[(k >> shift) & dmask], 1u);
+    };
     if (base < n) {
         const bool vec = (((int64_t)f * cap) & 3) == 0;
         static_assert(kScatParts == 2 && kSortRounds / 4 == 4, "the first scatter part is rounds 0 and 1");
@@ -45,6 +70,12 @@
 #pragma unroll
                     for (int ww = 0; ww < kSub * kSortWaves; ++ww) t += h[ww * kMaxRadix + dgt];
                     hist_part[(int64_t)f * kMaxRadix * n_tiles + hist_at(tm != 0, dgt, tile, n_tiles)] = t;
+                    if (vox) {
+                        uint32_t c = 0;
+#pragma unroll
+                        for (int ww = 0; ww < kSub * kSortWaves; ++ww) c += hv[ww * kMaxRadix + dgt];
+                        vhist_part[(int64_t)f * kMaxRadix * n_tiles + hist_at(tm != 0, dgt, tile, n_tiles)] = c;
+                    }
                 }
                 __syncthreads();
             }
@@ -53,9 +84,19 @@
                 atomicAdd(&hw[(v[r].y >> shift) & dmask], 1u);
                 atomicAdd(&hw[(v[r].z >> shift) & dmask], 1u);
                 atomicAdd(&hw[(v[r].w >> shift) & dmask], 1u);
+                if (vox) {
+                    count_vox(i, v[r].x, i > 0 ? src[i - 1] : 0u);
+                    count_vox(i + 1, v[r].y, v[r].x);
+                    count_vox(i + 2, v[r].z, v[r].y);
+                    count_vox(i + 3, v[r].w, v[r].z);
+                }
             } else {
                 for (int k = 0; k < 4; ++k)
-                    if (i + k < n) atomicAdd(&hw[(src[i + k] >> shift) & dmask], 1u);
+                    if (i + k < n) {
+                        const uint32_t key = src[i + k];
+                        atomicAdd(&hw[(key >> shift) & dmask], 1u);
+                        if (vox) count_vox(i + k, key, i + k > 0 ? src[i + k - 1] : 0u);
+                    }
             }
         }
     }
@@ -66,6 +107,12 @@
 #pragma unroll
         for (int ww = 0; ww < kSub * kSortWaves; ++ww) t += h[ww * kMaxRadix + dgt];
         dst[hist_at(tm != 0, dgt, tile, n_tiles)] = t;
+        if (vox) {
+            uint32_t c = 0;
+#pragma unroll
+            for (int ww = 0; ww < kSub * kSortWaves; ++ww) c += hv[ww * kMaxRadix + dgt];
+            vhist[(int64_t)f * kMaxRadix * n_tiles + hist_at(tm != 0, dgt, tile, n_tiles)] = c;
+        }
     }
 }
 
@@ -181,8 +228,8 @@
     }
 }
 
-__device__ __forceinline__ void scatter_tile(const ScatterJob& J, int tile, int part, ScatterLds& L, const uint32_t (&key)[kSortRounds],
-                                             const uint32_t (&val)[kSortRounds], uint32_t gstart)
+__device__ __forceinline__ uint32_t scatter_stage(const ScatterJob& J, int tile, int part, ScatterLds& L, const uint32_t (&key)[kSortRounds],
+                                                 const uint32_t (&val)[kSortRounds], uint32_t gstart)
 {
     uint32_t* smem = L.smem;
     uint32_t* stage = L.smem;
@@ -266,6 +313,17 @@
         }
     }
     __syncthreads();
+    return cnt;
+}
+
+__device__ __forceinline__ void scatter_tile(const ScatterJob& J, int tile, int part, ScatterLds& L, const uint32_t (&key)[kSortRounds],
+                                             const uint32_t (&val)[kSortRounds], uint32_t gstart)
+{
+    const uint32_t cnt = scatter_stage(J, tile, part, L, key, val, gstart);
+    const uint32_t* stage = L.smem;
+    const uint32_t* stage_v = L.smem + kScatTile;
+    const int shift = J.shift;
+    const uint32_t dmask = J.dmask;
 #pragma unroll
     for (int r = 0; r < kSortRounds; ++r) {
         const uint32_t p = r * kScatThreads + threadIdx.x;
@@ -282,12 +340,13 @@
                                                                      uint32_t* __restrict__ keys1, uint32_t* __restrict__ vals1,
                                                                      int64_t cap, const VoxelGeom* __restrict__ geom, int pass,
                                                                      int n_tiles, const uint32_t* __restrict__ hist_scanned,
-                                                                     const uint32_t* __restrict__ hist_part, int tm)
+                                                                     const uint32_t* __restrict__ hist_part, int tm, int fused)
 {
     __shared__ ScatterLds L;
     const int f = blockIdx.y;
     const VoxelGeom g = geom[f];
     if (g.overflow || pass >= (int)g.passes) return;
+    if (fused && fused_frame(g) && pass == (int)g.passes - 1) return;
     const int item = xcd_chunk_item(blockIdx.x, (int)(((int64_t)g.n + kScatTile - 1) / kScatTile));
     if (item < 0) return;
     const int tile = item / kScatParts, part = item % kScatParts;
diff --git a/online_3d_reconstruction_amd/csrc/kernels/util.inc b/online_3d_reconstruction_amd/csrc/kernels/util.inc
--- a/online_3d_reconstruction_amd/csrc/kernels/util.inc
+++ b/online_3d_reconstruction_amd/csrc/kernels/util.inc
@@ -129,6 +129,10 @@
     const uint32_t bpp = g.bpp < (uint32_t)kMaxRadixBits ? g.bpp : (uint32_t)kMaxRadixBits;
     return 1 << bpp;
 }
+__device__ __forceinline__ bool fused_frame(const VoxelGeom& g)
+{
+    return !g.overflow && g.passes >= 2u && g.grouped == 0u && g.n > 0u;
+}
 __device__ __forceinline__ uint32_t voxel_key_of(const uint4 v, const VoxelGeom& g, float z_offset)
 {
     const float x = __uint_as_float(v.x), y = __uint_as_float(v.y), z = __uint_as_float(v.z) + z_offset;
diff --git a/online_3d_reconstruction_amd/csrc/kernels/voxel_runs.inc b/online_3d_reconstruction_amd/csrc/kernels/voxel_runs.inc
--- a/online_3d_reconstruction_amd/csrc/kernels/voxel_runs.inc
+++ b/online_3d_reconstruction_amd/csrc/kernels/voxel_runs.inc
@@ -4,13 +4,14 @@
 __global__ __launch_bounds__(kHeadWaves * kWave) void k_run_heads(const uint32_t* __restrict__ keys0, const uint32_t* __restrict__ keys1,
                                                                   int64_t cap, const VoxelGeom* __restrict__ geom, int n_tiles,
                                                                   uint32_t* __restrict__ seg_cnt, int buf_sel,
-                                                                  uint8_t* __restrict__ head_bits)
+                                                                  uint8_t* __restrict__ head_bits, int fused)
 {
     static_assert(kSegTile == 16 * kWave, "16 records per lane");
     const int f = blockIdx.y, lane = threadIdx.x & 63;
     const int tile = blockIdx.x * kHeadWaves + (threadIdx.x >> 6);
     const VoxelGeom g = geom[f];
     if (g.overflow || tile >= n_tiles) return;
+    if (fused && fused_frame(g)) return;
     const int64_t n = g.n;
     const uint32_t* k = (buf_sel < 0 ? sorted_buf(g, keys0, keys1) : (buf_sel ? keys1 : keys0)) + (int64_t)f * cap;
     uint32_t c = 0;
@@ -47,13 +48,14 @@
     const uint32_t* __restrict__ keys0, const uint32_t* __restrict__ keys1, int64_t cap, const VoxelGeom* __restrict__ geom,
     int n_tiles, const uint32_t* __restrict__ seg_off, const uint32_t* __restrict__ n_vox, uint32_t* __restrict__ seg_start,
     int buf_sel, uint32_t* __restrict__ head_keys_out, const VoxelGeom* __restrict__ mode, const o3dr_point* __restrict__ in_pts,
-    float z_offset, const uint8_t* __restrict__ head_bits)
+    float z_offset, const uint8_t* __restrict__ head_bits, int fused)
 {
     static_assert(kSegTile == 16 * kWave, "16 records per lane");
     const int f = blockIdx.y, lane = threadIdx.x & 63;
     const int tile = blockIdx.x * kStartWaves + (threadIdx.x >> 6);
     const VoxelGeom g = geom[f];
     if (g.overflow) return;
+    if (fused && fused_frame(g)) return;
     if (mode && mode[f].grouped == 0u) return;
     const uint32_t n = g.n;
     const int64_t base = (int64_t)tile * kSegTile;
@@ -144,7 +146,7 @@
                                                        const uint32_t* __restrict__ n_grp, int frames, int passthrough,
                                                        uint32_t* __restrict__ n_out, uint64_t* __restrict__ out_off,
                                                        CloudCounters* __restrict__ cc, SortStats* __restrict__ stats,
-                                                       const VoxelGeom* __restrict__ sort_geom)
+                                                       const VoxelGeom* __restrict__ sort_geom, const uint32_t* __restrict__ n_vox_fused)
 {
     __shared__ uint32_t scan_lds[5];
     __shared__ unsigned long long acc[6];
@@ -164,6 +166,7 @@
                 atomicOr(&acc[3], (unsigned long long)O3DR_STATUS_VOXEL_OVERFLOW);
             } else {
                 m = (n_grp && sort_geom[f].grouped) ? n_grp[f] : (n_keep ? n_keep[f] : n_vox[f]);
+                if (n_vox_fused && fused_frame(g)) m = n_vox_fused[f];
                 atomicAdd(&acc[0], (unsigned long long)sort_geom[f].n * g.passes);
                 atomicAdd(&acc[5], (unsigned long long)sort_geom[f].n);
                 atomicAdd(&acc[1], (unsigned long long)g.n);
@@ -191,11 +194,13 @@
     }
 }
 
-__global__ void k_test_corrupt_payload(uint32_t* __restrict__ vals0, uint32_t* __restrict__ vals1, const VoxelGeom* __restrict__ geom)
+__global__ void k_test_corrupt_payload(uint32_t* __restrict__ vals0, uint32_t* __restrict__ vals1, const VoxelGeom* __restrict__ geom,
+                                       int fused)
 {
     const VoxelGeom g = geom[0];
     if (g.overflow || g.n == 0u) return;
-    uint32_t* v = ((g.passes + g.buf0) & 1u) ? vals1 : vals0;
+    const uint32_t last = (fused && fused_frame(g)) ? g.passes - 1u : g.passes;
+    uint32_t* v = ((last + g.buf0) & 1u) ? vals1 : vals0;
     v[g.n / 2u] = 0xfffffff0u;
 }
 
@@ -316,11 +321,11 @@
                                                          const uint64_t* __restrict__ out_off, float z_offset,
                                                          int passthrough, o3dr_point* __restrict__ out_base,
                                                          float* __restrict__ out_mm, int nbx, CloudCounters* __restrict__ cc,
-                                                         CloudHeads ch)
+                                                         CloudHeads ch, int fused)
 {
     const int f = blockIdx.y;
     const VoxelGeom g = geom[f];
-    if (!passthrough && (g.n == 0 || g.grouped != 0u)) return;
+    if (!passthrough && (g.n == 0 || g.grouped != 0u || (fused && fused_frame(g)))) return;
     const uint32_t n_o = n_out[f];
     if (kStride) {
         for (int64_t bx = blockIdx.x; bx * kPtThreads < (int64_t)n_o; bx += gridDim.x)
@@ -335,9 +340,11 @@
 }
 
 __global__ __launch_bounds__(256) void k_cloud_heads_fix(const uint32_t* __restrict__ n_out, const uint64_t* __restrict__ out_off,
-                                                         int waves_per_frame, CloudHeads ch)
+                                                         int waves_per_frame, CloudHeads ch, const VoxelGeom* __restrict__ geom,
+                                                         int fused)
 {
     const int f = blockIdx.y;
+    if (fused && fused_frame(geom[f])) return;
     const int64_t j = (int64_t)blockIdx.x * 256 + threadIdx.x;
     if (j >= waves_per_frame || j * kWave >= (int64_t)n_out[f]) return;
     bool head = j == 0;
@@ -354,7 +361,8 @@
 }
 
 __global__ __launch_bounds__(256) void k_cloud_bbox_fold(const float* __restrict__ slots, int nbx, int frames,
-                                                         const uint32_t* __restrict__ n_out, float* __restrict__ partial)
+                                                         const uint32_t* __restrict__ n_out, float* __restrict__ partial,
+                                                         const VoxelGeom* __restrict__ geom, int fused)
 {
     __shared__ float mm_lds[6 * 4];
     float lo[3] = {__builtin_inff(), __builtin_inff(), __builtin_inff()};
@@ -362,7 +370,9 @@
     const int64_t total = (int64_t)nbx * frames;
     for (int64_t i = (int64_t)blockIdx.x * 256 + threadIdx.x; i < total; i += (int64_t)gridDim.x * 256) {
         const int f = (int)(i / nbx), bx = (int)(i - (int64_t)f * nbx);
-        if ((int64_t)bx * 64 < (int64_t)n_out[f]) {
+        const bool used = (fused && fused_frame(geom[f])) ? (int64_t)bx * kScatTile < (int64_t)geom[f].n
+                                                         : (int64_t)bx * 64 < (int64_t)n_out[f];
+        if (used) {
 #pragma unroll
             for (int a = 0; a < 3; ++a) {
                 lo[a] = fminf(lo[a], slots[i * 6 + a]);
@@ -627,3 +637,301 @@
         if (c < cnt) dst[o0 + c] = slots[sidx];
     }
 }
+
+struct SumsJob {
+    const o3dr_point* in;
+    int64_t in_fstride;
+    float z_offset;
+    const uint32_t* vhist;
+    const uint32_t* vhist_part;
+    const uint64_t* out_off;
+    const uint32_t* n_out;
+    o3dr_point* out_base;
+    float* out_mm;
+    int mm_slots;
+    uint32_t* seg_first;
+    int parts;
+    CloudCounters* cc;
+    CloudHeads ch;
+};
+constexpr int kSegFirstWords = kMaxRadix + 1;
+struct SumsLds {
+    uint32_t heads[kScatTile / 32];
+    uint32_t wpre[kScatTile / 32];
+    uint32_t first[kMaxRadix];
+    uint32_t lastkey[kMaxRadix];
+    int32_t wlast[kScatWaves][3];
+    float mm[6 * kScatWaves];
+    uint32_t nfirst;
+};
+
+__device__ __forceinline__ void sums_add(const uint4& p, float z_offset, float& sx, float& sy, float& sz, float& sr, float& sg,
+                                         float& sb, float& sa)
+{
+    sx += __uint_as_float(p.x);
+    sy += __uint_as_float(p.y);
+    sz += __uint_as_float(p.z) + z_offset;
+    sr += (float)((p.w >> 16) & 255u);
+    sg += (float)((p.w >> 8) & 255u);
+    sb += (float)(p.w & 255u);
+    sa += (float)(p.w >> 24);
+}
+
+__global__ __launch_bounds__(kScatThreads, 4) void k_radix_scatter_sums(const uint32_t* __restrict__ keys0, const uint32_t* __restrict__ vals0,
+                                                                     const uint32_t* __restrict__ keys1, const uint32_t* __restrict__ vals1,
+                                                                     int64_t cap, const VoxelGeom* __restrict__ geom, int n_tiles,
+                                                                     const uint32_t* __restrict__ hist_scanned,
+                                                                     const uint32_t* __restrict__ hist_part, int tm, SumsJob S)
+{
+    __shared__ ScatterLds L;
+    __shared__ SumsLds M;
+    const int f = blockIdx.y;
+    const VoxelGeom g = geom[f];
+    if (!fused_frame(g)) return;
+    const int item = xcd_chunk_item(blockIdx.x, (int)(((int64_t)g.n + kScatTile - 1) / kScatTile));
+    if (item < 0) return;
+    const int tile = item / kScatParts, part = item % kScatParts;
+    const int pass = (int)g.passes - 1;
+    ScatterJob J;
+    const int par = (pass + (int)g.buf0) & 1;
+    J.kin = (par ? keys1 : keys0) + (int64_t)f * cap;
+    J.vin = (par ? vals1 : vals0) + (int64_t)f * cap;
+    J.kout = nullptr;
+    J.vout = nullptr;
+    J.hist = hist_scanned + (int64_t)f * kMaxRadix * n_tiles;
+    J.hist_part = hist_part + (int64_t)f * kMaxRadix * n_tiles;
+    J.n = g.n;
+    J.bins = geom_bins(g);
+    J.dmask = (uint32_t)J.bins - 1u;
+    J.shift = pass * (int)g.bpp;
+    J.pass = pass;
+    J.n_tiles = n_tiles;
+    J.frame_vec = (((int64_t)f * cap) & 3) == 0;
+    J.tm = tm != 0;
+    uint32_t key0[kSortRounds], val0[kSortRounds], g0;
+    scatter_load(J, tile, part, key0, val0, g0);
+    const uint32_t cnt = scatter_stage(J, tile, part, L, key0, val0, g0);
+    const uint32_t* stage = L.smem;
+    const uint32_t* stage_v = L.smem + kScatTile;
+    const int shift = J.shift, bins = J.bins;
+    const uint32_t dmask = J.dmask, lomask = (1u << shift) - 1u;
+    const int64_t n = g.n;
+    const int64_t base = (int64_t)tile * kSortTile + (int64_t)part * kScatTile;
+    const int tid = threadIdx.x, lane = tid & 63, w = tid >> 6;
+
+#pragma unroll
+    for (int r = 0; r < kSortRounds; ++r) {
+        const uint32_t p = r * kScatThreads + tid;
+        const bool h = p < cnt && (p == 0 || stage[p] != stage[p - 1]);
+        const unsigned long long b = __ballot(h);
+        if (lane < 2) M.heads[(r * kScatThreads + w * 64) / 32 + lane] = lane ? (uint32_t)(b >> 32) : (uint32_t)b;
+    }
+    if (tid == 0) M.nfirst = 0;
+    __syncthreads();
+    uint32_t runs;
+    {
+        const uint32_t c = tid < kScatTile / 32 ? (uint32_t)__popc(M.heads[tid]) : 0u;
+        const uint32_t ex = block_excl_scan_u32<kScatWaves>(c, L.scan_lds, runs);
+        if (tid < kScatTile / 32) M.wpre[tid] = ex;
+    }
+    __syncthreads();
+    auto run_index = [&](uint32_t p) -> uint32_t {
+        return M.wpre[p >> 5] + (uint32_t)__popc(M.heads[p >> 5] & ((1u << (p & 31u)) - 1u));
+    };
+
+    if (tid < bins) {
+        const uint32_t b = L.local_base[tid];
+        const uint32_t e = tid + 1 < bins ? L.local_base[tid + 1] : cnt;
+        uint32_t first = 0;
+        int32_t off = 0;
+        if (b < e) {
+            const uint32_t fj = run_index(b), key = stage[b];
+            bool cont = false;
+            for (int64_t i = base - 1; i >= 0; --i) {
+                const uint32_t k = J.kin[i];
+                if (((k ^ key) & lomask) != 0u) break;
+                if (k == key) {
+                    cont = true;
+                    break;
+                }
+            }
+            uint32_t vb = S.vhist[(int64_t)f * kMaxRadix * n_tiles + hist_at(J.tm, tid, tile, n_tiles)];
+            if (part != 0) vb += S.vhist_part[(int64_t)f * kMaxRadix * n_tiles + hist_at(J.tm, tid, tile, n_tiles)];
+            first = fj | (cont ? 0x80000000u : 0u);
+            off = (int32_t)vb - (int32_t)fj - (cont ? 1 : 0);
+            M.lastkey[tid] = stage[e - 1];
+        }
+        M.first[tid] = first;
+        L.delta[tid] = (uint32_t)off;
+    }
+    __syncthreads();
+    uint32_t* run_tab = L.smem;
+    {
+        uint32_t ent[kSortRounds];
+#pragma unroll
+        for (int r = 0; r < kSortRounds; ++r) {
+            const uint32_t p = r * kScatThreads + tid;
+            ent[r] = 0xffffffffu;
+            if (p < cnt && ((M.heads[p >> 5] >> (p & 31u)) & 1u)) ent[r] = run_index(p) | (((stage[p] >> shift) & dmask) << 13);
+        }
+        __syncthreads();
+#pragma unroll
+        for (int r = 0; r < kSortRounds; ++r)
+            if (ent[r] != 0xffffffffu) run_tab[ent[r] & 0x1fffu] = (uint32_t)(r * kScatThreads + tid) | (ent[r] & ~0x1fffu);
+        __syncthreads();
+    }
+
+    const uint4* src = reinterpret_cast<const uint4*>(S.in + (int64_t)f * S.in_fstride);
+    const uint64_t fo = S.out_off[f];
+    const uint32_t n_o = S.n_out[f];
+    uint4* out = reinterpret_cast<uint4*>(S.out_base + fo);
+    uint32_t* segf = S.seg_first + ((int64_t)f * S.parts + item) * kSegFirstWords;
+    float lo3[3] = {__builtin_inff(), __builtin_inff(), __builtin_inff()};
+    float hi3[3] = {-__builtin_inff(), -__builtin_inff(), -__builtin_inff()};
+    bool any = false, bad = false;
+    GroupCoord carry = {0, 0, 0};
+    for (uint32_t j0 = 0; j0 < runs; j0 += kScatThreads) {
+        const uint32_t j = j0 + (uint32_t)tid;
+        bool active = false, has_pred = false;
+        uint32_t o = 0;
+        uint4 res = make_uint4(0, 0, 0, 0);
+        if (j < runs) {
+            const uint32_t rt = run_tab[j];
+            const uint32_t b = rt & 0x1fffu, d = rt >> 13;
+            const uint32_t e = j + 1 < runs ? (run_tab[j + 1] & 0x1fffu) : cnt;
+            const uint32_t fst = M.first[d], fj = fst & 0x7fffffffu, cont = fst >> 31;
+            const bool own = !(cont && j == fj);
+            o = L.delta[d] + j;
+            if (own && o >= n_o) bad = true;
+            if (own && o < n_o) {
+                active = true;
+                has_pred = j > fj + cont;
+                float sx = 0.f, sy = 0.f, sz = 0.f, sr = 0.f, sg = 0.f, sb = 0.f, sa = 0.f;
+                uint32_t npts = e - b;
+                for (uint32_t li = b; li < e; li += 8) {
+                    uint32_t id[8];
+                    uint4 p[8];
+#pragma unroll
+                    for (int k = 0; k < 8; ++k) {
+                        id[k] = (li + k < e) ? stage_v[li + k] : 0xffffffffu;
+                        if (id[k] != 0xffffffffu && id[k] >= g.n) {
+                            bad = true;
+                            id[k] = 0xffffffffu;
+                        }
+                    }
+#pragma unroll
+                    for (int k = 0; k < 8; ++k)
+                        if (id[k] != 0xffffffffu) p[k] = src[id[k]];
+#pragma unroll
+                    for (int k = 0; k < 8; ++k)
+                        if (id[k] != 0xffffffffu) sums_add(p[k], S.z_offset, sx, sy, sz, sr, sg, sb, sa);
+                }
+                const uint32_t seg_end = (int)d + 1 < bins ? L.local_base[d + 1] : cnt;
+                if (e == seg_end && base + (int64_t)cnt < n) {
+                    const uint32_t key = M.lastkey[d];
+                    bool alive = true;
+                    for (int64_t i = base + cnt; alive && i < n; i += 4) {
+                        uint32_t kk[4], id[4];
+                        uint4 p[4];
+#pragma unroll
+                        for (int k = 0; k < 4; ++k) kk[k] = (i + k < n) ? J.kin[i + k] : ~key;
+#pragma unroll
+                        for (int k = 0; k < 4; ++k) {
+                            alive = alive && ((kk[k] ^ key) & lomask) == 0u;
+                            id[k] = 0xffffffffu;
+                            if (alive && kk[k] == key) {
+                                ++npts;
+                                id[k] = J.vin[i + k];
+                                if (id[k] >= g.n) {
+                                    bad = true;
+                                    id[k] = 0xffffffffu;
+                                }
+                            }
+                        }
+#pragma unroll
+                        for (int k = 0; k < 4; ++k)
+                            if (id[k] != 0xffffffffu) p[k] = src[id[k]];
+#pragma unroll
+                        for (int k = 0; k < 4; ++k)
+                            if (id[k] != 0xffffffffu) sums_add(p[k], S.z_offset, sx, sy, sz, sr, sg, sb, sa);
+                    }
+                }
+                const float nf = (float)npts;
+                const float cx = sx / nf, cy = sy / nf, cz = sz / nf - S.z_offset;
+                const uint32_t rgba = ((uint32_t)(sa / nf) << 24) | ((uint32_t)(sr / nf) << 16) | ((uint32_t)(sg / nf) << 8) |
+                                      (uint32_t)(sb / nf);
+                res = make_uint4(__float_as_uint(cx), __float_as_uint(cy), __float_as_uint(cz), rgba);
+                out[o] = res;
+                any = true;
+                lo3[0] = fminf(lo3[0], cx), lo3[1] = fminf(lo3[1], cy), lo3[2] = fminf(lo3[2], cz);
+                hi3[0] = fmaxf(hi3[0], cx), hi3[1] = fmaxf(hi3[1], cy), hi3[2] = fmaxf(hi3[2], cz);
+            }
+        }
+        if (S.ch.flags) {
+            uint32_t cell;
+            GroupCoord gc = {0, 0, 0};
+            if (active) gc = group_coord_of(res, S.ch.inv, S.ch.z_offset, cell);
+            GroupCoord prev;
+            prev.bx = wave_shr1_i32(gc.bx);
+            prev.iy = wave_shr1_i32(gc.iy);
+            prev.iz = wave_shr1_i32(gc.iz);
+            if (lane == 63) {
+                M.wlast[w][0] = gc.bx;
+                M.wlast[w][1] = gc.iy;
+                M.wlast[w][2] = gc.iz;
+            }
+            __syncthreads();
+            if (lane == 0 && w > 0) prev = GroupCoord{M.wlast[w - 1][0], M.wlast[w - 1][1], M.wlast[w - 1][2]};
+            if (lane == 0 && w == 0) prev = carry;
+            carry = GroupCoord{M.wlast[kScatWaves - 1][0], M.wlast[kScatWaves - 1][1], M.wlast[kScatWaves - 1][2]};
+            __syncthreads();
+            if (active && !has_pred) segf[1 + atomicAdd(&M.nfirst, 1u)] = o;
+            uint64_t word = ~0ull;
+            uint32_t bits = 0;
+            if (active) {
+                uint32_t bit;
+                head_flag_place(fo + o, word, bit);
+                if (has_pred && group_differs(gc, prev)) bits = 1u << bit;
+            }
+#pragma unroll
+            for (int off = 1; off < 64; off <<= 1) {
+                const uint32_t ob = __shfl_down(bits, off, 64);
+                const uint64_t ow = __shfl_down(word, off, 64);
+                if (lane + off < 64 && ow == word) bits |= ob;
+            }
+            const uint64_t uw = __shfl_up(word, 1, 64);
+            if (bits && (lane == 0 || uw != word)) atomicOr(&S.ch.flags[word], bits);
+        }
+    }
+    if (bad) atomicOr(&S.cc->status, O3DR_STATUS_INTERNAL);
+    if (S.out_mm) block_minmax_store<kScatWaves>(lo3, hi3, any, M.mm, S.out_mm + ((int64_t)f * S.mm_slots + item) * 6);
+    if (S.ch.flags) {
+        __syncthreads();
+        if (tid == 0) segf[0] = M.nfirst;
+    }
+}
+
+__global__ __launch_bounds__(kMaxRadix) void k_sums_heads_fix(const VoxelGeom* __restrict__ geom, const uint64_t* __restrict__ out_off,
+                                                              const o3dr_point* __restrict__ out_base, const uint32_t* __restrict__ seg_first,
+                                                              int parts, CloudHeads ch)
+{
+    const int f = blockIdx.y, item = blockIdx.x;
+    const VoxelGeom g = geom[f];
+    if (!fused_frame(g) || (int64_t)item * kScatTile >= (int64_t)g.n) return;
+    const uint32_t* segf = seg_first + ((int64_t)f * parts + item) * kSegFirstWords;
+    if (threadIdx.x >= segf[0]) return;
+    const uint32_t o = segf[1 + threadIdx.x];
+    const uint64_t go = out_off[f] + o;
+    bool head = o == 0;
+    if (!head) {
+        const uint4* cb = reinterpret_cast<const uint4*>(out_base);
+        uint32_t cell;
+        head = group_differs(group_coord_of(cb[go], ch.inv, ch.z_offset, cell), group_coord_of(cb[go - 1], ch.inv, ch.z_offset, cell));
+    }
+    if (head) {
+        uint64_t word;
+        uint32_t bit;
+        head_flag_place(go, word, bit);
+        atomicOr(&ch.flags[word], 1u << bit);
+    }
+}
diff --git a/online_3d_reconstruction_amd/csrc/o3dr_api.hip b/online_3d_reconstruction_amd/csrc/o3dr_api.hip
--- a/online_3d_reconstruction_amd/csrc/o3dr_api.hip
+++ b/online_3d_reconstruction_amd/csrc/o3dr_api.hip
@@ -65,6 +65,7 @@
     int exact_box = 0;
     int use_runs = 1;
     int small_path = 1;
+    int fused_sums = 0;
 
     Workspace ws;
     size_t ws_elems = 0;
@@ -109,6 +110,7 @@
     hipStream_t copy_stream = nullptr;
     hipEvent_t ev_copied[2] = {nullptr, nullptr}, ev_done[2] = {nullptr, nullptr};
     int test_corrupt = 0;
+    int test_corrupt_batch = 0;
     int test_fail_at = 0;
     int64_t xchg_stats[8] = {0, 0, 0, 0, 0, 0, 0, 0};
     DevBuf nn_q, nn_t, nn_cells, nn_src;
@@ -201,6 +203,10 @@
         size_t o_tile = off;  off += align256(TE * 4);
         size_t o_hist = off;  off += align256(TS * kMaxRadix * 4);
         size_t o_histp = off; off += align256(TS * kMaxRadix * 4);
+        size_t o_vh = off;    off += align256(TS * kMaxRadix * 4);
+        size_t o_vhp = off;   off += align256(TS * kMaxRadix * 4);
+        size_t o_sf = off;    off += align256(TS * kScatParts * (kMaxRadix + 1) * 4);
+        size_t o_nvf = off;   off += align256((size_t)F * 4);
         size_t o_segc = off;  off += align256(TG * 4);
         size_t o_hb = off;    off += align256(TG * 256);
         size_t o_part = off;  off += align256(((TS * kMaxRadix + TG + TE + E) / 4096 + 8 * (size_t)F + 16) * 4);
@@ -237,6 +243,10 @@
         w.tile_cnt = (uint32_t*)(base + o_tile);
         w.hist = (uint32_t*)(base + o_hist);
         w.hist_part = (uint32_t*)(base + o_histp);
+        w.vhist = (uint32_t*)(base + o_vh);
+        w.vhist_part = (uint32_t*)(base + o_vhp);
+        w.seg_first = (uint32_t*)(base + o_sf);
+        w.n_vox_fused = (uint32_t*)(base + o_nvf);
         w.seg_cnt = (uint32_t*)(base + o_segc);
         w.head_bits = (uint8_t*)(base + o_hb);
         w.scan_partial = (uint32_t*)(base + o_part);
@@ -385,6 +395,8 @@
     if (sm_env) c->small_path = atoi(sm_env) != 0;
     const char* th_env = getenv("O3DR_TEST_HOOKS");
     c->test_hooks = th_env && atoi(th_env) == 1;
+    const char* fs_env = getenv("O3DR_FUSED_SUMS");
+    if (fs_env) c->fused_sums = atoi(fs_env) != 0;
     const char* sl_env = getenv("O3DR_SLABS");
     if (sl_env && sl_env[0] == '0') c->slab_shift_env = -1;
     else if (sl_env && sl_env[0] == 's' && atoi(sl_env + 1) >= 0 && atoi(sl_env + 1) <= 20) c->slab_shift_env = atoi(sl_env + 1);
@@ -1473,6 +1485,9 @@
         v.mm_used = a.n_tiles + 1;
         v.stats = c->stats_dev;
         v.use_runs = 0;
+        v.fused_sums = c->fused_sums;
+        v.test_corrupt = c->test_corrupt_batch;
+        c->test_corrupt_batch = 0;
         if (with_sor) {
             v.mm_used = launch_sor(&c->prof, c->stream, c->ws, c->ws.pts, cap, c->ws.n_valid, nb, cap, a.n_tiles + 1, 1.0, c->ws.sor_pts,
                                    cap, c->ws.sor_n);
@@ -2675,6 +2690,13 @@
     c->test_corrupt = 1;
     return O3DR_OK;
 }
+extern "C" int o3dr_test_corrupt_next_batch(o3dr_ctx* c)
+{
+    CTX_ENTER(c);
+    if (!c->test_hooks) return fail(O3DR_ERR_INVALID_ARG, "test hooks are off (create the context with O3DR_TEST_HOOKS=1)");
+    c->test_corrupt_batch = 1;
+    return O3DR_OK;
+}
 
 extern "C" int o3dr_test_sor_distances(o3dr_ctx* c, float* out, int64_t n)
 {
diff --git a/online_3d_reconstruction_amd/csrc/o3dr_device.h b/online_3d_reconstruction_amd/csrc/o3dr_device.h
--- a/online_3d_reconstruction_amd/csrc/o3dr_device.h
+++ b/online_3d_reconstruction_amd/csrc/o3dr_device.h
@@ -100,6 +100,10 @@
     uint32_t* tile_cnt = nullptr;
     uint32_t* hist = nullptr;
     uint32_t* hist_part = nullptr;
+    uint32_t* vhist = nullptr;
+    uint32_t* vhist_part = nullptr;
+    uint32_t* n_vox_fused = nullptr;
+    uint32_t* seg_first = nullptr;
     uint32_t* seg_cnt = nullptr;
     uint8_t* head_bits = nullptr;
     uint32_t* scan_partial = nullptr;
@@ -202,6 +206,7 @@
     const uint8_t* heads_in = nullptr;
     int keys_ready = 0;
     int test_corrupt = 0;
+    int fused_sums = 0;
 };
 constexpr int kBoxFoldBlocks = 1024;
 void launch_voxel_grid(Profiler* pf, hipStream_t s, Workspace& ws, const VoxelArgs& v);
diff --git a/online_3d_reconstruction_amd/csrc/o3dr_kernels.hip b/online_3d_reconstruction_amd/csrc/o3dr_kernels.hip
--- a/online_3d_reconstruction_amd/csrc/o3dr_kernels.hip
+++ b/online_3d_reconstruction_amd/csrc/o3dr_kernels.hip
@@ -223,6 +223,7 @@
     const int64_t grp_slots = use_runs ? ws.grp_slots : 0;
     const int64_t max_groups = grp_slots / kGroupCells;
     const VoxelGeom* sort_geom = use_runs ? ws.geom_runs : ws.geom;
+    const int fuse = (v.fused_sums && !v.passthrough && !use_runs && v.min_points <= 1 && cap > 0) ? 1 : 0;
     if (!v.passthrough && cap > 0) {
         const dim3 grid(n_sort_tiles, F);
         if (use_runs) {
@@ -243,7 +244,7 @@
                 k_run_geom<<<cdiv64(F, 64), 64, 0, s>>>(ws.geom, ws.n_runs, F, ws.geom_runs, v.use_runs > 1 ? 1 : 0, grp_slots);
                 k_run_starts<<<dim3(cdiv64(n_seg_tiles, kStartWaves), F), kStartWaves * kWave, 0, s>>>(
                     ws.keys[0], ws.keys[1], cap, ws.geom, n_seg_tiles, ws.seg_cnt, ws.n_runs, ws.run_start, 0, ws.keys[1],
-                    ws.geom_runs, v.in, v.z_offset, hb);
+                    ws.geom_runs, v.in, v.z_offset, hb, 0);
             }
             {
                 ProfScope ps(pf, O3DR_K_KEYGEN, s);
@@ -260,13 +261,17 @@
         for (int pass = 0; pass < kMaxPasses; ++pass) {
             if (!(pass == 0 && !use_runs && !v.keys_ready)) {
                 ProfScope ps(pf, O3DR_K_SORT_HIST, s);
-                k_radix_hist<<<grid, kSortThreads, 0, s>>>(ws.keys[0], ws.keys[1], cap, sort_geom, pass, n_sort_tiles,
-                                                          ws.hist, ws.hist_part, tm);
+                if (fuse && pass >= 1)
+                    k_radix_hist<true><<<grid, kSortThreads, 0, s>>>(ws.keys[0], ws.keys[1], cap, sort_geom, pass, n_sort_tiles,
+                                                                     ws.hist, ws.hist_part, tm, ws.vhist, ws.vhist_part);
+                else
+                    k_radix_hist<false><<<grid, kSortThreads, 0, s>>>(ws.keys[0], ws.keys[1], cap, sort_geom, pass, n_sort_tiles,
+                                                                      ws.hist, ws.hist_part, tm, nullptr, nullptr);
             }
             {
                 ProfScope ps(pf, O3DR_K_OTHER, s);
                 if (tm)
-                    k_scan_hist_tm<<<F, 1024, tm_lds, s>>>(ws.hist, sort_geom, pass, n_sort_tiles);
+                    k_scan_hist_tm<<<F, 1024, tm_lds, s>>>(ws.hist, sort_geom, pass, n_sort_tiles, nullptr);
                 else
                     launch_scan(s, ws.hist, hist_row, hist_row, F, nullptr, nullptr, ws.scan_partial, sort_geom, pass,
                                 n_sort_tiles);
@@ -274,14 +279,21 @@
             {
                 ProfScope ps(pf, O3DR_K_SORT_SCATTER, s);
                 k_radix_scatter_lane<<<dim3(xcd_grid((int64_t)n_sort_tiles * kScatParts), F), kScatThreads, 0, s>>>(
-                    ws.keys[0], ws.vals[0], ws.keys[1], ws.vals[1], cap, sort_geom, pass, n_sort_tiles, ws.hist, ws.hist_part, tm);
-            }
+                    ws.keys[0], ws.vals[0], ws.keys[1], ws.vals[1], cap, sort_geom, pass, n_sort_tiles, ws.hist, ws.hist_part, tm, fuse);
+            }
+        }
+        if (fuse) {
+            ProfScope ps(pf, O3DR_K_OTHER, s);
+            if (tm)
+                k_scan_hist_tm<<<F, 1024, tm_lds, s>>>(ws.vhist, sort_geom, -1, n_sort_tiles, ws.n_vox_fused);
+            else
+                launch_scan(s, ws.vhist, hist_row, hist_row, F, ws.n_vox_fused, nullptr, ws.scan_partial, sort_geom, -1, n_sort_tiles);
         }
         const dim3 sgrid(n_seg_tiles, F);
         {
             ProfScope ps(pf, O3DR_K_SEGMENT, s);
             k_run_heads<<<dim3(cdiv64(n_seg_tiles, kHeadWaves), F), kHeadWaves * kWave, 0, s>>>(ws.keys[0], ws.keys[1], cap, sort_geom, n_seg_tiles,
-                                                                                       ws.seg_cnt, -1, ws.head_bits);
+                                                                                       ws.seg_cnt, -1, ws.head_bits, fuse);
         }
         {
             ProfScope ps(pf, O3DR_K_OTHER, s);
@@ -290,7 +302,7 @@
         {
             ProfScope ps(pf, O3DR_K_SEGMENT, s);
             k_run_starts<<<dim3(cdiv64(n_seg_tiles, kStartWaves), F), kStartWaves * kWave, 0, s>>>(ws.keys[0], ws.keys[1], cap, sort_geom, n_seg_tiles, ws.seg_cnt, ws.n_vox,
-                                              ws.seg_start, -1, nullptr, nullptr, nullptr, 0.f, ws.head_bits);
+                                              ws.seg_start, -1, nullptr, nullptr, nullptr, 0.f, ws.head_bits, fuse);
         }
         if (v.min_points > 1) {
             {
@@ -310,7 +322,7 @@
         }
     }
     if (v.test_corrupt && cap > 0 && !v.passthrough)
-        k_test_corrupt_payload<<<1, 1, 0, s>>>(ws.vals[0], ws.vals[1], sort_geom);
+        k_test_corrupt_payload<<<1, 1, 0, s>>>(ws.vals[0], ws.vals[1], sort_geom, fuse);
     if (cap > 0 && use_runs) {
         {
             ProfScope ps(pf, O3DR_K_OTHER, s);
@@ -333,7 +345,7 @@
     {
         ProfScope ps(pf, O3DR_K_OTHER, s);
         k_frame_offsets<<<1, 256, 0, s>>>(ws.geom, ws.n_vox, n_keep, use_runs ? ws.n_grp_out : nullptr, F, v.passthrough,
-                                          ws.n_out, ws.out_off, v.cc, v.stats, sort_geom);
+                                          ws.n_out, ws.out_off, v.cc, v.stats, sort_geom, fuse ? ws.n_vox_fused : nullptr);
     }
     const int nbx = cdiv64(cap, kPtThreads);
     if (cap > 0 && use_runs) {
@@ -349,23 +361,50 @@
         CloudHeads heads = v.cloud_heads;
         heads.wave_gc = ws.wave_gc;
         const uint32_t* keep = (v.min_points > 1 && !v.passthrough) ? ws.keep_idx : nullptr;
+        const int parts = n_sort_tiles * kScatParts;
+        if (fuse) {
+            ProfScope ps(pf, O3DR_K_CENTROID, s);
+            SumsJob S;
+            S.in = v.in;
+            S.in_fstride = v.in_fstride;
+            S.z_offset = v.z_offset;
+            S.vhist = ws.vhist;
+            S.vhist_part = ws.vhist_part;
+            S.out_off = ws.out_off;
+            S.n_out = ws.n_out;
+            S.out_base = v.out_base;
+            S.out_mm = out_mm;
+            S.mm_slots = nbx * (kPtThreads / 64);
+            S.seg_first = ws.seg_first;
+            S.parts = parts;
+            S.cc = v.cc;
+            S.ch = heads;
+            k_radix_scatter_sums<<<dim3(xcd_grid(parts), F), kScatThreads, 0, s>>>(ws.keys[0], ws.vals[0], ws.keys[1], ws.vals[1], cap, sort_geom,
+                                                                                  n_sort_tiles, ws.hist, ws.hist_part, tm, S);
+        }
         if (use_runs)
             k_centroid<true><<<dim3(nbx < 4096 ? nbx : 4096, F), kPtThreads, 0, s>>>(
                 v.in, v.in_fstride, ws.vals[0], ws.vals[1], cap, ws.seg_start, keep, ws.geom_runs, ws.n_out, ws.out_off,
-                v.z_offset, v.passthrough, v.out_base, out_mm, nbx, v.cc, CloudHeads{nullptr, {0.f, 0.f, 0.f}, 0.f, nullptr});
+                v.z_offset, v.passthrough, v.out_base, out_mm, nbx, v.cc, CloudHeads{nullptr, {0.f, 0.f, 0.f}, 0.f, nullptr}, 0);
+        else if (fuse)
+            k_centroid<true><<<dim3(nbx < 256 ? nbx : 256, F), kPtThreads, 0, s>>>(
+                v.in, v.in_fstride, ws.vals[0], ws.vals[1], cap, ws.seg_start, keep, ws.geom, ws.n_out, ws.out_off,
+                v.z_offset, v.passthrough, v.out_base, out_mm, nbx, v.cc, heads, fuse);
         else
             k_centroid<false><<<dim3(xcd_grid(nbx), F), kPtThreads, 0, s>>>(
                 v.in, v.in_fstride, ws.vals[0], ws.vals[1], cap, ws.seg_start, keep, ws.geom, ws.n_out, ws.out_off,
-                v.z_offset, v.passthrough, v.out_base, out_mm, nbx, v.cc, heads);
+                v.z_offset, v.passthrough, v.out_base, out_mm, nbx, v.cc, heads, fuse);
         if (!use_runs && v.cloud_heads.flags) {
             const int wpf = nbx * (kPtThreads / 64);
-            k_cloud_heads_fix<<<dim3(cdiv64(wpf, 256), F), 256, 0, s>>>(ws.n_out, ws.out_off, wpf, heads);
+            k_cloud_heads_fix<<<dim3(cdiv64(wpf, 256), F), 256, 0, s>>>(ws.n_out, ws.out_off, wpf, heads, sort_geom, fuse);
+            if (fuse)
+                k_sums_heads_fix<<<dim3(parts, F), kMaxRadix, 0, s>>>(sort_geom, ws.out_off, v.out_base, ws.seg_first, parts, heads);
         }
     }
     if (v.cloud_box && cap > 0 && !use_runs) {
         ProfScope ps(pf, O3DR_K_OTHER, s);
         const int nbx = cdiv64(cap, kPtThreads) * (kPtThreads / 64);
-        k_cloud_bbox_fold<<<kBoxFoldBlocks, 256, 0, s>>>(ws.out_mm, nbx, F, ws.n_out, ws.out_mm_partial);
+        k_cloud_bbox_fold<<<kBoxFoldBlocks, 256, 0, s>>>(ws.out_mm, nbx, F, ws.n_out, ws.out_mm_partial, sort_geom, fuse);
         k_cloud_bbox_merge<<<1, 384, 0, s>>>(ws.out_mm_partial, kBoxFoldBlocks, v.cloud_box);
     }
 }
@@ -402,32 +441,33 @@
         k_run_geom<<<1, 64, 0, s>>>(ws.geom, ws.n_runs, 1, ws.geom_runs, 1, INT64_MAX);
         k_run_starts<<<dim3(cdiv64(n_seg_tiles, kStartWaves), 1), kStartWaves * kWave, 0, s>>>(
             ws.keys[0], ws.keys[1], cap, ws.geom, n_seg_tiles, ws.seg_cnt, ws.n_runs, ws.run_start, 0, ws.keys[1], ws.geom_runs, in,
-            z_offset, ws.head_bits);
+            z_offset, ws.head_bits, 0);
     }
     const dim3 grid(n_sort_tiles, 1);
     const int64_t hist_row = (int64_t)kMaxRadix * n_sort_tiles;
     for (int pass = 0; pass < kMaxPasses; ++pass) {
         {
             ProfScope ps(pf, O3DR_K_SORT_HIST, s);
-            k_radix_hist<<<grid, kSortThreads, 0, s>>>(ws.keys[0], ws.keys[1], cap, sort_geom, pass, n_sort_tiles, ws.hist, ws.hist_part, tm);
+            k_radix_hist<false><<<grid, kSortThreads, 0, s>>>(ws.keys[0], ws.keys[1], cap, sort_geom, pass, n_sort_tiles, ws.hist, ws.hist_part,
+                                                              tm, nullptr, nullptr);
         }
         {
             ProfScope ps(pf, O3DR_K_OTHER, s);
             if (tm)
-                k_scan_hist_tm<<<1, 1024, tm_lds, s>>>(ws.hist, sort_geom, pass, n_sort_tiles);
+                k_scan_hist_tm<<<1, 1024, tm_lds, s>>>(ws.hist, sort_geom, pass, n_sort_tiles, nullptr);
             else
                 launch_scan(s, ws.hist, hist_row, hist_row, 1, nullptr, nullptr, ws.scan_partial, sort_geom, pass, n_sort_tiles);
         }
         {
             ProfScope ps(pf, O3DR_K_SORT_SCATTER, s);
             k_radix_scatter_lane<<<dim3(xcd_grid((int64_t)n_sort_tiles * kScatParts), 1), kScatThreads, 0, s>>>(
-                ws.keys[0], ws.vals[0], ws.keys[1], ws.vals[1], cap, sort_geom, pass, n_sort_tiles, ws.hist, ws.hist_part, tm);
+                ws.keys[0], ws.vals[0], ws.keys[1], ws.vals[1], cap, sort_geom, pass, n_sort_tiles, ws.hist, ws.hist_part, tm, 0);
         }
     }
     {
         ProfScope ps(pf, O3DR_K_SEGMENT, s);
         k_run_heads<<<dim3(cdiv64(n_seg_tiles, kHeadWaves), 1), kHeadWaves * kWave, 0, s>>>(ws.keys[0], ws.keys[1], cap, sort_geom,
-                                                                                             n_seg_tiles, ws.seg_cnt, -1, ws.head_bits);
+                                                                                             n_seg_tiles, ws.seg_cnt, -1, ws.head_bits, 0);
     }
     {
         ProfScope ps(pf, O3DR_K_OTHER, s);
@@ -437,9 +477,9 @@
         ProfScope ps(pf, O3DR_K_SEGMENT, s);
         k_run_starts<<<dim3(cdiv64(n_seg_tiles, kStartWaves), 1), kStartWaves * kWave, 0, s>>>(
             ws.keys[0], ws.keys[1], cap, sort_geom, n_seg_tiles, ws.seg_cnt, ws.n_vox, ws.seg_start, -1, nullptr, nullptr, nullptr, 0.f,
-            ws.head_bits);
-    }
-    if (test_corrupt) k_test_corrupt_payload<<<1, 1, 0, s>>>(ws.vals[0], ws.vals[1], sort_geom);
+            ws.head_bits, 0);
+    }
+    if (test_corrupt) k_test_corrupt_payload<<<1, 1, 0, s>>>(ws.vals[0], ws.vals[1], sort_geom, 0);
 }
 
 void launch_inc_fold(Profiler* pf, hipStream_t s, Workspace& ws, const o3dr_point* in, float z_offset, const IncFoldArgs& a,
@@ -573,14 +613,14 @@
     const size_t tm_lds = (size_t)n_sort_tiles * (kMaxRadix + 1) * sizeof(uint32_t);
     const int tm = tm_lds <= 48 * 1024 ? 1 : 0;
     for (int pass = 0; pass < passes && pass < kMaxPasses; ++pass) {
-        k_radix_hist<<<dim3(n_sort_tiles, F), kSortThreads, 0, s>>>(ws.keys[0], ws.keys[1], cap, ws.geom, pass, n_sort_tiles, ws.hist,
-                                                                    ws.hist_part, tm);
+        k_radix_hist<false><<<dim3(n_sort_tiles, F), kSortThreads, 0, s>>>(ws.keys[0], ws.keys[1], cap, ws.geom, pass, n_sort_tiles,
+                                                                           ws.hist, ws.hist_part, tm, nullptr, nullptr);
         if (tm)
-            k_scan_hist_tm<<<F, 1024, tm_lds, s>>>(ws.hist, ws.geom, pass, n_sort_tiles);
+            k_scan_hist_tm<<<F, 1024, tm_lds, s>>>(ws.hist, ws.geom, pass, n_sort_tiles, nullptr);
         else
             launch_scan(s, ws.hist, hist_row, hist_row, F, nullptr, nullptr, ws.scan_partial, ws.geom, pass, n_sort_tiles);
         k_radix_scatter_lane<<<dim3(xcd_grid((int64_t)n_sort_tiles * kScatParts), F), kScatThreads, 0, s>>>(
-            ws.keys[0], ws.vals[0], ws.keys[1], ws.vals[1], cap, ws.geom, pass, n_sort_tiles, ws.hist, ws.hist_part, tm);
+            ws.keys[0], ws.vals[0], ws.keys[1], ws.vals[1], cap, ws.geom, pass, n_sort_tiles, ws.hist, ws.hist_part, tm, 0);
     }
 }
 
```

Result: no change. 34400 frames/s, median of 6 (+0.5%).
